# bentherien/point-cloud-reid

Measured on AMD Instinct MI355X. Metric: siamese pair-comparisons/sec @1024 pts, higher is better.
Workload: dtype bf16x3

## Files before the change

### include/pcr.h

```cpp
#ifndef PCR_H_
#define PCR_H_

#ifdef __cplusplus
extern "C" {
#endif

typedef void *pcr_stream_t;

enum pcr_status {
  PCR_OK = 0,
  PCR_ERR_INVALID = 1,
  PCR_ERR_LAUNCH = 2
};

int pcr_abi_version(void);
#define PCR_PREC_F32 0
#define PCR_PREC_BF16X3 1
#define PCR_PREC_BF16 2
const char *pcr_status_string(int status);


int pcr_fps_f32(const float *xyz, float *temp, int *idx, int B, int N, int M, pcr_stream_t stream);

int pcr_fps_dist_f32(const float *dist, float *temp, int *idx, int B, int N, int M,
// ... 1 lines not shown

int pcr_pairwise_sqdist_f32(const float *a, const float *b, float *out, int B, int N, int M, int C, int norm,
                            pcr_stream_t stream);

int pcr_ball_query_f32(const float *centres, const float *xyz, int *idx, int B, int N, int M,
                       float min_r, float max_r, int K, pcr_stream_t stream);

int pcr_ball_query_cnt_f32(const float *centres, const float *xyz, int *idx, int *cnt, int B, int N, int M,
                           float min_r, float max_r, int K, pcr_stream_t stream);

long pcr_ball_query_rows_floats(int B, int M, int K);
int pcr_ball_query_rows_ok(int N, int K, float min_r);
int pcr_ball_query_rows_f32(const float *centres, const float *xyz, int *idx, int *cnt, float *rows, int B, int N, int M,
                            float min_r, float max_r, int K, pcr_stream_t stream);

int pcr_fps_ball_query_rows_ok(int N, int M, int K);
int pcr_fps_ball_query_rows_f32(const float *xyz, float *temp, int *idx, float *new_xyz, int *cnt, float *rows, int B,
                                int N, int M, float max_r, int K, pcr_stream_t stream);

int pcr_fps_py_f32(const float *xyz, float *temp, const int *start, int *idx, int B, int N, int M,
                   pcr_stream_t stream);
int pcr_query_ball_point_f32(const float *centres, const float *xyz, int *idx, int B, int N, int M, float radius,
                             int K, pcr_stream_t stream);

int pcr_knn_f32(const float *xyz, const float *centres, int *idx, float *dist2, int B, int N, int M,
                int K, pcr_stream_t stream);

int pcr_gather_fwd_f32(const float *feat, const int *idx, float *out, int B, int C, int N, int M,
                       pcr_stream_t stream);
int pcr_gather_bwd_f32(const float *grad_out, const int *idx, float *grad_feat, int B, int C, int N,
                       int M, pcr_stream_t stream);

int pcr_group_fwd_f32(const float *feat, const int *idx, float *out, int B, int C, int N, int S,
                      int K, pcr_stream_t stream);
int pcr_group_bwd_f32(const float *grad_out, const int *idx, float *grad_feat, int B, int C, int N,
                      int S, int K, pcr_stream_t stream);

int pcr_three_nn_f32(const float *unknown, const float *known, float *dist2, int *idx, int B, int N,
                     int M, pcr_stream_t stream);

int pcr_three_interp_fwd_f32(const float *feat, const int *idx, const float *weight, float *out,
                             int B, int C, int M, int N, pcr_stream_t stream);
int pcr_three_interp_bwd_f32(const float *grad_out, const int *idx, const float *weight,
                             float *grad_feat, int B, int C, int N, int M, pcr_stream_t stream);


int pcr_box_frames_f32(const float *boxes, float *frames, int T, pcr_stream_t stream);

int pcr_points_in_boxes_batch_f32(const float *points, const float *boxes, int *out, int B, int P, int T,
                                  pcr_stream_t stream);

int pcr_points_in_boxes_f32(const float *points, const float *boxes, int *out, int B, int P, int T, pcr_stream_t stream);

#define PCR_CROP_FRAME_SENSOR 0
#define PCR_CROP_FRAME_CENTRED 1
#define PCR_CROP_FRAME_BOX 2
#define PCR_CROP_RULE_TRACKER 0
#define PCR_CROP_RULE_DATASET 1
#define PCR_CROP_MAX_POINTS 2617344
#define PCR_CROP_MAX_BOXES 65536
#define PCR_CROP_MAX_SAMPLES 65536
#define PCR_CROP_MAX_STRIDE 16
int pcr_crop_boxes_ok(int P, int M, int n, int stride);
int pcr_crop_boxes_f32(const float *points, int stride, const float *boxes, const int *rand, const long long *seed,
                       float *clouds, int *lengths, int P, int M, int n, int frame, int rule, int z_is_centre,
                       pcr_stream_t stream);


#define PCR_ASSOC_MAX_OBJECTS 4096
#define PCR_ASSOC_MAX_CLASSES 32
int pcr_assoc_pairs_ok(int T, int D, int num_classes, int cap);
int pcr_assoc_pairs_i32(const int *track_labels, const int *det_labels, const int *track_lengths, const int *det_lengths,
                        int *pairs, int *count, int T, int D, int num_classes, int min_points, int cap,
                        pcr_stream_t stream);

int pcr_assoc_cost_f32(const float *logits, const int *pairs, const int *count, const float *track_miss,
                       const float *det_new, const float *dist, float dist_max, float dist_penalty, float fill,
                       float *cost, int T, int D, int cap, pcr_stream_t stream);

#define PCR_LSA_MAX 1024
int pcr_lsa_ok(int B, int R, int C);
int pcr_lsa_f32(const float *cost, int *col4row, int *row4col, float *u, float *v, int *info, int B, int R, int C,
                pcr_stream_t stream);

int pcr_lsa_blocks_ok(int R, int C, int G);
int pcr_lsa_blocks_f32(const float *cost, const int *row_block, const int *col_block, int *col4row, int *row4col, float *u,
                       float *v, int *info, int R, int C, int G, pcr_stream_t stream);
int pcr_assoc_blocks_i32(const int *track_labels, const int *det_labels, int *row_block, int *col_block, int T, int D,
                         int de, int te, int num_classes, pcr_stream_t stream);

#define PCR_ASSOC_MAX_DECISIONS 4
#define PCR_COST_MARGIN 0
#define PCR_COST_SOFTMAX 1
typedef struct pcr_assoc_multi {
  int T, D, dd, td, cap;
  int kind, reduce;
  float dist_max, dist_penalty, fill;
  const float *logits;
  const int *pairs, *count;
  const float *det_dec, *trk_dec, *dist;
  void *ws;
  float *cost;
  int *det_choice, *trk_choice;
} pcr_assoc_multi;
typedef struct pcr_assoc_decode {
  int T, D, dd, td;
  int reduce, born_dec, kill_dec;
  float fill;
  const float *cost;
  const int *col4row, *row4col, *solver_info, *det_choice, *trk_choice;
  int *track_to_det, *det_to_track, *det_decision, *track_decision, *born, *kill, *info;
} pcr_assoc_decode;
int pcr_assoc_multi_ok(int T, int D, int dd, int td, int cap);
int pcr_assoc_multi_ws_bytes(int T, int D, int dd, int td);
int pcr_assoc_cost_multi_f32(const pcr_assoc_multi *p, pcr_stream_t stream);
int pcr_assoc_decode_i32(const pcr_assoc_decode *p, pcr_stream_t stream);


int pcr_nearest_bev_f32(const float *boxes7, float *out5, int N, pcr_stream_t stream);
int pcr_bev_frames_f32(const float *boxes5, float *frames, int N, pcr_stream_t stream);

#define PCR_IOU_AXIS 0
#define PCR_IOU_ROTATED 1
#define PCR_IOU_OVERLAP 2
#define PCR_IOU_MAX_BOXES 65535
int pcr_iou_bev_f32(const float *a, const float *b, float *out, int A, int B, int kind, pcr_stream_t stream);

#define PCR_NMS_MAX 4096
int pcr_nms_ok(int N);
int pcr_nms_ws_bytes(int N);
int pcr_nms_f32(const float *boxes, const float *scores, const float *thresh, int *order, int *keep, int *count,
                int *info, void *ws, int N, int kind, int pre_max, pcr_stream_t stream);

int pcr_track_nms_f32(const float *boxes5, const int *classes, const float *scores, const float *thresh,
                      int *suppressed, int N, pcr_stream_t stream);


#define PCR_BANK_MAX_ROW 1048576
typedef struct pcr_bank {
  int C, D, W;
  int frame_limit, replace_all, reset_on_match, propagate;
  int *lengths;
  float *boxes, *scores;
  int *labels, *ids, *steps, *misses, *next_id, *info;
  const int *track_to_det, *det_to_track, *det_labels, *det_lengths;
  const float *det_boxes, *det_scores;
  const int *born, *kill;
  const float *carry;
  int *src, *det_slot, *det_id;
} pcr_bank;
int pcr_bank_ok(int C, int D, int W, int feat_floats, int xyz_floats);
int pcr_bank_plan_i32(const pcr_bank *p, pcr_stream_t stream);
int pcr_bank_move_f32(const int *src, const float *det_feats, const float *det_xyz, float *feats, float *xyz, int C, int D,
                      int feat_floats, int xyz_floats, pcr_stream_t stream);
int pcr_bank_dist_f32(const float *boxes, const int *ids, const float *det_boxes, const float *carry_inv, float *out,
                      int C, int D, int W, pcr_stream_t stream);
int pcr_bank_retire_i32(const int *mask, int *labels, int *ids, int *lengths, int C, pcr_stream_t stream);


#define PCR_STORE_BUCKETS 20
#define PCR_STORE_PAIR_ATTEMPTS 32
#define PCR_STORE_PAIR_WORDS 40
#define PCR_STORE_MAX_SAMPLES 65536
#define PCR_STORE_INFO_RETRY 1
#define PCR_STORE_INFO_ITEM 2
#define PCR_STORE_INFO_ROW 4
typedef struct pcr_store_tables {
  int num_objects, num_classes;
  const int *obj_cls, *obj_fp, *obj_id;
  const int *nums_off, *nums_rows;
  const int *bucket_off, *bucket_rows;
  const int *pool_off, *pool_objs;
} pcr_store_tables;
int pcr_store_gather_f32(const float *points, const long long *offsets, int R, const int *rows, const int *keys,
                         const int *rand, const long long *seed, float *clouds, int *sizes, int *info, int B, int n,
                         pcr_stream_t stream);
int pcr_store_train_pairs_i32(const pcr_store_tables *tables, const int *items, const int *keys, const int *rand,
                              const long long *seed, int *rows, int *labels, int *ids, int *info, int B,
                              pcr_stream_t stream);


#define PCR_TRUTH_MAX_IDS 65536
#define PCR_TRUTH_DET_MATCH 0
#define PCR_TRUTH_DET_NEWBORN 1
#define PCR_TRUTH_DET_FP 2
#define PCR_TRUTH_TRACK_FN 3
#define PCR_TRUTH_TRACK_FP 4
#define PCR_TRUTH_TOTAL_GT 15
#define PCR_TRUTH_TOTAL_CORRECT 16
#define PCR_TRUTH_FRAMES 17
#define PCR_TRUTH_GT_TOTAL 18
#define PCR_TRUTH_TP 19
#define PCR_TRUTH_FP 20
#define PCR_TRUTH_FN 21
#define PCR_TRUTH_SWITCHES 22
#define PCR_TRUTH_UNTRACKED 23
#define PCR_TRUTH_STATS 24
typedef struct pcr_truth {
  int C, D, G, gt_cap, skip_empty, forced;
  const int *ids;
  int *slot_gt, *slot_tte, *gt_last, *stats;
  const int *col4row, *row4col, *info;
  const float *cost, *thresh;
  const int *gt_labels, *gt_ids, *gt_tte, *det_labels;
  const int *track_to_det, *det_to_track, *born, *kill;
  int *det_gt, *true_t2d, *true_d2t, *det_truth, *track_truth;
  const int *det_slot, *det_id;
} pcr_truth;
int pcr_truth_ok(int C, int D, int G, int W, int gt_cap);
int pcr_truth_cost_f32(const float *det_boxes, const int *det_labels, const float *gt_boxes, const int *gt_labels,
                       const int *gt_ids, const float *iou, float *cost, int D, int G, int W, int gt_cap,
                       pcr_stream_t stream);
int pcr_truth_decide_i32(const pcr_truth *p, pcr_stream_t stream);
int pcr_truth_record_i32(const pcr_truth *p, pcr_stream_t stream);


int pcr_knn_prefix_f32(const float *xyz, int *idx, int B, int N, int S, int K, pcr_stream_t stream);
int pcr_knn_prefix2_f32(const float *xyz, int *idx, int *idx2, int B, int N, int S, int K, int S2, int K2,
                        pcr_stream_t stream);

long pcr_packed_weight_floats(int cout, int cin);
int pcr_pack_weight_f32(const float *w, int cout, int cin, float *packed);
long pcr_packed_weight_bf16_floats(int cout, int cin);
int pcr_pack_weight_bf16x2_f32(const float *w, int cout, int cin, float *packed);

typedef struct pcr_sa_params {
  int mode, B, N, S, K, D;
  int c1, c2, c3;
  const float *xyz, *feat;
  const int *idx, *centre_idx;
  const float *wp[3], *scale[3], *shift[3];
  const float *wa, *wpq;
  const float *wps[2], *shift_pad[2];
  const int *cnt;
  int *tile_ws;
  float *pq_ws;
  int pq_ready;
  int feat_point_major, out_point_major;
  float *out;
  const float *wa_packed;
  int precision;
  const float *wps_bf[2];
  const float *wa_shift_packed;
  const float *row_tab;
  int *claim_ws;
  int pq_has_xyz;
} pcr_sa_params;
int pcr_sa_mlp_f32(const pcr_sa_params *p, pcr_stream_t stream);
long pcr_sa_claim_ws_ints(int c1, int c2, int c3, int K, int N, int precision);
long pcr_sa_tile_ws_ints(int B, int S, int K, int c2, int c3);
int pcr_sa_krow_uses_tiles(int c1, int c2, int c3, int K, int precision);
int pcr_sa_uses_row_table(int c1, int c2, int c3, int K, int precision);

int pcr_dense_pm_f32(const float *x, const float *wp, float *y, int B, int cin, int cout, int L,
                     int x_point_major, pcr_stream_t stream);
int pcr_dense_pm_prec_f32(const float *x, const float *wp_bf, float *y, int B, int cin, int cout, int L,
                          int x_point_major, int precision, pcr_stream_t stream);
int pcr_dense_pm_xyz_f32(const float *x, const float *wp_bf, const float *xyz, const float *wxyz, float *y, int B, int cin,
                         int cout, int L, int x_point_major, int precision, int q_rows, int q_off, pcr_stream_t stream);
int pcr_sa_tables_take_xyz(int mode, int D, int c1, int c2, int c3, int K, int precision);

typedef struct pcr_attn_params {
  int B, Lq, Sk;
  int c1, c2, d, cout;
  int nhead;
  int q_pos, residual;
  const float *feat_q, *xyz_q;
  const float *feat_k, *xyz_k;
  const int *kv_index;
  const int *q_index;
  const float *pos0_w, *pos0_b;
  const float *wq, *bq;
  const float *wkv, *bkv;
  const float *wmerge;
  const float *wmlp0, *wmlp2;
  const float *ln1_g, *ln1_b, *ln2_g, *ln2_b;
  const float *wfinal, *bfinal; int cfinal;
  const float *wkv_wide, *bkv_wide, *wmerge_packed;
  float *kv;
  float *out;
  int precision;
  const float *wq_bf, *wmlp0_bf, *wmlp2_bf, *wfinal_bf;
  int kv_splits;
  float *kv_part;
  const float *wkv_bf;
  const float *wmlp0_bf_xpad;
  float *pool_out;
} pcr_attn_params;
long pcr_attn_kv_floats(int d);
int pcr_attn_kv_splits(int B, int Sk, int d);
int pcr_attn_kv_f32(const pcr_attn_params *p, pcr_stream_t stream);
int pcr_attn_apply_f32(const pcr_attn_params *p, pcr_stream_t stream);
int pcr_attn_apply_pool_ok(const pcr_attn_params *p);

typedef struct pcr_live {
  const int *count;
  int period;
  int offset;
} pcr_live;
int pcr_attn_live_ok(const pcr_attn_params *p);
int pcr_attn_kv_live_f32(const pcr_attn_params *p, const pcr_live *live, pcr_stream_t stream);
int pcr_attn_apply_live_f32(const pcr_attn_params *p, const pcr_live *live, pcr_stream_t stream);

typedef struct pcr_head_params {
  int P, C, L, groups;
  const float *o;
  const float *w1, *w2;
  const float *gn1_g, *gn1_b, *gn2_g, *gn2_b;
  const float *w_out, *b_out;
  float *pooled, *logits;
  const float *w1t, *w2t;
} pcr_head_params;
int pcr_pool_head_f32(const pcr_head_params *p, pcr_stream_t stream);
int pcr_pool_head_live_f32(const pcr_head_params *p, const pcr_live *live, const float *dead_value, pcr_stream_t stream);

int pcr_pool_both_f32(const float *x, float *out, int B, int C, int L, pcr_stream_t stream);

int pcr_channel_max_f32(const float *x, float *out, int B, int C, int L, int window, pcr_stream_t stream);

int pcr_dense_f32(const float *x, const float *wp, const float *scale, const float *shift, float *y,
                  int B, int cin, int cout, int L, int act, pcr_stream_t stream);
int pcr_dense_xpm_f32(const float *x, const float *wp, const float *scale, const float *shift, float *y,
                      int B, int cin, int cout, int L, int act, pcr_stream_t stream);

int pcr_dense_gn_f32(const float *x, const float *wp, const float *gamma, const float *beta, const float *res,
                     float *y, int B, int cin, int cout, int L, int groups, int relu, pcr_stream_t stream);
int pcr_dense_prec_ok(int cin, int cout, int L);
int pcr_dense_prec_f32(const float *x, const float *wp_bf, const float *scale, const float *shift, float *y, int B, int cin,
                       int cout, int L, int act, int precision, pcr_stream_t stream);
int pcr_dense_gn_prec_f32(const float *x, const float *wp_bf, const float *gamma, const float *beta, const float *res,
                          float *y, int B, int cin, int cout, int L, int groups, int relu, int precision,
                          pcr_stream_t stream);
int pcr_dense_xpm_prec_ok(int cin, int cout, int L);
int pcr_dense_xpm_prec_f32(const float *x, const float *wp_bf, const float *scale, const float *shift, float *y, int B,
                           int cin, int cout, int L, int act, int precision, pcr_stream_t stream);


int pcr_max_over_l_f32(const float *x, float *out, int B, int C, int L, pcr_stream_t stream);

int pcr_dense_max_ok(int cin, int cout, int L);
int pcr_dense_max_f32(const float *x, const float *wp, const float *scale, const float *shift, float *out, int B, int cin,
                      int cout, int L, int act, pcr_stream_t stream);

int pcr_pack_bmm_f32(const float *t, float *wp_per_cloud, int B, int k, pcr_stream_t stream);
int pcr_dense_bmm_f32(const float *x, const float *wp_per_cloud, float *y, int B, int cin, int cout, int L,
                      pcr_stream_t stream);

int pcr_groupnorm_f32(const float *x, const float *gamma, const float *beta, const float *res, float *y, int B,
                      int C, int L, int groups, int relu, pcr_stream_t stream);


int pcr_knn_feat_f32(const float *x, float *xx_ws, int *idx, int B, int C, int N, int K, long x_bstride,
                     pcr_stream_t stream);

int pcr_edge_max_f32(const float *ta, const float *tb, const int *idx, const float *shift, float slope, float *out,
                     long out_bstride, float *out2, long out2_bstride, int B, int N, int Co, int K,
                     pcr_stream_t stream);

int pcr_local_attn_f32(const float *qkv, const int *idx, float *msg, int B, int N, int C, int K, int nhead, float eps,
                       pcr_stream_t stream);


int pcr_pack_weight_dev_f32(const float *w, int rows, int cols, int ld, int transpose, float *packed, pcr_stream_t stream);

int pcr_train_groups(int B, int L);
int pcr_train_groups_bwd(int B, int L, int cout, int cin);
struct pcr_tdense_fwd;
struct pcr_tdense_bwd;
int pcr_tdense_fwd_groups(const struct pcr_tdense_fwd *p);
int pcr_tdense_bwd_groups(const struct pcr_tdense_bwd *p);
int pcr_set_stream_min_blocks(int n);

typedef struct pcr_tdense_fwd {
  int B, cin1, cin2, cout, L;
  const float *x, *x2;
  const float *isc, *ish;
  int in_relu;
  const float *wp, *bias;
  const float *res;
  int out_relu;
  float *y;
  float *stats;
  int pool_K;
  const float *pool_gamma;
  float *pool_ymax;
  int *pool_arg;
} pcr_tdense_fwd;
int pcr_tdense_fwd_f32(const pcr_tdense_fwd *p, pcr_stream_t stream);
int pcr_tdense_fwd_pooled(const pcr_tdense_fwd *p);

typedef struct pcr_tdense_bwd {
  int B, cin1, cin2, cout, L;
  const float *g, *y;
  int dy_mode;
  const float *ka, *kb, *kc;
  const int *argmax;
  const float *pooled;
  int K, S;
  const float *x, *x2;
  const float *isc, *ish, *iinv;
  int in_relu;
  const float *wpT;
  float *dx, *dx2, *dstats, *dwp, *dbp;
  long part_stride;
  int precision;
  const float *wpT_bf;
} pcr_tdense_bwd;
int pcr_tdense_bwd_f32(const pcr_tdense_bwd *p, pcr_stream_t stream);
int pcr_pack_weight_bf16_dev_f32(const float *w, int rows, int cols, int ld, int transpose, float *packed,
                                 pcr_stream_t stream);

int pcr_local_attn_train_fwd_f32(const float *qkv, const int *idx, float *msg, int B, int N, int C, int K, int nhead,
                                 float eps, pcr_stream_t stream);
int pcr_local_attn_train_bwd_f32(const float *qkv, const int *idx, const float *g, float *dq, long dq_bstride, float *edge,
                                 int B, int N, int C, int K, int nhead, float eps, pcr_stream_t stream);

int pcr_reduce_parts_f32(const float *part, int nparts, long stride, int rows, int cols, int ld, float *out,
                         pcr_stream_t stream);

typedef struct pcr_reduce_job {
  const float *part;
  float *out;
  long stride;
  int nparts, rows, cols, ld;
} pcr_reduce_job;
int pcr_reduce_multi_f32(const pcr_reduce_job *jobs, int n, pcr_stream_t stream);

typedef struct pcr_bn_fwd_fin {
  const float *part;
  int nparts, C;
  double R;
  const float *gamma, *beta;
  float eps, momentum;
  float *running_mean, *running_var;
  float *scale, *shift, *inv_scale, *mean, *invstd;
  const float *shift0;
  int shift0_stride;
} pcr_bn_fwd_fin;
int pcr_bn_fwd_finalize_f32(const pcr_bn_fwd_fin *p, pcr_stream_t stream);

typedef struct pcr_bn_bwd_fin {
  const float *part;
  int nparts, C;
  double R;
  const float *gamma, *mean, *invstd;
  float *ka, *kb, *kc, *dgamma, *dbeta;
  const float *centre;
} pcr_bn_bwd_fin;
int pcr_bn_bwd_finalize_f32(const pcr_bn_bwd_fin *p, pcr_stream_t stream);

int pcr_sa_l1_fwd_f32(const float *xyz, const int *idx, const float *tab, const float *wa, const float *bias,
                      float *y, float *stats, int B, int N, int S, int K, int c1, pcr_stream_t stream);
int pcr_sa_l1_bwd_f32(const float *xyz, const int *idx, const float *g, const float *y, const float *ka,
                      const float *kb, const float *kc, float *dtab, float *dwa, int B, int N, int S, int K, int c1,
                      pcr_stream_t stream);
int pcr_sa_pool_fwd_f32(const float *y, const float *scale, const float *shift, float *pooled, int *argmax, float *ymax,
                        int B, int C, int S, int K, pcr_stream_t stream);
int pcr_sa_pool_bwd_stats_f32(const float *gp, const float *pooled, const float *ymax, float *part, float *gz, int B, int C,
                              int S, pcr_stream_t stream);

int pcr_tnorm_fwd_f32(const float *x, const float *gamma, const float *beta, const float *res, float *y, float *mean,
                      float *rstd, int B, int C, int L, int G, float eps, int relu, pcr_stream_t stream);
int pcr_tnorm_bwd_f32(const float *g, const float *x, const float *gamma, const float *mean, const float *rstd,
                      const float *y_relu, float *dx, float *dres, float *part, int B, int C, int L, int G,
                      pcr_stream_t stream);

typedef struct pcr_linattn {
  int B, Lq, Sk, d, H;
  float eps;
  const float *q, *k, *v;
  long q_bs, k_bs, v_bs;
  float *out, *A, *ks;
  const float *dout;
  float *dq, *dk, *dv;
  long dq_bs, dk_bs, dv_bs;
  int kv_roll;
} pcr_linattn;
int pcr_linattn_fwd_f32(const pcr_linattn *p, pcr_stream_t stream);
int pcr_linattn_bwd_f32(const pcr_linattn *p, pcr_stream_t stream);

typedef struct pcr_attn_tail {
  int B, L, d, c1, hid, out, residual;
  float eps;
  const float *msg, *res;
  const float *wm, *w0, *w2, *wmT, *w0T, *w2T;
  const float *g1, *b1, *g2, *b2;
  float *outp;
  const float *dout;
  float *dmsg, *dres, *parts;
  long part_stride;
  int precision;
  int fwd_precision;
} pcr_attn_tail;
int pcr_attn_tail_ok(int d, int c1, int hid, int out, int residual);
int pcr_attn_tail_part_floats(int d, int c1, int hid, int out);
int pcr_attn_tail_groups(const pcr_attn_tail *p);
int pcr_attn_tail_fwd_f32(const pcr_attn_tail *p, pcr_stream_t stream);
int pcr_attn_tail_bwd_f32(const pcr_attn_tail *p, pcr_stream_t stream);

typedef struct pcr_attn_head {
  int B, L, c, hd, d, np, src;
  const float *x, *xyz;
  const float *p1, *p2, *c1, *c2, *p2T;
  const float *w[3], *wT[3];
  float *outp;
  const float *dout;
  float *dx, *parts;
  long part_stride;
  int precision;
  int fwd_precision;
} pcr_attn_head;
int pcr_attn_head_ok(int c, int hd, int d, int np, int src);
int pcr_attn_head_part_floats(int c, int hd, int d, int np, int src);
int pcr_attn_head_groups(const pcr_attn_head *p);
int pcr_attn_head_fwd_f32(const pcr_attn_head *p, pcr_stream_t stream);
int pcr_attn_head_bwd_f32(const pcr_attn_head *p, pcr_stream_t stream);

int pcr_pool_pair_fwd_f32(const float *o, float *pooled, int *arg, int P, int C, int L, pcr_stream_t stream);
int pcr_pool_pair_bwd_f32(const float *g, const int *arg, float *dout, int P, int C, int L, pcr_stream_t stream);
int pcr_pool_both_fwd_f32(const float *o, float *pooled, int *arg, int P, int C, int L, pcr_stream_t stream);
int pcr_pool_both_bwd_f32(const float *g, const int *arg, float *dout, int P, int C, int L, pcr_stream_t stream);
int pcr_channel_max_fwd_f32(const float *x, float *y, int *arg, int B, int C, int L, int W, pcr_stream_t stream);
int pcr_channel_max_bwd_f32(const float *g, const int *arg, float *dx, int B, int C, int L, int W, pcr_stream_t stream);

int pcr_bn_sums_f32(const float *y, const float *g, const float *scale, const float *shift, int relu, float slope,
                    const float *centre, int centre_first, float *part, int nparts, int B, int C, int L,
                    pcr_stream_t stream);
int pcr_bn_affine_f32(const float *y, const float *g, const float *a0, const float *a1, const float *a2,
                      const float *scale, const float *shift, const float *centre, int relu, float slope, float *out,
                      int B, int C, int L, pcr_stream_t stream);
int pcr_edge_pool_fwd_f32(const float *y, const float *scale, const float *shift, float slope, float *pooled, int *arg,
                          float *yraw, int B, int C, int N, int K, pcr_stream_t stream);
int pcr_edge_pool_route_f32(const float *gp, const float *pooled, const int *arg, float slope, float *g, int B, int C,
                            int N, int K, pcr_stream_t stream);
int pcr_bmm_apply_f32(const float *x, const float *T, float *y, int B, int k, int N, int transposed, pcr_stream_t stream);
int pcr_bmm_dt_f32(const float *x, const float *dy, float *dT, int B, int k, int N, pcr_stream_t stream);

typedef struct pcr_pack_desc {
  const float *w;
  float *out;
  int rows, cols;
  int kind;
  int reserved;
} pcr_pack_desc;
int pcr_pack_weights_multi_f32(const pcr_pack_desc *descs_dev, int n, pcr_stream_t stream);

typedef struct pcr_opt_tensor {
  float *p, *g, *m, *v;
  long n;
  float step_size, bc2_sqrt, decay, one_m_beta1, beta2, one_m_beta2, eps, pad_;
} pcr_opt_tensor;
int pcr_opt_chunk(void);
int pcr_grad_sumsq_f32(const pcr_opt_tensor *tab, const int *chunk_tensor, const int *chunk_first, int n_chunks,
                       double *part, pcr_stream_t stream);
int pcr_adamw_step_f32(const pcr_opt_tensor *tab, const int *chunk_tensor, const int *chunk_first, int n_chunks,
                       const double *part, float max_norm, float *grad_norm, pcr_stream_t stream);


int pcr_wall_clock_khz(void);
int pcr_last_launch_arith(void);
int pcr_clock_probe(unsigned long long *ticks, int n_wg, int iters, pcr_stream_t stream);

#ifdef __cplusplus
}
#endif
#endif
```

### point-cloud-reid_amd/csrc/attn_kernels_impl.h

```cpp
#pragma once
#ifndef PCR_ATTN_PREC
#define PCR_ATTN_PREC 0
#endif
#include "tile_dense.h"

#include <stdio.h>

#include <vector>

namespace {
constexpr int kAPrec = PCR_ATTN_PREC;
struct AttnArgs {
  pcr_attn_params p;
  int dbg;
  int wpc;
  const int *live_count;
  int live_period, live_offset;
};

struct LiveWalk {
  unsigned n, period;
  long total;
  __device__ __forceinline__ long map(long v) const {
    const unsigned q = (unsigned)v / n;
    return (long)q * period + ((unsigned)v - q * n);
  }
};
__device__ __forceinline__ unsigned live_pairs(const AttnArgs &a) {
  int c = __builtin_amdgcn_readfirstlane(*a.live_count);
  c = c < 0 ? 0 : c;
  c -= a.live_offset;
  return (unsigned)(c < 0 ? 0 : (c > a.live_period ? a.live_period : c));
}
__device__ __forceinline__ LiveWalk live_walk(const AttnArgs &a) {
  LiveWalk w;
  w.n = live_pairs(a);
  w.period = (unsigned)a.live_period;
  const unsigned B = (unsigned)a.p.B, full = B / w.period, rem = B - full * w.period;
  w.total = (long)full * w.n + (rem < w.n ? rem : w.n);
  return w;
}
__device__ __forceinline__ bool live_cloud(const AttnArgs &a, unsigned b) {
  return b % (unsigned)a.live_period < live_pairs(a);
}

constexpr int kATraceWgs = 512, kATraceRecs = 24, kATraceMarks = 8;
__device__ unsigned long long g_attn_trace[2 * kATraceWgs * kATraceRecs * kATraceMarks];


__device__ __forceinline__ void pos_hidden(float *dst, int RP, const float *P, const float *w0,
                                           const float *b0, int d, int T) {
  for (int e = threadIdx.x; e < d * T; e += blockDim.x) {
    const int o = e / T, t = e - o * T;
    const float v = w0[o * 3] * P[t] + w0[o * 3 + 1] * P[RP + t] + w0[o * 3 + 2] * P[2 * RP + t] + b0[o];
    dst[o * RP + t] = fmaxf(v, 0.f);
  }
}

__device__ __forceinline__ void load_xyz3(float *P, int RP, const float *xyz, int L, int t0, int T) {
  for (int e = threadIdx.x; e < 3 * T; e += blockDim.x) {
    const int c = e / T, t = e - c * T;
    P[c * RP + t] = t0 + t < L ? xyz[(size_t)(t0 + t) * 3 + c] : 0.f;
  }
}

__device__ __forceinline__ void attn_kv_fold_write(const pcr_attn_params &p, const float *KVl, const float *s_kt, size_t b) {
  const int d = p.d, dh = d / p.nhead, ld = d + 1, tid = threadIdx.x;
  float *kv = p.kv + b * ((size_t)d * d + d);
  const int d_o = kThreads / d, d_dd = kThreads - d_o * d;
  int o = tid / d, dd = tid - o * d;
  int v0 = (dd / dh) * dh;
  for (int e = tid; e < d * d; e += kThreads, o += d_o, dd += d_dd) {
    if (dd >= d) {
      dd -= d;
      o++;
    }
    if (d_dd) v0 = (dd / dh) * dh;
    const float *wm = p.wmerge + (size_t)o * d + v0;
    const float *kr = KVl + dd * ld + v0;
    float m = 0.f;
#pragma unroll 8
    for (int v = 0; v < dh; v++) m += wm[v] * kr[v];
    if constexpr (kAPrec == 0) {
      const int kb = dd >> 3, rem = dd & 7;
      kv[(((size_t)kb * d + o) * 2 + (rem & 1)) * 4 + (rem >> 1)] = m;
    } else {
      const int s16 = dd >> 4, kk = dd & 15;
      const int hh = (kk >> 2) & 1, jj = (kk & 3) + ((kk >> 3) << 2);
      const size_t unit = (((size_t)s16 * (d >> 5) + (o >> 5)) * 2) * 64 + hh * 32 + (o & 31);
      const __bf16 hi = (__bf16)m;
      const __bf16 lo = (__bf16)(m - (float)hi);
      __bf16 *img = reinterpret_cast<__bf16 *>(kv);
      img[unit * 8 + jj] = hi;
      img[(unit + 64) * 8 + jj] = lo;
    }
  }
  __syncthreads();
  if (tid < d) kv[(size_t)d * d + tid] = s_kt[tid];
}

__device__ __forceinline__ void attn_kv_fold_mfma(const pcr_attn_params &p, const float *KVt, const float *s_kt, size_t b) {
  const int d = p.d, dh = d / p.nhead, ld = d + 1, tid = threadIdx.x;
  float *kv = p.kv + b * ((size_t)d * d + d);
  for (int hd = 0; hd < p.nhead; hd++) {
    const float *wm = p.wmerge_packed + (size_t)(hd * dh / 8) * d * 8;
    tile_dense(KVt + (size_t)(hd * dh) * ld + hd * dh, dh, ld, dh >> 5, wm, d, [&](float m, int o, int t) {
      const int dd = hd * dh + t;
      if constexpr (kAPrec == 0) {
        const int kb = dd >> 3, rem = dd & 7;
        kv[(((size_t)kb * d + o) * 2 + (rem & 1)) * 4 + (rem >> 1)] = m;
      } else {
        const int s16 = dd >> 4, kk = dd & 15;
        const int hh = (kk >> 2) & 1, jj = (kk & 3) + ((kk >> 3) << 2);
        const size_t unit = (((size_t)s16 * (d >> 5) + (o >> 5)) * 2) * 64 + hh * 32 + (o & 31);
        const __bf16 hi = (__bf16)m;
        const __bf16 lo = (__bf16)(m - (float)hi);
        __bf16 *img = reinterpret_cast<__bf16 *>(kv);
        img[unit * 8 + jj] = hi;
        img[(unit + 64) * 8 + jj] = lo;
      }
    });
  }
  __syncthreads();
  if (tid < d) kv[(size_t)d * d + tid] = s_kt[tid];
}

template <int TB, int NR, int WSEL, int NTW, bool BFP = false>
__device__ __forceinline__ void attn_kv_body(const AttnArgs &a) {
  constexpr int T = 32 * TB, RP = T + 1;
  constexpr int NPF = 4;
  extern __shared__ __attribute__((aligned(16))) float smem[];
  const pcr_attn_params &p = a.p;
  const int d = p.d, c2 = p.c2;
  float *XH = smem;
  float *KB = XH;
  float *VB = XH + d * RP;
  float *P = XH + (c2 + d) * RP;
  float *s_w0 = P + 3 * RP, *s_b0 = s_w0 + 3 * d;
  const int tail_a = (c2 + d + 3) * RP + 4 * d, tail_b = d * (d + 1) + d;
  float *s_ks = smem + (tail_a > tail_b ? tail_a : tail_b);
  const int tid = threadIdx.x, lane = tid & 63, wave = tid >> 6;
  const int l31 = lane & 31, h = lane >> 5;
  const size_t b = blockIdx.x;
  for (int e = tid; e < 3 * d; e += kThreads) s_w0[e] = p.pos0_w[e];
  for (int e = tid; e < d; e += kThreads) s_b0[e] = p.pos0_b[e];
  const float *feat = p.feat_k + b * c2 * p.Sk;
  const float *xyz = p.xyz_k + b * p.Sk * 3;
  const int nb = d >> 5, nT = nb * nb;
  const int dh = d / p.nhead;
  const float sk = (float)p.Sk;
  const float *bkv = p.bkv;

  f32x16 acc[NTW];
#pragma unroll
  for (int i = 0; i < NTW; i++)
#pragma unroll
    for (int r = 0; r < 16; r++) acc[i][r] = 0.f;
  int tile_ib[NTW];
#pragma unroll
  for (int it = 0; it < NTW; it++) tile_ib[it] = (wave + 4 * it) / nb;
  const int krow = tid % d, kpart = tid / d, kparts = kThreads / d;
  float ksum = 0.f;

  const int Q = T >> 2, npieces = c2 * Q;
#ifndef PCR_KV_PREFETCH
#define PCR_KV_PREFETCH 1
#endif
  const bool vec_ok = PCR_KV_PREFETCH && ((p.Sk & 3) == 0) && ((reinterpret_cast<size_t>(feat) & 15) == 0) && npieces <= NPF * kThreads;
  f32x4 pf[NPF];
  auto fetch = [&](int t0) {
#pragma unroll
    for (int u = 0; u < NPF; u++) {
      const int e = tid + u * kThreads;
      const int c = e / Q, q = e - c * Q;
      const bool ok = e < npieces;
      pf[u] = *reinterpret_cast<const f32x4 *>(feat + (size_t)(ok ? c : 0) * p.Sk + t0 + 4 * (ok ? q : 0));
    }
  };
  auto stash = [&]() {
#pragma unroll
    for (int u = 0; u < NPF; u++) {
      const int e = tid + u * kThreads;
      if (e < npieces) {
        const int c = e / Q, q = e - c * Q;
        float *dst = XH + c * RP + 4 * q;
        dst[0] = pf[u][0];
        dst[1] = pf[u][1];
        dst[2] = pf[u][2];
        dst[3] = pf[u][3];
      }
    }
  };
  const int nsplit = p.kv_splits > 1 ? p.kv_splits : 1;
  const int ntile = (p.Sk + T - 1) / T, tps = (ntile + nsplit - 1) / nsplit;
  const int t_lo = (int)blockIdx.y * tps * T;
  const int t_hi = (t_lo + tps * T) < p.Sk ? (t_lo + tps * T) : p.Sk;
  bool have = false;
  if (vec_ok && t_lo + T <= p.Sk && t_lo < t_hi) {
    fetch(t_lo);
    have = true;
  }
  for (int t0 = t_lo; t0 < t_hi; t0 += T) {
    const int valid = p.Sk - t0;
    if (have) stash();
    else load_tile(XH, RP, feat, c2, c2, p.Sk, t0, T);
    load_xyz3(P, RP, xyz, p.Sk, t0, T);
    __syncthreads();
    have = vec_ok && t0 + 2 * T <= p.Sk && t0 + T < t_hi;
    pos_hidden(XH + c2 * RP, RP, P, s_w0, s_b0, d, T);
    __syncthreads();
    auto kv_epi = [&](const f32x16 &acc, int cb, int tb, int l31, int h) {
      const int t = tb * 32 + l31;
      float *dst = XH + (cb * 32 + 4 * h) * RP + t;
      const bool live = t < valid;
      if (cb * 32 < d) {
#pragma unroll
        for (int r = 0; r < 16; r++) dst[((r & 3) + 8 * (r >> 2)) * RP] = live ? elu1(acc[r]) : 0.f;
      } else {
#pragma unroll
        for (int r = 0; r < 16; r++) dst[((r & 3) + 8 * (r >> 2)) * RP] = live ? acc[r] / sk : 0.f;
      }
    };
    auto kv_hook = [&]() { if (have) fetch(t0 + T); };
    if constexpr (BFP && kAPrec != 0 && WSEL != 0)
      tile_dense2p<kAPrec, TB, NR, WSEL, true>(XH, c2 + d, p.wkv_bf, 2 * d, true, kv_epi, bkv, nullptr, kv_hook);
    else
      tile_dense2<TB, NR, WSEL, true>(XH, c2 + d, p.wkv, 2 * d, true, kv_epi, bkv, nullptr, kv_hook);
    __syncthreads();
    {
      const float *row = KB + krow * RP;
      for (int t = kpart; t < T; t += kparts) ksum += row[t];
    }
#pragma unroll
    for (int it = 0; it < NTW; it++) {
      const int item = wave + 4 * it;
      if (item < nT) {
        const int ib = tile_ib[it], jb = item - ib * nb;
        const float *ap = KB + (ib * 32 + l31) * RP + h;
        const float *bp = VB + (jb * 32 + l31) * RP + h;
#pragma unroll 4
        for (int ks = 0; ks < T / 2; ks++)
          acc[it] = __builtin_amdgcn_mfma_f32_32x32x2f32(ap[2 * ks], bp[2 * ks], acc[it], 0, 0, 0);
      }
    }
    __syncthreads();
  }
  if (nsplit > 1) {
    float *part = p.kv_part + ((size_t)b * nsplit + blockIdx.y) * ((size_t)d * d + d);
    s_ks[tid] = ksum;
#pragma unroll
    for (int it = 0; it < NTW; it++) {
      const int item = wave + 4 * it;
      if (item < nT) {
        const int ib = tile_ib[it], jb = item - ib * nb;
#pragma unroll
        for (int r = 0; r < 16; r++)
          part[(size_t)(ib * 32 + (r & 3) + 8 * (r >> 2) + 4 * h) * d + jb * 32 + l31] = acc[it][r];
      }
    }
    __syncthreads();
    if (tid < d) {
      float s = 0.f;
      for (int pp = 0; pp < kparts; pp++) s += s_ks[pp * d + tid];
      part[(size_t)d * d + tid] = s;
    }
    return;
  }
  float *KVl = smem;
  const int ld = d + 1;
  const bool mfma_fold = p.wmerge_packed != nullptr && (dh & 31) == 0 && (d & 31) == 0;
  float *s_kt = smem + d * ld;
  s_ks[tid] = ksum;
#pragma unroll
  for (int it = 0; it < NTW; it++) {
    const int item = wave + 4 * it;
    if (item < nT) {
      const int ib = tile_ib[it], jb = item - ib * nb;
      const int v = jb * 32 + l31;
      const int hv = v / dh;
      const bool aligned = (dh & 31) == 0;
      const bool same_blk = (ib * 32) / dh == hv;
#pragma unroll
      for (int r = 0; r < 16; r++) {
        const int dd = ib * 32 + (r & 3) + 8 * (r >> 2) + 4 * h;
        const bool same = aligned ? same_blk : (dd / dh == hv);
        if (mfma_fold) KVl[v * ld + dd] = same ? acc[it][r] : 0.f;
        else KVl[dd * ld + v] = same ? acc[it][r] : 0.f;
      }
    }
  }
  __syncthreads();
  if (tid < d) {
    float s = 0.f;
    for (int pp = 0; pp < kparts; pp++) s += s_ks[pp * d + tid];
    s_kt[tid] = s;
  }
  if (mfma_fold) attn_kv_fold_mfma(p, KVl, s_kt, b);
  else attn_kv_fold_write(p, KVl, s_kt, b);
}

template <int TB, int NR, int WSEL, int NTW>
__global__ __launch_bounds__(kThreads) void attn_kv_kernel(AttnArgs a) {
  attn_kv_body<TB, NR, WSEL, NTW>(a);
}
template <int TB, int NR, int WSEL, int NTW>
__global__ __launch_bounds__(kThreads) __attribute__((amdgpu_waves_per_eu(3, 3))) void attn_kv_kernel_o3(AttnArgs a) {
  attn_kv_body<TB, NR, WSEL, NTW>(a);
}
template <int TB, int NR, int WSEL, int NTW>
__global__ __launch_bounds__(kThreads) __attribute__((amdgpu_waves_per_eu(3, 3))) void attn_kv_kernel_o3_live(AttnArgs a) {
  if (!live_cloud(a, blockIdx.x)) return;
  attn_kv_body<TB, NR, WSEL, NTW>(a);
}
template <int TB, int NR, int WSEL, int NTW, bool BFP = false>
__global__ __launch_bounds__(kThreads) __attribute__((amdgpu_waves_per_eu(2, 2))) void attn_kv_kernel_o2(AttnArgs a) {
  attn_kv_body<TB, NR, WSEL, NTW, BFP>(a);
}

constexpr int kKvsWaves = 8;
template <bool DIAG, bool BF, int XS = 4, bool ONEW = false, bool GATE = false>
// ... 382 lines not shown
          for (int e = 0; e < 8; e++) xv[e] = xf[8 * s2 + e];
          bf_split8(xv, ah[s2], al[s2], true);
        }
        f32x16 acc[2];
#pragma unroll
        for (int cb = 0; cb < 2; cb++)
#pragma unroll
          for (int r = 0; r < 16; r++) acc[cb][r] = 0.f;
        const bf16x8 *wb = reinterpret_cast<const bf16x8 *>(s_w) + lane;
#pragma unroll
        for (int s2 = 0; s2 < 4; s2++) {
          bf16x8 wh[2], wl[2];
#pragma unroll
          for (int cb = 0; cb < 2; cb++) {
            wh[cb] = wb[((s2 * 2 + cb) * 2) * 64];
            wl[cb] = wb[((s2 * 2 + cb) * 2 + 1) * 64];
          }
#pragma unroll
          for (int cb = 0; cb < 2; cb++) acc[cb] = __builtin_amdgcn_mfma_f32_32x32x16_bf16(ah[s2], wh[cb], acc[cb], 0, 0, 0);
#pragma unroll
          for (int cb = 0; cb < 2; cb++) acc[cb] = __builtin_amdgcn_mfma_f32_32x32x16_bf16(al[s2], wh[cb], acc[cb], 0, 0, 0);
#pragma unroll
          for (int cb = 0; cb < 2; cb++) acc[cb] = __builtin_amdgcn_mfma_f32_32x32x16_bf16(ah[s2], wl[cb], acc[cb], 0, 0, 0);
        }
#pragma unroll
        for (int r = 0; r < 16; r++) {
          acc[0][r] = elu1(acc[0][r] + bias0);
          acc[1][r] = (acc[1][r] + bias1) * inv_sk;
          ks += acc[0][r];
        }
#pragma unroll
        for (int r = 0; r < 16; r++) kv = __builtin_amdgcn_mfma_f32_32x32x2f32(acc[0][r], acc[1][r], kv, 0, 0, 0);
      }
    }
    ks += __shfl_xor(ks, 32, 64);
    float *KVl = s_red + cslot * KVS, *s_kt = KVl + D * LD;
    for (int round = 0; round < wpc2; round++) {
      if (wsub == round) {
#pragma unroll
        for (int r = 0; r < 16; r++) {
          float *dst = KVl + ((r & 3) + 8 * (r >> 2) + 4 * h) * LD + j;
          *dst = round == 0 ? kv[r] : *dst + kv[r];
        }
        if (h == 0) s_kt[j] = round == 0 ? ks : s_kt[j] + ks;
      }
      __syncthreads();
    }
    if (live && wsub == 0) {
      float *kvo = p.kv + (size_t)b * ((size_t)D * D + D);
      const float *ap = s_wm + j * LD + h;
      const float *bp = KVl + j * LD + h;
      const int hd = j / dh;
      f32x16 m;
#pragma unroll
      for (int r = 0; r < 16; r++) m[r] = 0.f;
#pragma unroll 4
      for (int s2 = 0; s2 < 16; s2++) {
        const float bv = bp[2 * s2];
        m = __builtin_amdgcn_mfma_f32_32x32x2f32((2 * s2 + h) / dh == hd ? bv : 0.f, ap[2 * s2], m, 0, 0, 0);
      }
      bf16x8 *img = reinterpret_cast<bf16x8 *>(kvo);
#pragma unroll
      for (int G = 0; G < 2; G++) {
        float v[8];
#pragma unroll
        for (int e = 0; e < 8; e++) v[e] = m[8 * G + e];
        bf16x8 hi, lo;
        bf_split8(v, hi, lo, true);
        const size_t unit = (((size_t)G * (D >> 5)) * 2) * 64 + h * 32 + j;
        img[unit] = hi;
        img[unit + 64] = lo;
      }
      if (lane < D) kvo[(size_t)D * D + lane] = s_kt[lane];
    }
    __syncthreads();
  }
}
#endif

__global__ __launch_bounds__(kThreads) void attn_kv_fold_kernel(AttnArgs a) {
  extern __shared__ __attribute__((aligned(16))) float smem[];
  const pcr_attn_params &p = a.p;
  const int d = p.d, dh = d / p.nhead, ld = d + 1, nsplit = p.kv_splits, tid = threadIdx.x;
  const size_t b = blockIdx.x, per = (size_t)d * d + d;
  float *KVl = smem, *s_kt = smem + d * ld;
  const float *part = p.kv_part + b * nsplit * per;
  for (int e = tid; e < d * d + d; e += kThreads) {
    float v = part[e];
    for (int y = 1; y < nsplit; y++) v += part[(size_t)y * per + e];
    if (e < d * d) {
      const int dd = e / d, c = e - dd * d;
      KVl[dd * ld + c] = (dd / dh == c / dh) ? v : 0.f;
    } else {
      s_kt[e - d * d] = v;
    }
  }
  __syncthreads();
  attn_kv_fold_write(p, KVl, s_kt, b);
}

#if PCR_ATTN_PREC == 0
template <int NRW>
__global__ __launch_bounds__(kThreads) void attn_kv_wide_kernel(AttnArgs a) {
  constexpr int TB = 1, T = 32, RP = 33, BAND = 64, RPK = BAND + 1;
  extern __shared__ __attribute__((aligned(16))) float smem[];
  const pcr_attn_params &p = a.p;
  const int d = p.d, c2 = p.c2, dh = d / p.nhead;
  const int g = blockIdx.x, hd = (g * BAND) / dh;
  const int OPW = BAND + dh;
  float *XH = smem;
  float *KB = XH, *VB = XH + BAND * RP;
  float *P = XH + (c2 + d) * RP;
  float *s_w0 = P + 3 * RP, *s_b0 = s_w0 + 3 * d;
  float *s_ks = s_b0 + d;
  const int tid = threadIdx.x, lane = tid & 63, wave = tid >> 6;
  const int l31 = lane & 31, h = lane >> 5;
  const size_t b = blockIdx.y;
  for (int e = tid; e < 3 * d; e += kThreads) s_w0[e] = p.pos0_w[e];
  for (int e = tid; e < d; e += kThreads) s_b0[e] = p.pos0_b[e];
  const float *feat = p.feat_k + b * c2 * p.Sk;
  const float *xyz = p.xyz_k + b * p.Sk * 3;
  const float sk = (float)p.Sk;
  const float *wband = p.wkv_wide + (size_t)g * ((size_t)ceil8(c2 + d) * OPW);
  const float *bband = p.bkv_wide + (size_t)g * OPW;
  const int nj = dh >> 5, nT = 2 * nj;
  f32x16 acc[4];
#pragma unroll
  for (int i = 0; i < 4; i++)
#pragma unroll
    for (int r = 0; r < 16; r++) acc[i][r] = 0.f;
  const int krow = tid & (BAND - 1), kpart = tid >> 6;
  float ksum = 0.f;
  for (int t0 = 0; t0 < p.Sk; t0 += T) {
    const int valid = p.Sk - t0;
    load_tile(XH, RP, feat, c2, c2, p.Sk, t0, T);
    load_xyz3(P, RP, xyz, p.Sk, t0, T);
    __syncthreads();
    pos_hidden(XH + c2 * RP, RP, P, s_w0, s_b0, d, T);
    __syncthreads();
    tile_dense2<TB, NRW, 0, true>(XH, c2 + d, wband, OPW, true,
                                  [&](const f32x16 &acc, int cb, int tb, int l31, int h) {
      const int t = tb * 32 + l31;
      float *dst = XH + (cb * 32 + 4 * h) * RP + t;
      const bool live = t < valid;
      if (cb * 32 < BAND) {
#pragma unroll
        for (int r = 0; r < 16; r++) dst[((r & 3) + 8 * (r >> 2)) * RP] = live ? elu1(acc[r]) : 0.f;
      } else {
#pragma unroll
        for (int r = 0; r < 16; r++) dst[((r & 3) + 8 * (r >> 2)) * RP] = live ? acc[r] / sk : 0.f;
      }
    }, bband);
    __syncthreads();
    {
      const float *row = KB + krow * RP;
      for (int t = kpart; t < T; t += 4) ksum += row[t];
    }
#pragma unroll
    for (int it = 0; it < 4; it++) {
      const int item = wave + 4 * it;
      if (item < nT) {
        const int ib = item / nj, jb = item - ib * nj;
        const float *ap = KB + (ib * 32 + l31) * RP + h;
        const float *bp = VB + (jb * 32 + l31) * RP + h;
#pragma unroll 4
        for (int ks = 0; ks < T / 2; ks++)
          acc[it] = __builtin_amdgcn_mfma_f32_32x32x2f32(ap[2 * ks], bp[2 * ks], acc[it], 0, 0, 0);
      }
    }
    __syncthreads();
  }
  float *KVt = smem;
  s_ks[tid] = ksum;
  __syncthreads();
  const float ks_total = tid < BAND ? s_ks[tid] + s_ks[64 + tid] + s_ks[128 + tid] + s_ks[192 + tid] : 0.f;
  __syncthreads();
#pragma unroll
  for (int it = 0; it < 4; it++) {
    const int item = wave + 4 * it;
    if (item < nT) {
      const int ib = item / nj, jb = item - ib * nj;
      const int v = jb * 32 + l31;
#pragma unroll
      for (int r = 0; r < 16; r++) KVt[v * RPK + ib * 32 + (r & 3) + 8 * (r >> 2) + 4 * h] = acc[it][r];
    }
  }
  __syncthreads();
  float *kv = p.kv + b * ((size_t)d * d + d);
  if (tid < BAND) kv[(size_t)d * d + g * BAND + tid] = ks_total;
  const float *wm = p.wmerge_packed + (size_t)(hd * dh / 8) * d * 8;
  tile_dense(KVt, dh, RPK, 2, wm, d, [&](float m, int o, int t) {
    const int dd = g * BAND + t;
    const int kb = dd >> 3, rem = dd & 7;
    kv[(((size_t)kb * d + o) * 2 + (rem & 1)) * 4 + (rem >> 1)] = m;
  });
}

#endif

template <int TB, int NR, bool GATE = false>
__global__ __launch_bounds__(kThreads) void attn_apply_kernel(AttnArgs a) {
  if constexpr (GATE) {
    if (!live_cloud(a, blockIdx.y)) return;
  }
  constexpr int T = 32 * TB, RP = T + 1;
  extern __shared__ __attribute__((aligned(16))) float smem[];
  const pcr_attn_params &p = a.p;
  const int d = p.d, c1 = p.c1, cout = p.cout;
  const int catC = c1 + d, catP = ceil8(catC);
  int rowsU = catP > 2 * d ? catP : 2 * d;
  if (ceil32(cout) > rowsU) rowsU = ceil32(cout);
  if (ceil32(p.cfinal) > rowsU) rowsU = ceil32(p.cfinal);
  float *U = smem;
  float *P = U + rowsU * RP;
  float *zs = P + 3 * RP;
  float *red = zs + p.nhead * RP;
  float *cst = red + 2 * (kThreads / T) * T;
  float *s_ksum = cst, *s_ln1g = cst + d, *s_ln1b = cst + 2 * d, *s_ln2g = cst + 3 * d, *s_ln2b = s_ln2g + cout;
  float *s_w0 = s_ln2b + cout, *s_b0 = s_w0 + 3 * d;
  const int tid = threadIdx.x;
  const size_t b = blockIdx.y;
  const int t0 = blockIdx.x * T;
  const size_t bq_ = p.q_index ? (size_t)p.q_index[b] : b;
  const float *feat = p.feat_q + bq_ * c1 * p.Lq;
  const size_t kb_ = p.kv_index ? (size_t)p.kv_index[b] : b;
  const float *kv = p.kv + kb_ * ((size_t)d * d + d);
  const int dh = d / p.nhead;
  for (int e = tid; e < d; e += kThreads) {
    s_ksum[e] = kv[(size_t)d * d + e];
    s_ln1g[e] = p.ln1_g[e];
    s_ln1b[e] = p.ln1_b[e];
    if (p.q_pos) {
      s_w0[3 * e] = p.pos0_w[3 * e];
      s_w0[3 * e + 1] = p.pos0_w[3 * e + 1];
      s_w0[3 * e + 2] = p.pos0_w[3 * e + 2];
      s_b0[e] = p.pos0_b[e];
    }
  }
  for (int e = tid; e < cout; e += kThreads) {
    s_ln2g[e] = p.ln2_g[e];
    s_ln2b[e] = p.ln2_b[e];
  }
  const float *ksum = s_ksum;
  float *MSG = U + c1 * RP;

  load_tile(U, RP, feat, c1, c1, p.Lq, t0, T);
  if (p.q_pos) {
    load_xyz3(P, RP, p.xyz_q + bq_ * p.Lq * 3, p.Lq, t0, T);
    __syncthreads();
    pos_hidden(MSG, RP, P, s_w0, s_b0, d, T);
    for (int e = tid; e < (catP - catC) * T; e += kThreads) U[(catC + e / T) * RP + e % T] = 0.f;
  } else {
    for (int e = tid; e < (catP - c1) * T; e += kThreads) U[(c1 + e / T) * RP + e % T] = 0.f;
  }
  __syncthreads();
  tile_dense2p<kAPrec, TB, NR>(U, p.q_pos ? catP : ceil8(c1), p.wq, d, true,
                               [&](float v, int o, int t) { MSG[o * RP + t] = elu1(v); }, p.bq);
  __syncthreads();
  for (int e = tid; e < p.nhead * T; e += kThreads) {
    const int hd = e / T, t = e - hd * T;
    float z = 0.f;
    for (int c = 0; c < dh; c++) z += MSG[(hd * dh + c) * RP + t] * ksum[hd * dh + c];
    zs[hd * RP + t] = (1.0f / (z + 1e-6f)) * (float)p.Sk;
  }
  __syncthreads();
  for (int hd = 0; hd < p.nhead; hd++)
    for (int e = tid; e < dh * T; e += kThreads) {
      const int o = hd * dh + e / T, t = e % T;
      MSG[o * RP + t] *= zs[hd * RP + t];
    }
  __syncthreads();
  tile_dense2p<kAPrec, TB, NR>(MSG, d, kv, d, true, [&](float v, int o, int t) { MSG[o * RP + t] = v; });
  __syncthreads();
  tile_layernorm(MSG, d, RP, T, s_ln1g, s_ln1b, red);
  tile_dense2p<kAPrec, TB, NR>(U, catP, p.wmlp0, 2 * d, true, [&](float v, int o, int t) { U[o * RP + t] = fmaxf(v, 0.f); });
  __syncthreads();
  tile_dense2p<kAPrec, TB, NR>(U, 2 * d, p.wmlp2, ceil32(cout), true, [&](float v, int o, int t) { U[o * RP + t] = v; });
  __syncthreads();
  tile_layernorm(U, cout, RP, T, s_ln2g, s_ln2b, red);
  if (p.residual) {
    for (int e = tid; e < cout * T; e += kThreads) {
      const int c = e / T, t = e - c * T;
      if (t0 + t < p.Lq) U[c * RP + t] += feat[(size_t)c * p.Lq + t0 + t];
    }
    __syncthreads();
  }
  int cres = cout;
  if (p.cfinal) {
    const int cf = p.cfinal;
    tile_dense2p<kAPrec, TB, NR>(U, cout, p.wfinal, ceil32(cf), true, [&](float v, int o, int t) { U[o * RP + t] = v; },
                                 p.bfinal);
    __syncthreads();
    cres = cf;
  }
  float *out = p.out + b * cres * p.Lq;
  for (int e = tid; e < cres * T; e += kThreads) {
    const int c = e / T, t = e - c * T;
    if (t0 + t < p.Lq) out[(size_t)c * p.Lq + t0 + t] = U[c * RP + t];
  }
}

#if PCR_ATTN_PREC != 0
constexpr int kApsWaves = 8;
template <bool QPOS, int C1S, int CF, int NOB = 2, int ND = 2, bool POOL = false, bool GATE = false>
__global__ __launch_bounds__(64 * kApsWaves) __attribute__((amdgpu_waves_per_eu(2, 2)))
void attn_apply_stream64_kernel(AttnArgs a) {
  static_assert(!QPOS || C1S == 2 * ND, "q_pos needs c1 == d");
  static_assert(NOB <= 2 || (NOB == 4 && !CF), "cout = 128 has no trailing conv");
  static_assert(!POOL || (!CF && NOB == 2), "pooled output: cout = 64, no trailing conv");
  constexpr int D = 32 * ND, SD = 2 * ND;
  constexpr int SQ = C1S + (QPOS ? SD : 0), S0 = C1S + SD, NX = 8 * C1S;
  extern __shared__ __attribute__((aligned(16))) float smem[];
  const pcr_attn_params &p = a.p;
  bf16x8 *s_wq = reinterpret_cast<bf16x8 *>(smem);
  bf16x8 *s_w0 = s_wq + SQ * ND * 128;
  bf16x8 *s_w2 = s_w0 + S0 * ND * 256;
  float *s_c = reinterpret_cast<float *>(s_w2 + ND * NOB * 512);
  f32x4 *s_p0 = reinterpret_cast<f32x4 *>(s_c + 448);
  float *s_ks = reinterpret_cast<float *>(s_p0 + 64);
  const int tid = threadIdx.x, lane = tid & 63, j = lane & 31, h = lane >> 5;
  const int wave = __builtin_amdgcn_readfirstlane(tid >> 6);
  LiveWalk lw{};
  if constexpr (GATE) {
    lw = live_walk(a);
    if ((long)blockIdx.x * kApsWaves >= lw.total * (POOL ? 1 : (p.Lq >> 5))) return;
  }
  {
    const f32x4 *wq = reinterpret_cast<const f32x4 *>(p.wq),
                *w0 = reinterpret_cast<const f32x4 *>((p.c1 & 15) ? p.wmlp0_bf_xpad : p.wmlp0),
                *w2 = reinterpret_cast<const f32x4 *>(p.wmlp2);
    f32x4 *dq = reinterpret_cast<f32x4 *>(s_wq), *d0 = reinterpret_cast<f32x4 *>(s_w0), *d2 = reinterpret_cast<f32x4 *>(s_w2);
    for (int e = tid; e < SQ * ND * 128; e += 64 * kApsWaves) dq[e] = wq[e];
    for (int e = tid; e < S0 * ND * 256; e += 64 * kApsWaves) d0[e] = w0[e];
    for (int e = tid; e < ND * NOB * 512; e += 64 * kApsWaves) d2[e] = w2[e];
    if (tid < D) {
      s_c[tid] = p.bq[tid];
      s_c[64 + tid] = p.ln1_g[tid];
      s_c[128 + tid] = p.ln1_b[tid];

      if (QPOS) s_p0[tid] = f32x4{p.pos0_w[3 * tid], p.pos0_w[3 * tid + 1], p.pos0_w[3 * tid + 2], p.pos0_b[tid]};
    }
    if (tid < 32 * NOB) {
      s_c[192 + tid] = p.ln2_g[tid];
      s_c[192 + 32 * NOB + tid] = p.ln2_b[tid];
    }
    if (CF && tid < 32 * CF) s_c[320 + tid] = p.bfinal[tid];
  }
  __syncthreads();
  const int nblk = p.Lq >> 5;
  const long nB = GATE ? lw.total : (long)p.B;
  const long nitem = nB * nblk;
  const int dh = D / p.nhead;
  const float skf = (float)p.Sk;
  float *ksw = s_ks + wave * 64;
  auto cvec = [&](const float *base, int cb, int g) __attribute__((always_inline)) {
    return *reinterpret_cast<const f32x4 *>(base + 32 * cb + 8 * g + 4 * h);
  };
  auto to_ops = [&](const f32x16 &acc, int G, bf16x8 &oh, bf16x8 &ol) __attribute__((always_inline)) {
    float v[8];
#pragma unroll
    for (int e = 0; e < 8; e++) v[e] = acc[8 * G + e];
    bf_split8(v, oh, ol, true);
  };
#ifdef PCR_SA_TRACE_BUILD
  const bool tracing = (a.dbg & 256) && lane == 0 && (wave == 0 || wave == 5) && blockIdx.x < kATraceWgs;
  unsigned long long *trace = g_attn_trace + (size_t)(2 * blockIdx.x + (wave ? 1 : 0)) * (kATraceRecs * kATraceMarks);
  int trace_it = 0;
#define PCR_AMARK(m)                                                                                       \
  do {                                                                                                     \
    if (tracing && trace_it < kATraceRecs) trace[trace_it * kATraceMarks + (m)] = __builtin_readcyclecounter(); \
  } while (0)
#define PCR_ANEXT() trace_it++
#else
#define PCR_AMARK(m) do { } while (0)
#define PCR_ANEXT() do { } while (0)
#endif
  const long nwav = (long)gridDim.x * kApsWaves, gw = (long)blockIdx.x * kApsWaves + wave;
  long pc = gw;
  int pblk = 0;
  float pmax = -INFINITY, psum = 0.f;
  for (long it = gw; POOL ? pc < nB : it < nitem; it += POOL ? 0 : nwav) {
    asm volatile("" ::: "memory");
    PCR_AMARK(0);
    const long vb = POOL ? pc : it / nblk;
    const int blk = POOL ? pblk : (int)(it - vb * nblk);
    const long b = GATE ? lw.map(vb) : vb;
    const size_t bq_ = p.q_index ? (size_t)p.q_index[b] : (size_t)b;
    const size_t kb_ = p.kv_index ? (size_t)p.kv_index[b] : (size_t)b;
    const float *kvp = p.kv + kb_ * ((size_t)D * D + D);
    const int t = blk * 32 + j;
    const __amdgpu_buffer_rsrc_t rfeat = __builtin_amdgcn_make_buffer_rsrc(
        const_cast<float *>(p.feat_q + bq_ * p.c1 * p.Lq), 0, p.c1 * p.Lq * 4, 0x00020000);
    const int vo = (4 * h * p.Lq + t) * 4;
    float xf[NX];
#pragma unroll
    for (int e = 0; e < NX; e++) {
      const int ch = 16 * (e >> 3) + bf_kpos(0, e & 7);
      xf[e] = __builtin_bit_cast(float, __builtin_amdgcn_raw_buffer_load_b32(rfeat, vo, ch * p.Lq * 4, 0));
    }
    if (lane < D) ksw[lane] = kvp[(size_t)D * D + lane];
    bf16x8 bh[4 * ND], bl[4 * ND];
    if constexpr (QPOS) {
      const float *xyz = p.xyz_q + (bq_ * p.Lq + t) * 3;
      const float px = xyz[0], py = xyz[1], pz = xyz[2];
#pragma unroll
      for (int s2 = 0; s2 < SD; s2++) {
        float hv[8];
#pragma unroll
        for (int e = 0; e < 8; e++) {
          const f32x4 w = s_p0[16 * s2 + bf_kpos(0, e) + 4 * h];
          const float v = w[0] * px + w[1] * py + w[2] * pz + w[3];
          hv[e] = relu_i(v);
        }
        bf_split8(hv, bh[C1S + s2], bl[C1S + s2], true);
      }
    }
#pragma unroll
    for (int e = 0; e < NX; e++) asm volatile("" : "+v"(xf[e]));
#pragma unroll
    for (int s2 = 0; s2 < C1S; s2++) {
      float xv[8];
#pragma unroll
      for (int e = 0; e < 8; e++) xv[e] = xf[8 * s2 + e];
      bf_split8(xv, bh[s2], bl[s2], true);
    }
    PCR_AMARK(1);
    f32x16 q[ND];
#pragma unroll
    for (int cb = 0; cb < ND; cb++)
#pragma unroll
      for (int r = 0; r < 16; r++) q[cb][r] = 0.f;
    {
      const bf16x8 *wb = s_wq + lane;
#pragma unroll
      for (int s2 = 0; s2 < SQ; s2++) {
        bf16x8 wh[ND], wl[ND];
#pragma unroll
        for (int cb = 0; cb < ND; cb++) {
          wh[cb] = wb[((s2 * ND + cb) * 2) * 64];
          wl[cb] = wb[((s2 * ND + cb) * 2 + 1) * 64];
        }
#pragma unroll
        for (int cb = 0; cb < ND; cb++) q[cb] = __builtin_amdgcn_mfma_f32_32x32x16_bf16(wh[cb], bh[s2], q[cb], 0, 0, 0);
#pragma unroll
        for (int cb = 0; cb < ND; cb++) q[cb] = __builtin_amdgcn_mfma_f32_32x32x16_bf16(wh[cb], bl[s2], q[cb], 0, 0, 0);
#pragma unroll
        for (int cb = 0; cb < ND; cb++) q[cb] = __builtin_amdgcn_mfma_f32_32x32x16_bf16(wl[cb], bh[s2], q[cb], 0, 0, 0);
      }
    }
    PCR_AMARK(2);
    bf16x8 mh[SD][ND], ml[SD][ND];
    {
      const bf16x8 *mb = reinterpret_cast<const bf16x8 *>(kvp) + lane;
#pragma unroll
      for (int s2 = 0; s2 < SD; s2++)
#pragma unroll
        for (int cb = 0; cb < ND; cb++) {
          mh[s2][cb] = mb[((s2 * ND + cb) * 2) * 64];
          ml[s2][cb] = mb[((s2 * ND + cb) * 2 + 1) * 64];
        }
    }
    __builtin_amdgcn_fence(__ATOMIC_RELEASE, "wavefront");
    __builtin_amdgcn_wave_barrier();
    __builtin_amdgcn_fence(__ATOMIC_ACQUIRE, "wavefront");
    float z16[2][2] = {{0.f, 0.f}, {0.f, 0.f}};
#pragma unroll
    for (int cb = 0; cb < ND; cb++)
#pragma unroll
      for (int g = 0; g < 4; g++) {
        const f32x4 bqv = cvec(s_c, cb, g), ksv = cvec(ksw, cb, g);
        float zz = 0.f;
#pragma unroll
        for (int qq = 0; qq < 4; qq++) {
          const float v = elu1(q[cb][4 * g + qq] + bqv[qq]);
          q[cb][4 * g + qq] = v;
          zz += v * ksv[qq];
        }
        if ((g & 1) == 0) z16[cb][g >> 1] = zz;
        else z16[cb][g >> 1] += zz;
      }
    float zs[2][2];
    {
      float za = z16[0][0], zb = z16[0][1], zc = z16[1][0], zd = z16[1][1];
      if (dh >= 32) {
        za += zb; zb = za;
        zc += zd; zd = zc;
      }
      if (ND == 2 && dh >= 64) {
        za += zc; zb = za; zc = za; zd = za;
      }
      za += __shfl_xor(za, 32, 64);
      zb += __shfl_xor(zb, 32, 64);
      zc += __shfl_xor(zc, 32, 64);
      zd += __shfl_xor(zd, 32, 64);
      zs[0][0] = (1.0f / (za + 1e-6f)) * skf;
      zs[0][1] = (1.0f / (zb + 1e-6f)) * skf;
      zs[1][0] = (1.0f / (zc + 1e-6f)) * skf;
      zs[1][1] = (1.0f / (zd + 1e-6f)) * skf;
    }
#pragma unroll
    for (int cb = 0; cb < ND; cb++)
#pragma unroll
      for (int r = 0; r < 16; r++) q[cb][r] *= zs[cb][r >> 3];
    bf16x8 ch_[SD], cl_[SD];
#pragma unroll
    for (int cb = 0; cb < ND; cb++)
#pragma unroll
      for (int G = 0; G < 2; G++) to_ops(q[cb], G, ch_[2 * cb + G], cl_[2 * cb + G]);
    f32x16 m[ND];
#pragma unroll
    for (int cb = 0; cb < ND; cb++)
#pragma unroll
      for (int r = 0; r < 16; r++) m[cb][r] = 0.f;
#pragma unroll
    for (int s2 = 0; s2 < SD; s2++) {
#pragma unroll
      for (int cb = 0; cb < ND; cb++) m[cb] = __builtin_amdgcn_mfma_f32_32x32x16_bf16(mh[s2][cb], ch_[s2], m[cb], 0, 0, 0);
#pragma unroll
      for (int cb = 0; cb < ND; cb++) m[cb] = __builtin_amdgcn_mfma_f32_32x32x16_bf16(mh[s2][cb], cl_[s2], m[cb], 0, 0, 0);
#pragma unroll
      for (int cb = 0; cb < ND; cb++) m[cb] = __builtin_amdgcn_mfma_f32_32x32x16_bf16(ml[s2][cb], ch_[s2], m[cb], 0, 0, 0);
    }
    auto layernorm = [&](auto &v, auto nb_tag, const float *gam, const float *bet) __attribute__((always_inline)) {
      constexpr int NB = decltype(nb_tag)::value;
      float sm = 0.f;
#pragma unroll
      for (int cb = 0; cb < NB; cb++)
#pragma unroll
        for (int r = 0; r < 16; r++) sm += v[cb][r];
      sm += __shfl_xor(sm, 32, 64);
      const float mean = sm / (32.0f * NB);
      float vr = 0.f;
#pragma unroll
      for (int cb = 0; cb < NB; cb++)
#pragma unroll
        for (int r = 0; r < 16; r++) {
          const float dlt = v[cb][r] - mean;
          vr += dlt * dlt;
        }
      vr += __shfl_xor(vr, 32, 64);
      const float inv = 1.0f / sqrtf(vr / (32.0f * NB) + 1e-5f);
#pragma unroll
      for (int cb = 0; cb < NB; cb++)
#pragma unroll
        for (int g = 0; g < 4; g++) {
          const f32x4 gv = cvec(gam, cb, g), bv = cvec(bet, cb, g);
#pragma unroll
          for (int qq = 0; qq < 4; qq++) v[cb][4 * g + qq] = (v[cb][4 * g + qq] - mean) * inv * gv[qq] + bv[qq];
        }
    };
    PCR_AMARK(3);
    layernorm(m, std::integral_constant<int, ND>{}, s_c + 64, s_c + 128);
    PCR_AMARK(4);
#pragma unroll
    for (int s2 = 0; s2 < C1S; s2++) {
      float xv[8];
#pragma unroll
      for (int e = 0; e < 8; e++) xv[e] = xf[8 * s2 + e];
      bf_split8(xv, bh[s2], bl[s2], true);
    }
#pragma unroll
    for (int cb = 0; cb < ND; cb++)
#pragma unroll
      for (int G = 0; G < 2; G++) to_ops(m[cb], G, bh[C1S + 2 * cb + G], bl[C1S + 2 * cb + G]);
    f32x16 f[SD];
#pragma unroll
    for (int cb = 0; cb < SD; cb++)
#pragma unroll
      for (int r = 0; r < 16; r++) f[cb][r] = 0.f;
    {
      const bf16x8 *wb = s_w0 + lane;
#pragma unroll
      for (int s2 = 0; s2 < S0; s2++) {
        bf16x8 wh[SD], wl[SD];
#pragma unroll
        for (int cb = 0; cb < SD; cb++) {
          wh[cb] = wb[((s2 * SD + cb) * 2) * 64];
          wl[cb] = wb[((s2 * SD + cb) * 2 + 1) * 64];
        }
#pragma unroll
        for (int cb = 0; cb < SD; cb++) f[cb] = __builtin_amdgcn_mfma_f32_32x32x16_bf16(wh[cb], bh[s2], f[cb], 0, 0, 0);
#pragma unroll
        for (int cb = 0; cb < SD; cb++) f[cb] = __builtin_amdgcn_mfma_f32_32x32x16_bf16(wh[cb], bl[s2], f[cb], 0, 0, 0);
#pragma unroll
        for (int cb = 0; cb < SD; cb++) f[cb] = __builtin_amdgcn_mfma_f32_32x32x16_bf16(wl[cb], bh[s2], f[cb], 0, 0, 0);
      }
    }
#pragma unroll
    for (int cb = 0; cb < SD; cb++) {
#pragma unroll
      for (int r = 0; r < 16; r++) f[cb][r] = relu_i(f[cb][r]);
#pragma unroll
      for (int G = 0; G < 2; G++) to_ops(f[cb], G, bh[2 * cb + G], bl[2 * cb + G]);
    }
    PCR_AMARK(5);
    f32x16 o[NOB];
#pragma unroll
    for (int cb = 0; cb < NOB; cb++)
#pragma unroll
      for (int r = 0; r < 16; r++) o[cb][r] = 0.f;
    {
      const bf16x8 *wb = s_w2 + lane;
#pragma unroll
      for (int s2 = 0; s2 < 4 * ND; s2++) {
        bf16x8 wh[NOB], wl[NOB];
#pragma unroll
        for (int cb = 0; cb < NOB; cb++) {
          wh[cb] = wb[((s2 * NOB + cb) * 2) * 64];
          wl[cb] = wb[((s2 * NOB + cb) * 2 + 1) * 64];
        }
#pragma unroll
        for (int cb = 0; cb < NOB; cb++) o[cb] = __builtin_amdgcn_mfma_f32_32x32x16_bf16(wh[cb], bh[s2], o[cb], 0, 0, 0);
#pragma unroll
        for (int cb = 0; cb < NOB; cb++) o[cb] = __builtin_amdgcn_mfma_f32_32x32x16_bf16(wh[cb], bl[s2], o[cb], 0, 0, 0);
#pragma unroll
        for (int cb = 0; cb < NOB; cb++) o[cb] = __builtin_amdgcn_mfma_f32_32x32x16_bf16(wl[cb], bh[s2], o[cb], 0, 0, 0);
      }
    }
    PCR_AMARK(6);
    layernorm(o, std::integral_constant<int, NOB>{}, s_c + 192, s_c + 192 + 32 * NOB);
    if constexpr (C1S == 2 * NOB) {
      if (p.residual) {
#pragma unroll
        for (int cb = 0; cb < NOB; cb++)
#pragma unroll
          for (int r = 0; r < 16; r++) o[cb][r] += xf[16 * cb + r];
      }
    }
    if constexpr (POOL) {
      float vm[16], vs[16];
      {
        const bool up = (j & 1) != 0;
#pragma unroll
        for (int r = 0; r < 16; r++) {
          const float lo_ = o[r >> 4][r & 15], hi_ = o[(r + 16) >> 4][(r + 16) & 15];
          const float tk = up ? hi_ : lo_, uk = up ? lo_ : hi_;
          const float pu = __uint_as_float(pcr_sort_partner<2, 1>(__float_as_uint(uk), lane));
          vm[r] = fmaxf(tk, pu);
          vs[r] = tk + pu;
        }
      }
#define PCR_POOL_STEP(N, J, BIT)                                                                      \
      {                                                                                               \
        const bool up = (j & BIT) != 0;                                                               \
        _Pragma("unroll") for (int r = 0; r < N; r++) {                                               \
          const float tm = up ? vm[r + N] : vm[r], um = up ? vm[r] : vm[r + N];                       \
          const float ts = up ? vs[r + N] : vs[r], us = up ? vs[r] : vs[r + N];                       \
          vm[r] = fmaxf(tm, __uint_as_float(pcr_sort_partner<2 * J, J>(__float_as_uint(um), lane)));  \
          vs[r] = ts + __uint_as_float(pcr_sort_partner<2 * J, J>(__float_as_uint(us), lane));        \
        }                                                                                             \
      }
      PCR_POOL_STEP(8, 2, 2)
      PCR_POOL_STEP(4, 4, 4)
      PCR_POOL_STEP(2, 8, 8)
      PCR_POOL_STEP(1, 16, 16)
#undef PCR_POOL_STEP
      pmax = fmaxf(pmax, vm[0]);
      psum += vs[0];
      if (++pblk == nblk) {
        const int e = ((j & 1) << 4) | ((j & 2) << 2) | (j & 4) | ((j & 8) >> 2) | ((j & 16) >> 4);
        const int ch = 16 * (e >> 3) + bf_kpos(h, e & 7);
        float *po = p.pool_out + (size_t)b * 128;
        po[ch] = pmax;
        po[64 + ch] = psum;
        pmax = -INFINITY;
        psum = 0.f;
        pblk = 0;
        pc += nwav;
      }
    } else if constexpr (!CF) {
      const __amdgpu_buffer_rsrc_t rout =
          __builtin_amdgcn_make_buffer_rsrc(p.out + (size_t)b * (32 * NOB) * p.Lq, 0, 32 * NOB * p.Lq * 4, 0x00020000);
#pragma unroll
      for (int e = 0; e < 16 * NOB; e++) {
        const int ch = 16 * (e >> 3) + bf_kpos(0, e & 7);
        const float v = o[e >> 4][e & 15];
        __builtin_amdgcn_raw_buffer_store_b32(__builtin_bit_cast(unsigned, v), rout, vo, ch * p.Lq * 4, 0);
      }
    } else {
#pragma unroll
      for (int cb = 0; cb < NOB; cb++)
#pragma unroll
        for (int G = 0; G < 2; G++) to_ops(o[cb], G, bh[2 * cb + G], bl[2 * cb + G]);
      f32x16 fo[CF ? CF : 1];
#pragma unroll
      for (int cb = 0; cb < CF; cb++)
#pragma unroll
        for (int r = 0; r < 16; r++) fo[cb][r] = 0.f;
      const bf16x8 *wb = reinterpret_cast<const bf16x8 *>(p.wfinal) + lane;
#pragma unroll
      for (int s2 = 0; s2 < 2 * NOB; s2++) {
        bf16x8 wh[CF ? CF : 1], wl[CF ? CF : 1];
#pragma unroll
        for (int cb = 0; cb < CF; cb++) {
          wh[cb] = wb[((s2 * CF + cb) * 2) * 64];
          wl[cb] = wb[((s2 * CF + cb) * 2 + 1) * 64];
        }
#pragma unroll
        for (int cb = 0; cb < CF; cb++) fo[cb] = __builtin_amdgcn_mfma_f32_32x32x16_bf16(wh[cb], bh[s2], fo[cb], 0, 0, 0);
#pragma unroll
        for (int cb = 0; cb < CF; cb++) fo[cb] = __builtin_amdgcn_mfma_f32_32x32x16_bf16(wh[cb], bl[s2], fo[cb], 0, 0, 0);
#pragma unroll
        for (int cb = 0; cb < CF; cb++) fo[cb] = __builtin_amdgcn_mfma_f32_32x32x16_bf16(wl[cb], bh[s2], fo[cb], 0, 0, 0);
      }
      const __amdgpu_buffer_rsrc_t rout =
          __builtin_amdgcn_make_buffer_rsrc(p.out + (size_t)b * (32 * CF) * p.Lq, 0, 32 * CF * p.Lq * 4, 0x00020000);
#pragma unroll
      for (int cb = 0; cb < CF; cb++)
#pragma unroll
        for (int g = 0; g < 4; g++) {
          const f32x4 bv = cvec(s_c + 320, cb, g);
#pragma unroll
          for (int qq = 0; qq < 4; qq++) {
            const int e = 16 * cb + 4 * g + qq;
            const int ch = 16 * (e >> 3) + bf_kpos(0, e & 7);
            const float v = fo[cb][4 * g + qq] + bv[qq];
            __builtin_amdgcn_raw_buffer_store_b32(__builtin_bit_cast(unsigned, v), rout, vo, ch * p.Lq * 4, 0);
          }
        }
    }
    __builtin_amdgcn_wave_barrier();
    PCR_AMARK(7);
    PCR_ANEXT();
  }
#undef PCR_AMARK
#undef PCR_ANEXT
}

template <int NB, bool TRANS = false>
__device__ __forceinline__ void ap128_step(f32x16 (&acc)[NB], const bf16x8 *wb, int ls, const bf16x8 &bh, const bf16x8 &bl) {
  auto mm = [](const bf16x8 &w, const bf16x8 &x, const f32x16 &c) __attribute__((always_inline)) {
    return TRANS ? __builtin_amdgcn_mfma_f32_32x32x16_bf16(x, w, c, 0, 0, 0) : __builtin_amdgcn_mfma_f32_32x32x16_bf16(w, x, c, 0, 0, 0);
  };
#pragma unroll
  for (int c0 = 0; c0 < NB; c0 += 4) {
    bf16x8 wh[4], wl[4];
#pragma unroll
    for (int cb = 0; cb < 4; cb++) {
      wh[cb] = wb[((ls * NB + c0 + cb) * 2) * 64];
      wl[cb] = wb[((ls * NB + c0 + cb) * 2 + 1) * 64];
    }
#pragma unroll
    for (int cb = 0; cb < 4; cb++) acc[c0 + cb] = mm(wh[cb], bh, acc[c0 + cb]);
#pragma unroll
    for (int cb = 0; cb < 4; cb++) acc[c0 + cb] = mm(wh[cb], bl, acc[c0 + cb]);
#pragma unroll
    for (int cb = 0; cb < 4; cb++) acc[c0 + cb] = mm(wl[cb], bh, acc[c0 + cb]);
    asm volatile("" ::: "memory");
  }
}
constexpr int kAp128Waves = 4, kAp128ChunkU = 2048, kAp128Chunks = 16;
constexpr int kAp128Npc = kAp128ChunkU / (64 * kAp128Waves);
__device__ __forceinline__ void ring128_fetch(f32x4 (&stg)[kAp128Npc], __amdgpu_buffer_rsrc_t r, int kk, int tid) {
#pragma unroll
  for (int u = 0; u < kAp128Npc; u++)
    stg[u] = __builtin_bit_cast(f32x4, __builtin_amdgcn_raw_buffer_load_b128(r, tid * 16, (kk * kAp128ChunkU + u * 64 * kAp128Waves) * 16, 0));
  asm volatile("" ::: "memory");
}
__device__ __forceinline__ void ring128_commit(f32x4 *s_ring, const f32x4 (&stg)[kAp128Npc], int k, int tid) {
  f32x4 *dst = s_ring + (k & 1) * kAp128ChunkU + tid;
#pragma unroll
  for (int u = 0; u < kAp128Npc; u++) dst[u * 64 * kAp128Waves] = stg[u];
  __syncthreads();
}
constexpr size_t kAp128Lds = (size_t)2 * kAp128ChunkU * 16 + (640 + 4 * 128 + kAp128Waves * 128) * sizeof(float);
template <int NH>
__global__ __launch_bounds__(64 * kAp128Waves) __attribute__((amdgpu_waves_per_eu(1, 1)))
void attn_apply_stream128_kernel(AttnArgs a) {
  constexpr int D = 128, ND = 4, SD = 8, GPH = 8 / NH;
  extern __shared__ __attribute__((aligned(16))) float smem[];
  const pcr_attn_params &p = a.p;
  f32x4 *s_ring = reinterpret_cast<f32x4 *>(smem);
  int coff = 2 * kAp128ChunkU * 4;
  asm volatile("" : "+s"(coff));
  float *s_c = smem + coff;
  f32x4 *s_p0 = reinterpret_cast<f32x4 *>(s_c + 640);
  float *s_ks = s_c + 640 + 4 * 128;
  const int tid = threadIdx.x, lane = tid & 63, j = lane & 31, h = lane >> 5;
  const int wave = __builtin_amdgcn_readfirstlane(tid >> 6);
  const __amdgpu_buffer_rsrc_t rwq = __builtin_amdgcn_make_buffer_rsrc(const_cast<float *>(p.wq), 0, 4 * kAp128ChunkU * 16, 0x00020000),
                               rw0 = __builtin_amdgcn_make_buffer_rsrc(const_cast<float *>(p.wmlp0), 0, 8 * kAp128ChunkU * 16, 0x00020000),
                               rw2 = __builtin_amdgcn_make_buffer_rsrc(const_cast<float *>(p.wmlp2), 0, 4 * kAp128ChunkU * 16, 0x00020000);
  f32x4 stg[kAp128Npc];
  auto fetch = [&](int k) __attribute__((always_inline)) {
    k %= kAp128Chunks;
    ring128_fetch(stg, k < 4 ? rwq : (k < 12 ? rw0 : rw2), k < 4 ? k : (k < 12 ? k - 4 : k - 12), tid);
  };
  auto commit = [&](int k) __attribute__((always_inline)) { ring128_commit(s_ring, stg, k, tid); };
  for (int e = tid; e < D; e += 64 * kAp128Waves) {
    s_c[e] = p.bq[e];
    s_c[128 + e] = p.ln1_g[e];
    s_c[256 + e] = p.ln1_b[e];
    s_c[384 + e] = p.ln2_g[e];
    s_c[512 + e] = p.ln2_b[e];
    s_p0[e] = f32x4{p.pos0_w[3 * e], p.pos0_w[3 * e + 1], p.pos0_w[3 * e + 2], p.pos0_b[e]};
  }
  fetch(0);
  commit(0);
  const int nblk = p.Lq >> 5;
  const long nitem = (long)p.B * nblk;
  const float skf = (float)p.Sk;
  float *ksw = s_ks + wave * 128;
  auto cvec = [&](const float *base, int cb, int g) __attribute__((always_inline)) {
    return *reinterpret_cast<const f32x4 *>(base + 32 * cb + 8 * g + 4 * h);
  };
  auto to_ops = [&](const f32x16 &acc, int G, bf16x8 &oh, bf16x8 &ol) __attribute__((always_inline)) {
    float v[8];
#pragma unroll
    for (int e = 0; e < 8; e++) v[e] = acc[8 * G + e];
    bf_split8(v, oh, ol, true);
  };
  auto layernorm = [&](f32x16 (&v)[ND], const float *gam, const float *bet) __attribute__((always_inline)) {
    float sm = 0.f;
#pragma unroll
    for (int cb = 0; cb < ND; cb++)
#pragma unroll
      for (int r = 0; r < 16; r++) sm += v[cb][r];
    sm += __shfl_xor(sm, 32, 64);
    const float mean = sm / (float)D;
    float vr = 0.f;
#pragma unroll
    for (int cb = 0; cb < ND; cb++)
#pragma unroll
      for (int r = 0; r < 16; r++) {
        const float dlt = v[cb][r] - mean;
        vr += dlt * dlt;
      }
    vr += __shfl_xor(vr, 32, 64);
    const float inv = 1.0f / sqrtf(vr / (float)D + 1e-5f);
#pragma unroll
    for (int cb = 0; cb < ND; cb++)
#pragma unroll
      for (int g = 0; g < 4; g++) {
        const f32x4 gv = cvec(gam, cb, g), bv = cvec(bet, cb, g);
#pragma unroll
        for (int qq = 0; qq < 4; qq++) v[cb][4 * g + qq] = (v[cb][4 * g + qq] - mean) * inv * gv[qq] + bv[qq];
      }
  };
  for (long it0 = (long)blockIdx.x * kAp128Waves; it0 < nitem; it0 += (long)gridDim.x * kAp128Waves) {
    const long item = it0 + wave;
    const bool live = item < nitem;
    const long it = live ? item : nitem - 1;
    const long b = it / nblk;
    const int blk = (int)(it - b * nblk);
    const size_t bq_ = p.q_index ? (size_t)p.q_index[b] : (size_t)b;
    const size_t kb_ = p.kv_index ? (size_t)p.kv_index[b] : (size_t)b;
    const float *kvp = p.kv + kb_ * ((size_t)D * D + D);
    const int t = blk * 32 + j;
    const __amdgpu_buffer_rsrc_t rfeat = __builtin_amdgcn_make_buffer_rsrc(
        const_cast<float *>(p.feat_q + bq_ * D * p.Lq), 0, D * p.Lq * 4, 0x00020000);
    const int vo = (4 * h * p.Lq + t) * 4;
    auto load_x = [&](float (&xf)[64]) __attribute__((always_inline)) {
#pragma unroll
      for (int e = 0; e < 64; e++) {
        const int ch = 16 * (e >> 3) + bf_kpos(0, e & 7);
        xf[e] = __builtin_bit_cast(float, __builtin_amdgcn_raw_buffer_load_b32(rfeat, vo, ch * p.Lq * 4, 0));
      }
    };
    ksw[lane] = kvp[(size_t)D * D + lane];
    ksw[64 + lane] = kvp[(size_t)D * D + 64 + lane];
    bf16x8 bh[16], bl[16];
    {
      float xf[64];
      load_x(xf);
      const float *xyz = p.xyz_q + (bq_ * p.Lq + t) * 3;
      const float px = xyz[0], py = xyz[1], pz = xyz[2];
#pragma unroll
      for (int s2 = 0; s2 < SD; s2++) {
        float hv[8];
#pragma unroll
        for (int e = 0; e < 8; e++) {
          const f32x4 w = s_p0[16 * s2 + bf_kpos(0, e) + 4 * h];
          const float v = w[0] * px + w[1] * py + w[2] * pz + w[3];
          hv[e] = relu_i(v);
        }
        bf_split8(hv, bh[SD + s2], bl[SD + s2], true);
      }
#pragma unroll
      for (int e = 0; e < 64; e++) asm volatile("" : "+v"(xf[e]));
#pragma unroll
      for (int s2 = 0; s2 < SD; s2++) {
        float xv[8];
#pragma unroll
        for (int e = 0; e < 8; e++) xv[e] = xf[8 * s2 + e];
        bf_split8(xv, bh[s2], bl[s2], true);
      }
    }
    f32x16 q[ND];
#pragma unroll
    for (int cb = 0; cb < ND; cb++)
#pragma unroll
      for (int g = 0; g < 4; g++) {
        const f32x4 bqv = cvec(s_c, cb, g);
#pragma unroll
        for (int qq = 0; qq < 4; qq++) q[cb][4 * g + qq] = bqv[qq];
      }
#pragma unroll
    for (int k = 0; k < 4; k++) {
      fetch(k + 1);
      const bf16x8 *wb = reinterpret_cast<const bf16x8 *>(s_ring + (k & 1) * kAp128ChunkU) + lane;
#pragma unroll
      for (int ls = 0; ls < 4; ls++) ap128_step<ND>(q, wb, ls, bh[4 * k + ls], bl[4 * k + ls]);
      commit(k + 1);
    }
    float zg[SD];
#pragma unroll
    for (int cb = 0; cb < ND; cb++)
#pragma unroll
      for (int g = 0; g < 4; g++) {
        const f32x4 ksv = cvec(ksw, cb, g);
        float zz = 0.f;
#pragma unroll
        for (int qq = 0; qq < 4; qq++) {
          const float v = elu1(q[cb][4 * g + qq]);
          q[cb][4 * g + qq] = v;
          zz += v * ksv[qq];
        }
        if ((g & 1) == 0) zg[2 * cb + (g >> 1)] = zz;
        else zg[2 * cb + (g >> 1)] += zz;
      }
    float zs[NH];
#pragma unroll
    for (int hd = 0; hd < NH; hd++) {
      float z = zg[hd * GPH];
#pragma unroll
      for (int gi = 1; gi < GPH; gi++) z += zg[hd * GPH + gi];
      z += __shfl_xor(z, 32, 64);
      zs[hd] = (1.0f / (z + 1e-6f)) * skf;
    }
#pragma unroll
    for (int cb = 0; cb < ND; cb++)
#pragma unroll
      for (int r = 0; r < 16; r++) q[cb][r] *= zs[(2 * cb + (r >> 3)) / GPH];
    {
      bf16x8 ch_[SD], cl_[SD];
#pragma unroll
      for (int cb = 0; cb < ND; cb++)
#pragma unroll
        for (int G = 0; G < 2; G++) to_ops(q[cb], G, ch_[2 * cb + G], cl_[2 * cb + G]);
#pragma unroll
      for (int cb = 0; cb < ND; cb++)
#pragma unroll
        for (int r = 0; r < 16; r++) q[cb][r] = 0.f;
      const bf16x8 *mb = reinterpret_cast<const bf16x8 *>(kvp) + lane;
      bf16x8 mh[2][ND], ml[2][ND];
#pragma unroll
      for (int cb = 0; cb < ND; cb++) {
        mh[0][cb] = mb[(cb * 2) * 64];
        ml[0][cb] = mb[(cb * 2 + 1) * 64];
      }
#pragma unroll
      for (int s2 = 0; s2 < SD; s2++) {
        const int c = s2 & 1;
        if (s2 + 1 < SD) {
#pragma unroll
          for (int cb = 0; cb < ND; cb++) {
            mh[c ^ 1][cb] = mb[(((s2 + 1) * ND + cb) * 2) * 64];
            ml[c ^ 1][cb] = mb[(((s2 + 1) * ND + cb) * 2 + 1) * 64];
          }
        }
        asm volatile("" ::: "memory");
#pragma unroll
        for (int cb = 0; cb < ND; cb++) q[cb] = __builtin_amdgcn_mfma_f32_32x32x16_bf16(mh[c][cb], ch_[s2], q[cb], 0, 0, 0);
#pragma unroll
        for (int cb = 0; cb < ND; cb++) q[cb] = __builtin_amdgcn_mfma_f32_32x32x16_bf16(mh[c][cb], cl_[s2], q[cb], 0, 0, 0);
#pragma unroll
        for (int cb = 0; cb < ND; cb++) q[cb] = __builtin_amdgcn_mfma_f32_32x32x16_bf16(ml[c][cb], ch_[s2], q[cb], 0, 0, 0);
      }
    }
    layernorm(q, s_c + 128, s_c + 256);
#pragma unroll
    for (int cb = 0; cb < ND; cb++)
#pragma unroll
      for (int G = 0; G < 2; G++) to_ops(q[cb], G, bh[SD + 2 * cb + G], bl[SD + 2 * cb + G]);
    f32x16 f[2 * ND];
#pragma unroll
    for (int cb = 0; cb < 2 * ND; cb++)
#pragma unroll
      for (int r = 0; r < 16; r++) f[cb][r] = 0.f;
#pragma unroll
// ... 131 lines not shown
        fetch(k + 1);
        if (has) {
          const bf16x8 *wb = reinterpret_cast<const bf16x8 *>(s_ring + (k & 1) * kAp128ChunkU) + lane;
#pragma unroll
          for (int ls = 0; ls < 2; ls++) {
            if (k < 4) {
              ap128_step<8, true>(acc, wb, ls, bh[2 * k + ls], bl[2 * k + ls]);
            } else {
              const int s2 = 2 * k + ls - SD;
              float hv[8];
#pragma unroll
              for (int e = 0; e < 8; e++) {
                const f32x4 w = s_p0[16 * s2 + bf_kpos(0, e) + 4 * h];
                const float v = w[0] * pxyz[0] + w[1] * pxyz[1] + w[2] * pxyz[2] + w[3];
                hv[e] = relu_i(v);
              }
              bf16x8 hh, hl;
              bf_split8(hv, hh, hl, true);
              ap128_step<8, true>(acc, wb, ls, hh, hl);
            }
          }
        }
        commit(k + 1);
      }
      if (hasn) issue(bn, blkn);
      else {
#pragma unroll
        for (int e = 0; e < 64; e++) xf[e] = 0.f;
        pxyz[0] = pxyz[1] = pxyz[2] = 0.f;
      }
      if (has) {
        float bias[8];
#pragma unroll
        for (int cb = 0; cb < 8; cb++) bias[cb] = s_bkv[cb * 32 + j];
#pragma unroll
        for (int r = 0; r < 16; r++) {
#pragma unroll
          for (int cb = 0; cb < 4; cb++) {
            acc[cb][r] = elu1(acc[cb][r] + bias[cb]);
            ks[cb] += acc[cb][r];
            acc[4 + cb][r] = (acc[4 + cb][r] + bias[4 + cb]) * inv_sk;
          }
        }
#pragma unroll
        for (int i = 0; i < NKV; i++) {
          const int hd = i / (TPH * TPH), ib = hd * TPH + (i % (TPH * TPH)) / TPH, jb = hd * TPH + i % TPH;
#pragma unroll
          for (int r = 0; r < 16; r++) kv[i] = __builtin_amdgcn_mfma_f32_32x32x2f32(acc[4 + jb][r], acc[ib][r], kv[i], 0, 0, 0);
        }
      }
    }
#pragma unroll
    for (int cb = 0; cb < 4; cb++) ks[cb] += __shfl_xor(ks[cb], 32, 64);
    if (wpc > 1) {
      int ln = lane;
      asm volatile("" : "+v"(ln));
      float *red = s_red + (size_t)cslot * KVU * 64 + ln;
      for (int round = 0; round < wpc; round++) {
        if (wsub == round) {
#pragma unroll
          for (int i = 0; i < NKV; i++)
#pragma unroll
            for (int r = 0; r < 16; r++) {
              float *dst = red + (i * 16 + r) * 64;
              *dst = round == 0 ? kv[i][r] : *dst + kv[i][r];
            }
#pragma unroll
          for (int cb = 0; cb < 4; cb++) {
            float *dst = red + (NKV * 16 + cb) * 64;
            *dst = round == 0 ? ks[cb] : *dst + ks[cb];
          }
        }
        __syncthreads();
      }
#pragma unroll
      for (int i = 0; i < NKV; i++)
#pragma unroll
        for (int r = 0; r < 16; r++) kv[i][r] = red[(i * 16 + r) * 64];
#pragma unroll
      for (int cb = 0; cb < 4; cb++) ks[cb] = red[(NKV * 16 + cb) * 64];
    }
    if (live) {
      int ln = lane;
      asm volatile("" : "+v"(ln));
      const int j = ln & 31, h = ln >> 5;
      const __amdgpu_buffer_rsrc_t rkv =
          __builtin_amdgcn_make_buffer_rsrc(p.kv + (size_t)b * ((size_t)D * D + D), 0, (D * D + D) * 4, 0x00020000);
      const __amdgpu_buffer_rsrc_t rwm = __builtin_amdgcn_make_buffer_rsrc(const_cast<float *>(p.wmerge), 0, D * D * 4, 0x00020000);
      for (int ob = wsub; ob < 4; ob += wpc) {
        const int wrow = ((ob * 32 + j) * D + 4 * h) * 4;
#pragma unroll
        for (int hd = 0; hd < NH; hd++) {
          f32x4 w[TPH][4];
#pragma unroll
          for (int jj = 0; jj < TPH; jj++)
#pragma unroll
            for (int g = 0; g < 4; g++)
              w[jj][g] = __builtin_bit_cast(f32x4, __builtin_amdgcn_raw_buffer_load_b128(rwm, wrow, ((hd * TPH + jj) * 32 + 8 * g) * 4, 0));
#pragma unroll
          for (int dl = 0; dl < TPH; dl++) {
            const int db = hd * TPH + dl;
            f32x16 m;
#pragma unroll
            for (int r = 0; r < 16; r++) m[r] = 0.f;
#pragma unroll
            for (int jj = 0; jj < TPH; jj++) {
              const int i = hd * TPH * TPH + dl * TPH + jj;
#pragma unroll
              for (int r = 0; r < 16; r++) m = __builtin_amdgcn_mfma_f32_32x32x2f32(kv[i][r], w[jj][r >> 2][r & 3], m, 0, 0, 0);
            }
#pragma unroll
            for (int G = 0; G < 2; G++) {
              float v[8];
#pragma unroll
              for (int e = 0; e < 8; e++) v[e] = m[8 * G + e];
              bf16x8 hi, lo;
              bf_split8(v, hi, lo, true);
              const int unit = (((db * 2 + G) * (D >> 5) + ob) * 2) * 64 + h * 32 + j;
              __builtin_amdgcn_raw_buffer_store_b128(__builtin_bit_cast(u32x4, hi), rkv, unit * 16, 0, 0);
              __builtin_amdgcn_raw_buffer_store_b128(__builtin_bit_cast(u32x4, lo), rkv, (unit + 64) * 16, 0, 0);
            }
          }
        }
      }
      if (wsub == 0 && h == 0) {
#pragma unroll
        for (int cb = 0; cb < 4; cb++)
          __builtin_amdgcn_raw_buffer_store_b32(__builtin_bit_cast(unsigned, ks[cb]), rkv, (D * D + cb * 32 + j) * 4, 0, 0);
      }
    }
  }
}
#endif

}

static int attn_check(const pcr_attn_params &p) {
  if (p.B < 0 || p.Lq < 1 || p.Sk < 1 || p.c1 < 1 || p.c2 < 1 || p.cout < 1 || p.nhead < 1) return 1;
  if (p.d < 32 || p.d > 512 || (p.d & 31) || p.d % p.nhead) return 1;
  if (p.d > 128 && ((p.d & 63) || ((p.d / p.nhead) & 63) || p.d / p.nhead > 256)) return 1;
  if ((p.c2 & 7) || p.cout > 512 || p.cfinal > 512) return 1;
  if (!p.feat_q || !p.feat_k || !p.xyz_k || !p.kv || !p.pos0_w || !p.pos0_b || !p.wq || !p.bq || !p.wkv ||
      !p.bkv || !p.wmerge || !p.wmlp0 || !p.wmlp2 || !p.ln1_g || !p.ln1_b || !p.ln2_g || !p.ln2_b)
    return 1;
  if (p.q_pos && (!p.xyz_q || p.c1 != p.c2 || p.c1 != p.d)) return 1;
  if (p.residual && p.cout != p.c1) return 1;
  if (p.cfinal && (!p.wfinal || !p.bfinal || (p.cout & 7))) return 1;
  return 0;
}

static void attn_dump_trace(const char *path, const char *tag, int wgs, int B, int Sk) {
  static int launches = 0;
  static const int skip = pcr_tune_int("PCR_SA_TRACE_SKIP");
  launches++;
  if (launches <= skip || launches > skip + 8) return;
  static std::vector<unsigned long long> host(2 * kATraceWgs * kATraceRecs * kATraceMarks);
  if (hipDeviceSynchronize() != hipSuccess) return;
  if (hipMemcpyFromSymbol(host.data(), HIP_SYMBOL(g_attn_trace), host.size() * sizeof(unsigned long long)) != hipSuccess) return;
  FILE *f = fopen(path, "a");
  if (!f) return;
  const int n = 2 * (wgs < kATraceWgs ? wgs : kATraceWgs);
  fprintf(f, "launch %d kernel %s wgs %d B %d Sk %d\n", launches, tag, wgs, B, Sk);
  for (int w = 0; w < n; w++) {
    const unsigned long long *t = host.data() + (size_t)w * (kATraceRecs * kATraceMarks);
    fprintf(f, "wg %d", w);
    for (int i = 0; i < kATraceRecs * kATraceMarks; i++) fprintf(f, " %llu", t[i]);
    fprintf(f, "\n");
  }
  fclose(f);
}

static bool attn_set_live(AttnArgs &a, const pcr_live *live) {
  a.live_count = nullptr;
  a.live_period = a.live_offset = 0;
  if (!live) return true;
  if (!live->count || live->period < 1 || live->offset < 0) return false;
  a.live_count = live->count;
  a.live_period = live->period;
  a.live_offset = live->offset;
  return true;
}
static bool attn_live_shape(const pcr_attn_params &p) {
  return p.d == 64 && p.c1 == 64 && p.c2 == 64 && p.cout == 64 && p.kv_splits <= 1;
}
template <auto KERN, auto KERN_LIVE>
static inline int attn_launch_g(dim3 grid, dim3 block, size_t lds, hipStream_t st, const AttnArgs &a) {
  return a.live_count ? pcr_launch_lds<KERN_LIVE>(grid, block, lds, st, a) : pcr_launch_lds<KERN>(grid, block, lds, st, a);
}

static int attn_kv_narrow(const pcr_attn_params *pp, const pcr_live *live, pcr_stream_t stream) {
  AttnArgs a;
  a.p = *pp;
  a.dbg = 0;
  a.wpc = 0;
  if (!attn_set_live(a, live) || (live && !attn_live_shape(*pp))) return PCR_ERR_INVALID;
  const int d = pp->d;
  if (pp->c2 < pp->d) return PCR_ERR_INVALID;
  const int tb = d <= 64 ? 2 : 1, RP = 32 * tb + 1;
  size_t lds = (size_t)(pp->c2 + d + 3) * RP + 4 * d;
  const size_t lds2 = (size_t)d * (d + 1) + d;
  if (lds2 > lds) lds = lds2;
  lds = (lds + kThreads) * sizeof(float);
  if (lds > (size_t)kMaxDynLds) return PCR_ERR_INVALID;
  const int ntile = (pp->Sk + 32 * tb - 1) / (32 * tb);
  int ns = pp->kv_splits > 1 ? pp->kv_splits : 1;
  if (ns > 1 && (!pp->kv_part || ns > 64)) return PCR_ERR_INVALID;
  if (ns > ntile) ns = ntile;
  a.p.kv_splits = ns;
  dim3 g(pp->B, ns), blk(kThreads);
  hipStream_t st = pcr_s(stream);
  constexpr bool kBfUnit = kAPrec != 0;
  const bool bfk = kBfUnit && pp->wkv_bf != nullptr;
  if (ns == 1 && d == 64 && (pp->c2 == 64 || (pp->c2 == 128 && bfk && pp->Sk >= 128)) && (pp->Sk & 31) == 0 && pp->nhead >= 1 &&
      64 % pp->nhead == 0) {
    const bool bf = bfk;
    const bool wide = pp->c2 == 128;
    pcr_note_arith(bf ? PCR_PREC_BF16X3 : PCR_PREC_F32);
    const int nblk = pp->Sk >> 5;
    const int minw = wide ? 4 : 2;
    int wpc2 = 1;
    while (wpc2 * 2 <= (nblk < 4 ? nblk : 4)) wpc2 *= 2;
    if (wpc2 < minw) wpc2 = minw;
    static const int no_onew = pcr_tune_int("PCR_ATTN_NO_ONEW");
    const bool onew = kBfUnit && bf && !wide && nblk <= 4 && !no_onew;
    if (onew) wpc2 = 1;
    const int cpg = kKvsWaves / wpc2;
    const size_t wu = bf ? (size_t)((wide ? 8 : 4) + 4) * 512 : 4096;
    const size_t lds_s = (wu * 4 + 256 + 128 + 64 * 65 + (onew ? (size_t)0 : (size_t)cpg * (64 * 65 + 64))) * sizeof(float);
    const long rounds = ((long)pp->B + cpg - 1) / cpg;
    const int gs = (int)(rounds < pcr_cu_count() ? rounds : pcr_cu_count());
    const dim3 gg(gs), bb(64 * kKvsWaves);
    const bool mh = pp->nhead >= 2;
    if (bf && wide) {
      if (live) return PCR_ERR_INVALID;
      constexpr int W = kBfUnit ? 8 : 4;
      return mh ? pcr_launch_lds<attn_kv_stream64_kernel<true, kBfUnit, W>>(gg, bb, lds_s, st, a)
                : pcr_launch_lds<attn_kv_stream64_kernel<false, kBfUnit, W>>(gg, bb, lds_s, st, a);
    }
    if (!bf)
      return mh ? attn_launch_g<attn_kv_stream64_kernel<true, false>, attn_kv_stream64_kernel<true, false, 4, false, true>>(gg, bb, lds_s, st, a)
                : attn_launch_g<attn_kv_stream64_kernel<false, false>, attn_kv_stream64_kernel<false, false, 4, false, true>>(gg, bb, lds_s, st, a);
    static const char *atrace = pcr_tune_str("PCR_ATTN_TRACE");
    if (atrace) a.dbg |= 256;
    int rc;
    if (onew)
      rc = mh ? attn_launch_g<attn_kv_stream64_kernel<true, kBfUnit, 4, kBfUnit>, attn_kv_stream64_kernel<true, kBfUnit, 4, kBfUnit, true>>(gg, bb, lds_s, st, a)
              : attn_launch_g<attn_kv_stream64_kernel<false, kBfUnit, 4, kBfUnit>, attn_kv_stream64_kernel<false, kBfUnit, 4, kBfUnit, true>>(gg, bb, lds_s, st, a);
    else
      rc = mh ? attn_launch_g<attn_kv_stream64_kernel<true, kBfUnit>, attn_kv_stream64_kernel<true, kBfUnit, 4, false, true>>(gg, bb, lds_s, st, a)
              : attn_launch_g<attn_kv_stream64_kernel<false, kBfUnit>, attn_kv_stream64_kernel<false, kBfUnit, 4, false, true>>(gg, bb, lds_s, st, a);
    if (atrace) attn_dump_trace(atrace, "kv64", gs, (int)pp->B, pp->Sk);
    return rc;
  }
#if PCR_ATTN_PREC != 0
  if (ns == 1 && d == 32 && pp->c2 == 32 && pp->wkv_bf && (pp->Sk & 31) == 0 && pp->nhead >= 1 && 32 % pp->nhead == 0) {
    pcr_note_arith(PCR_PREC_BF16X3);
    const int nblk = pp->Sk >> 5;
    int wpc2 = 1;
    while (wpc2 * 2 <= (nblk < kKvsWaves ? nblk : kKvsWaves)) wpc2 *= 2;
    if (wpc2 < 2) wpc2 = 2;
    const int cpg = kKvsWaves / wpc2;
    const size_t lds_s = (size_t)(4096 + 128 + 64 + 32 * 33 + cpg * (32 * 33 + 32)) * sizeof(float);
    const long rounds = ((long)pp->B + cpg - 1) / cpg;
    const long cap = 2L * pcr_cu_count();
    return pcr_launch_lds<attn_kv_stream32_kernel>(dim3((unsigned)(rounds < cap ? rounds : cap)), dim3(64 * kKvsWaves), lds_s, st, a);
  }
  static const int no_kv128 = pcr_tune_int("PCR_ATTN_NO_KV128");
  if (ns == 1 && d == 128 && pp->c2 == 128 && pp->wkv_bf && (pp->Sk & 31) == 0 && pp->Sk >= 256 &&
      (pp->nhead == 2 || pp->nhead == 4) && !no_kv128) {
    pcr_note_arith(PCR_PREC_BF16X3);
    a.wpc = attn_kv128_wpc(pp->Sk >> 5);
    static const int wpc_t = pcr_tune_int("PCR_ATTN_KV128_WPC");
    if (wpc_t == 1 || wpc_t == 2 || wpc_t == 4) a.wpc = wpc_t;
    const int cpg = kAp128Waves / a.wpc;
    const size_t lds_s = kKv128Lds0 + (a.wpc > 1 ? (size_t)cpg * (16 * (16 / pp->nhead) + 4) * 64 * sizeof(float) : 0);
    const long nwg = ((long)pp->B + cpg - 1) / cpg;
    const dim3 gg((unsigned)(nwg < pcr_cu_count() ? nwg : pcr_cu_count())), bb(64 * kAp128Waves);
    return pp->nhead == 2 ? pcr_launch_lds<attn_kv_stream128_kernel<2>>(gg, bb, lds_s, st, a)
                          : pcr_launch_lds<attn_kv_stream128_kernel<4>>(gg, bb, lds_s, st, a);
  }
#endif
  if (live && (d != 64 || ns != 1)) return PCR_ERR_INVALID;
  pcr_note_arith(PCR_PREC_F32);
  int rc;
  if (d == 32) rc = pcr_launch_lds<attn_kv_kernel<2, 1, 2, 1>>(g, blk, lds, st, a);
  else if (d == 64) rc = attn_launch_g<attn_kv_kernel_o3<2, 1, 1, 1>, attn_kv_kernel_o3_live<2, 1, 1, 1>>(g, blk, lds, st, a);
  else if (d == 128) {
    if (kBfUnit && pp->wkv_bf && pp->Sk >= 256) rc = pcr_launch_lds<attn_kv_kernel_o2<1, 2, 1, 4, true>>(g, blk, lds, st, a);
    else rc = pcr_launch_lds<attn_kv_kernel_o2<1, 2, 1, 4>>(g, blk, lds, st, a);
  }
  else rc = pcr_launch_lds<attn_kv_kernel<1, 2, 0, 4>>(g, blk, lds, st, a);
  if (rc != PCR_OK || ns == 1) return rc;
  return pcr_launch_lds<attn_kv_fold_kernel>(dim3(pp->B), blk, ((size_t)d * (d + 1) + d) * sizeof(float), st, a);
}

static bool aps64_shape(const pcr_attn_params &p) {
  const bool aps_in = p.c1 == 64 || ((p.c1 == 32 || (p.c1 < 16 && p.wmlp0_bf_xpad)) && !p.q_pos && !p.residual);
  const bool aps_out = (p.cout == 64 && (p.cfinal == 0 || p.cfinal == 128) && p.c1 >= 32) ||
                       (p.cout == 128 && !p.cfinal && !p.residual && p.c1 == 64) ||
                       (p.cout == 32 && p.cfinal == 64 && !p.residual && p.c1 < 16);
  return p.d == 64 && aps_in && aps_out && (p.Lq & 31) == 0 && (p.nhead == 1 || p.nhead == 2 || p.nhead == 4);
}

static int attn_apply_launch(const pcr_attn_params *pp, const pcr_live *live, pcr_stream_t stream) {
  const pcr_attn_params &p = *pp;
  AttnArgs a;
  a.p = p;
  a.dbg = 0;
  a.wpc = 0;
  if (!attn_set_live(a, live) || (live && !attn_live_shape(p))) return PCR_ERR_INVALID;
  const int tb = p.d <= 32 ? 4 : (p.d <= 64 ? 2 : 1), T = 32 * tb, RP = T + 1;
  const int catP = ceil8(p.c1 + p.d);
  int rowsU = catP > 2 * p.d ? catP : 2 * p.d;
  if (ceil32(p.cout) > rowsU) rowsU = ceil32(p.cout);
  if (ceil32(p.cfinal) > rowsU) rowsU = ceil32(p.cfinal);
  size_t lds = ((size_t)(rowsU + 3 + p.nhead) * RP + 2 * (kThreads / T) * T + 7 * p.d + 2 * p.cout) *
               sizeof(float);
  if (lds > (size_t)kMaxDynLds) return PCR_ERR_INVALID;
  dim3 g((p.Lq + T - 1) / T, p.B), blk(kThreads);
  hipStream_t st = pcr_s(stream);
  pcr_note_arith(kAPrec != 0 ? PCR_PREC_BF16X3 : PCR_PREC_F32);
#if PCR_ATTN_PREC != 0
  const int aps_c1s = (p.c1 + 15) >> 4, aps_nd = p.d >> 5;
  const size_t aps_lds = (size_t)((aps_c1s + (p.q_pos ? 2 * aps_nd : 0)) * aps_nd * 128 + (aps_c1s + 2 * aps_nd) * aps_nd * 256 +
                                  aps_nd * (p.cout >> 5) * 512) * 16 +
                         (size_t)(448 + 256 + 64 * kApsWaves) * sizeof(float);
  static const int no_s128 = pcr_tune_int("PCR_ATTN_NO_STREAM128");
  if (p.d == 128 && p.c1 == 128 && p.cout == 128 && !p.cfinal && p.q_pos && p.residual && (p.Lq & 31) == 0 && p.Lq >= 256 &&
      (p.nhead == 1 || p.nhead == 2 || p.nhead == 4) && !no_s128) {
    const long nitem = (long)p.B * (p.Lq >> 5);
    const long nwg = (nitem + kAp128Waves - 1) / kAp128Waves;
    const dim3 gg((unsigned)(nwg < pcr_cu_count() ? nwg : pcr_cu_count())), bb(64 * kAp128Waves);
    if (p.nhead == 1) return pcr_launch_lds<attn_apply_stream128_kernel<1>>(gg, bb, kAp128Lds, st, a);
    if (p.nhead == 2) return pcr_launch_lds<attn_apply_stream128_kernel<2>>(gg, bb, kAp128Lds, st, a);
    return pcr_launch_lds<attn_apply_stream128_kernel<4>>(gg, bb, kAp128Lds, st, a);
  }
  if (p.d == 32 && p.c1 == 32 && p.cout == 32 && !p.cfinal && (p.Lq & 31) == 0 && (p.nhead == 1 || p.nhead == 2)) {
    const long nitem = (long)p.B * (p.Lq >> 5);
    const long nwg = (nitem + kApsWaves - 1) / kApsWaves;
    const dim3 gg((unsigned)(nwg < pcr_cu_count() ? nwg : pcr_cu_count())), bb(64 * kApsWaves);
    return p.q_pos ? pcr_launch_lds<attn_apply_stream64_kernel<true, 2, 0, 1, 1>>(gg, bb, aps_lds, st, a)
                   : pcr_launch_lds<attn_apply_stream64_kernel<false, 2, 0, 1, 1>>(gg, bb, aps_lds, st, a);
  }
  if (aps64_shape(p) && aps_lds <= (size_t)kMaxDynLds) {
    const int nob = p.cout >> 5;
    const long nitem = (long)p.B * (p.Lq >> 5);
    const long nwg = (nitem + kApsWaves - 1) / kApsWaves;
    const dim3 gg((unsigned)(nwg < pcr_cu_count() ? nwg : pcr_cu_count())), bb(64 * kApsWaves);
    const bool cf = p.cfinal != 0;
    static const char *aptrace = pcr_tune_str("PCR_ATTN_TRACE");
    if (aptrace) a.dbg = 256;
    if (pp->pool_out) {
      const long nwgp = ((long)p.B + kApsWaves - 1) / kApsWaves;
      const dim3 ggp((unsigned)(nwgp < pcr_cu_count() ? nwgp : pcr_cu_count()));
      return attn_launch_g<attn_apply_stream64_kernel<false, 4, 0, 2, 2, true>, attn_apply_stream64_kernel<false, 4, 0, 2, 2, true, true>>(ggp, bb, aps_lds, st, a);
    }
    int rc;
    if (nob == 4)
      rc = p.q_pos ? pcr_launch_lds<attn_apply_stream64_kernel<true, 4, 0, 4>>(gg, bb, aps_lds, st, a)
                   : pcr_launch_lds<attn_apply_stream64_kernel<false, 4, 0, 4>>(gg, bb, aps_lds, st, a);
    else if (p.c1 < 16) rc = pcr_launch_lds<attn_apply_stream64_kernel<false, 1, 2, 1>>(gg, bb, aps_lds, st, a);
    else if (p.c1 == 32)
      rc = cf ? pcr_launch_lds<attn_apply_stream64_kernel<false, 2, 4>>(gg, bb, aps_lds, st, a)
              : pcr_launch_lds<attn_apply_stream64_kernel<false, 2, 0>>(gg, bb, aps_lds, st, a);
    else if (p.q_pos)
      rc = cf ? attn_launch_g<attn_apply_stream64_kernel<true, 4, 4>, attn_apply_stream64_kernel<true, 4, 4, 2, 2, false, true>>(gg, bb, aps_lds, st, a)
              : attn_launch_g<attn_apply_stream64_kernel<true, 4, 0>, attn_apply_stream64_kernel<true, 4, 0, 2, 2, false, true>>(gg, bb, aps_lds, st, a);
    else
      rc = cf ? attn_launch_g<attn_apply_stream64_kernel<false, 4, 4>, attn_apply_stream64_kernel<false, 4, 4, 2, 2, false, true>>(gg, bb, aps_lds, st, a)
              : attn_launch_g<attn_apply_stream64_kernel<false, 4, 0>, attn_apply_stream64_kernel<false, 4, 0, 2, 2, false, true>>(gg, bb, aps_lds, st, a);
    if (aptrace) attn_dump_trace(aptrace, "apply64", (int)gg.x, (int)p.B, p.Lq);
    return rc;
  }
#endif
  const bool wide = 2 * p.d > 128 || p.cout > 128 || p.cfinal > 128;
  if (tb == 4 && !live)
    return wide ? pcr_launch_lds<attn_apply_kernel<4, 2>>(g, blk, lds, st, a) : pcr_launch_lds<attn_apply_kernel<4, 1>>(g, blk, lds, st, a);
  if (tb == 2)
    return wide ? attn_launch_g<attn_apply_kernel<2, 2>, attn_apply_kernel<2, 2, true>>(g, blk, lds, st, a)
                : attn_launch_g<attn_apply_kernel<2, 1>, attn_apply_kernel<2, 1, true>>(g, blk, lds, st, a);
  if (live) return PCR_ERR_INVALID;
  int widest = 2 * p.d > p.cout ? 2 * p.d : p.cout;
  if (p.cfinal > widest) widest = p.cfinal;
#if PCR_ATTN_PREC == 0
  if (widest > 512) return pcr_launch_lds<attn_apply_kernel<1, 8>>(g, blk, lds, st, a);
  if (widest > 256) return pcr_launch_lds<attn_apply_kernel<1, 4>>(g, blk, lds, st, a);
#else
  if (widest > 256) return PCR_ERR_INVALID;
#endif
  return pcr_launch_lds<attn_apply_kernel<1, 2>>(g, blk, lds, st, a);
}

#if PCR_ATTN_PREC == 1
int pcr_attn_kv_bf3(const pcr_attn_params *pp, const pcr_live *live, pcr_stream_t stream) { return attn_kv_narrow(pp, live, stream); }
int pcr_attn_apply_bf3(const pcr_attn_params *pp, const pcr_live *live, pcr_stream_t stream) { return attn_apply_launch(pp, live, stream); }
#else
int pcr_attn_kv_bf3(const pcr_attn_params *pp, const pcr_live *live, pcr_stream_t stream);
int pcr_attn_apply_bf3(const pcr_attn_params *pp, const pcr_live *live, pcr_stream_t stream);

static bool attn_bf(const pcr_attn_params &p, pcr_attn_params &q) {
  const int widest = 2 * p.d > p.cout ? (2 * p.d > p.cfinal ? 2 * p.d : p.cfinal) : (p.cout > p.cfinal ? p.cout : p.cfinal);
  if (p.precision == 0 || p.d > 128 || widest > 256 || !p.wq_bf || !p.wmlp0_bf || !p.wmlp2_bf ||
      (p.cfinal && !p.wfinal_bf))
    return false;
  q = p;
  q.wq = p.wq_bf; q.wmlp0 = p.wmlp0_bf; q.wmlp2 = p.wmlp2_bf; q.wfinal = p.wfinal_bf;
  return true;
}

PCR_EXPORT int pcr_attn_kv_splits(int B, int Sk, int d) {
  (void)B;
  if (Sk < 1 || d > 64) return 1;
  if ((d == 64 || d == 32) && (Sk & 31) == 0) return 1;
  const int ntile = (Sk + 63) / 64;
  return ntile >= 16 ? 4 : (ntile >= 8 ? 2 : 1);
}

static int attn_kv_entry(const pcr_attn_params *pp, const pcr_live *live, pcr_stream_t stream) {
  if (!pp || attn_check(*pp)) return PCR_ERR_INVALID;
  if (live && !attn_live_shape(*pp)) return PCR_ERR_INVALID;
  if (pp->B == 0) return PCR_OK;
  const int d = pp->d;
  if (d > 128) {
    AttnArgs a;
    a.p = *pp;
    a.dbg = 0;
    a.wpc = 0;
    if (!pp->wkv_wide || !pp->bkv_wide || !pp->wmerge_packed || pp->B > 65535) return PCR_ERR_INVALID;
    pcr_note_arith(PCR_PREC_F32);
    const int dh = d / pp->nhead;
    size_t lds = ((size_t)(pp->c2 + d + 3) * 33 + 4 * d + kThreads) * sizeof(float);
    const size_t lds2 = (size_t)dh * 65 * sizeof(float);
    if (lds2 > lds) lds = lds2;
    if (lds > (size_t)kMaxDynLds) return PCR_ERR_INVALID;
    dim3 g(d / 64, pp->B), blk(kThreads);
    if (64 + dh <= 256) return pcr_launch_lds<attn_kv_wide_kernel<2>>(g, blk, lds, pcr_s(stream), a);
    return pcr_launch_lds<attn_kv_wide_kernel<3>>(g, blk, lds, pcr_s(stream), a);
  }
  pcr_attn_params q;
  if (attn_bf(*pp, q)) return pcr_attn_kv_bf3(&q, live, stream);
  return attn_kv_narrow(pp, live, stream);
}

PCR_EXPORT int pcr_attn_kv_f32(const pcr_attn_params *pp, pcr_stream_t stream) { return attn_kv_entry(pp, nullptr, stream); }
PCR_EXPORT int pcr_attn_kv_live_f32(const pcr_attn_params *pp, const pcr_live *live, pcr_stream_t stream) {
  return attn_kv_entry(pp, live, stream);
}
PCR_EXPORT int pcr_attn_live_ok(const pcr_attn_params *pp) {
  return (pp && !attn_check(*pp) && attn_live_shape(*pp)) ? 1 : 0;
}

static bool attn_pool_ok(const pcr_attn_params &p) {
  pcr_attn_params q;
  return aps64_shape(p) && p.c1 == 64 && p.cout == 64 && !p.cfinal && !p.q_pos && attn_bf(p, q);
}

PCR_EXPORT int pcr_attn_apply_pool_ok(const pcr_attn_params *pp) {
  return (pp && !attn_check(*pp) && attn_pool_ok(*pp)) ? 1 : 0;
}

static int attn_apply_entry(const pcr_attn_params *pp, const pcr_live *live, pcr_stream_t stream) {
  if (!pp || attn_check(*pp) || (!pp->out && !pp->pool_out)) return PCR_ERR_INVALID;
  if (pp->pool_out && !attn_pool_ok(*pp)) return PCR_ERR_INVALID;
  if (live && !attn_live_shape(*pp)) return PCR_ERR_INVALID;
  if (pp->B == 0) return PCR_OK;
  if (pp->B > 65535) return PCR_ERR_INVALID;
  pcr_attn_params q;
  if (attn_bf(*pp, q)) return pcr_attn_apply_bf3(&q, live, stream);
  return attn_apply_launch(pp, live, stream);
}

PCR_EXPORT int pcr_attn_apply_f32(const pcr_attn_params *pp, pcr_stream_t stream) { return attn_apply_entry(pp, nullptr, stream); }
PCR_EXPORT int pcr_attn_apply_live_f32(const pcr_attn_params *pp, const pcr_live *live, pcr_stream_t stream) {
  return attn_apply_entry(pp, live, stream);
}
#endif
```

### point-cloud-reid_amd/mmdet3d/models/backbone_net.py

```python
import torch.nn as nn

from .pointnet2_utils import PointNetFeaturePropagationSA, PointNetSetAbstractionEdgeSA


_NO_KNN2 = bool(__import__("os").environ.get("PCR_NO_KNN2"))


class Pointnet_Backbone(nn.Module):
    def __init__(self, input_channels=3, use_xyz=True, conv_out=32, mul=1, radius=[0.3, 0.5, 0.7],
                 nsample=[32, 48, 48]):
        super().__init__()
        sa1, sa2, sa3 = 32 * mul, 64 * mul, 128 * mul
        self.SA_modules = nn.ModuleList()
        for r, k, widths in ((radius[0], nsample[0], [input_channels, sa1, sa1, sa1]),
                             (radius[1], nsample[1], [sa2, sa2, sa2, sa2]),
                             (radius[2], nsample[2], [sa3, sa3, sa3, sa3])):
            self.SA_modules.append(PointNetSetAbstractionEdgeSA(npoint=None, radius=r, nsample=k, mlp=widths,
                                                                sampling="RANDOM", use_xyz=use_xyz, use_knn=True))
        self.FP_modules = nn.ModuleList()
        self.FP_modules.append(PointNetFeaturePropagationSA(mlp=[67, sa1, sa1], mlp_inte=[sa2, 3, sa2, sa2, sa1]))
        self.FP_modules.append(PointNetFeaturePropagationSA(mlp=[160, sa3, sa2], mlp_inte=[sa3, sa1, sa3, sa2, sa2]))
        self.FP_modules.append(PointNetFeaturePropagationSA(mlp=[192, sa3, sa3], mlp_inte=[sa3, sa2, sa3, sa2, sa3]))
        self.cov_final = nn.Conv1d(sa1, conv_out, kernel_size=1)
        self.FP_modules[0].interpolation.fuse_final_conv(self.cov_final)

    def _break_up_pc(self, pc):
        xyz = pc[..., 0:3].contiguous()
        features = pc[..., 3:].transpose(1, 2).contiguous() if pc.size(-1) > 3 else None
        return xyz, features

    def forward(self, pointcloud, numpoints):
        if self.training:
            from pcr_amd import train_graph
            return train_graph.backbone(self, pointcloud, numpoints)
        xyz, features = self._break_up_pc(pointcloud)
        l_xyz, l_features = [xyz], [features]
        shared = None
        for i, sa in enumerate(self.SA_modules):
            knn_idx = None
            if i == 0 and len(self.SA_modules) > 1 and hasattr(sa, "shares_knn_with") and not _NO_KNN2 and \
                    sa.shares_knn_with(self.SA_modules[1], xyz.shape[1], numpoints[0], numpoints[1]):
                from pcr_amd import engine
                knn_idx, shared = engine.knn_prefix2(xyz.contiguous(), numpoints[0], sa.nsample, numpoints[1],
                                                     self.SA_modules[1].nsample)
            elif i == 1 and shared is not None:
                knn_idx = shared
            li_xyz, li_features = sa(l_xyz[i], l_features[i], numpoints[i]) if knn_idx is None else \
                sa(l_xyz[i], l_features[i], numpoints[i], knn_idx=knn_idx)
            l_xyz.append(li_xyz)
            l_features.append(li_features)
        l_features[0] = xyz.transpose(1, 2).contiguous()
        for i in (2, 1, 0):
            l_features[i] = self.FP_modules[i](l_xyz[i], l_xyz[i + 1], l_features[i], l_features[i + 1])
        if self.FP_modules[0].interpolation._final is not None:
            return l_xyz[0], l_features[0]
        return l_xyz[0], self._cov_final_unfused(l_features[0])

    def _cov_final_unfused(self, x):
        from pcr_amd import engine
        key = (str(x.device), engine.param_version(self.cov_final))
        if getattr(self, "_cf_key", None) != key:
            object.__setattr__(self, "_cf_w", engine.pack_weight(self.cov_final.weight, x.device))
            object.__setattr__(self, "_cf_b", self.cov_final.bias.detach().to(x.device).float().contiguous())
            object.__setattr__(self, "_cf_key", key)
        return engine.dense(x.contiguous(), self._cf_w, self.cov_final.weight.shape[0], None, self._cf_b, 0)
```

### point-cloud-reid_amd/mmdet3d/models/pointnet2_utils.py

```python
import torch
import torch.nn as nn

from pcr_amd import engine
from pcr_amd import _lib as L


def random_point_sample(xyz, npoint):
    return torch.arange(npoint, dtype=torch.long, device=xyz.device).repeat(xyz.size(0), 1)


def farthest_point_sample(xyz, npoint, start=None):
    L.require_cuda(xyz)
    L.require_f32(xyz)
    xyz = xyz.contiguous()
    B, N, _ = xyz.shape
    if start is None:
        start = torch.randint(0, N, (B,), dtype=torch.long).to(xyz.device)
    if not start.is_cuda and start.numel() and (int(start.min()) < 0 or int(start.max()) >= N):
        raise L.PcrError("farthest_point_sample: start index outside [0, %d)" % N)
    start = start.to(device=xyz.device, dtype=torch.int32).contiguous()
    idx = torch.empty((B, npoint), dtype=torch.int32, device=xyz.device)
    temp = torch.full((B, N), 1e10, dtype=torch.float32, device=xyz.device)
    L.run.pcr_fps_py_f32(xyz, temp, start, idx, B, N, npoint, L.stream_ptr())
    return idx.long()


def query_ball_point(radius, nsample, xyz, new_xyz):
    L.require_cuda(xyz, new_xyz)
    L.require_f32(xyz, new_xyz)
    xyz, new_xyz = xyz.contiguous(), new_xyz.contiguous()
    B, N, _ = xyz.shape
    S = new_xyz.shape[1]
    idx = torch.empty((B, S, nsample), dtype=torch.int32, device=xyz.device)
    L.run.pcr_query_ball_point_f32(new_xyz, xyz, idx, B, N, S, radius, nsample, L.stream_ptr())
    return idx.long()


def knn_point(nsample, xyz, new_xyz):
    from mmdet3d.ops.point_ops import knn
    return knn(nsample, xyz.contiguous(), new_xyz.contiguous(), False).transpose(1, 2).contiguous().long()


def index_points(points, idx):
    from mmdet3d.ops.point_ops import gather_points, grouping_operation
    feats = points.transpose(1, 2).contiguous()
    i32 = idx.to(torch.int32).contiguous()
    if idx.dim() == 2:
        return gather_points(feats, i32).transpose(1, 2).contiguous()
    return grouping_operation(feats, i32).permute(0, 2, 3, 1).contiguous()


class _Planned(nn.Module):

    def _plan(self, device, build):
        if self.training:
            raise L.PcrError(
                "%s: the fused HIP path implements eval-mode inference (BatchNorm folded from running "
                "statistics); call .eval() -- training kernels are listed as next work in DESIGN.md"
                % type(self).__name__)
        key = (str(device), engine.param_version(self))
        if getattr(self, "_plan_key", None) != key:
            object.__setattr__(self, "_plan_obj", build(device))
            object.__setattr__(self, "_plan_key", key)
        return self._plan_obj


def _attn_holder(m, pos_name, d_model, c_q, c_k, c_pos_out, c_ff_in, out_dim):
    setattr(m, pos_name, nn.Sequential(nn.Linear(3, d_model), nn.ReLU(), nn.Linear(d_model, c_pos_out)))
    m.q_proj = nn.Linear(c_q, d_model, bias=False)
    m.k_proj = nn.Linear(c_k, d_model, bias=False)
    m.v_proj = nn.Linear(c_k, d_model, bias=False)
    m.merge = nn.Linear(d_model, d_model, bias=False)
    m.mlp = nn.Sequential(nn.Linear(c_ff_in, d_model * 2, bias=False), nn.ReLU(True),
                          nn.Linear(d_model * 2, out_dim, bias=False))
    m.norm1 = nn.LayerNorm(d_model)
    m.norm2 = nn.LayerNorm(out_dim)


class Self_Attention(_Planned):

    def __init__(self, d_model, nhead, attention="linear"):
        super().__init__()
        self.dim = d_model // nhead
        self.nhead = nhead
        _attn_holder(self, "pos_mlp", d_model, d_model, d_model, d_model, d_model * 2, d_model)

    def forward(self, feat, xyz, mask=None):
        assert mask is None, "masks are never passed by the ReID model path"
        plan = self._plan(feat.device, lambda dev: engine.AttnPlan(self, "pos_mlp", dev, self.nhead,
                                                                   q_pos=True, k_pos=True, residual=True))
        feat = feat.contiguous()
        xyz = xyz.contiguous()
        return plan.run(feat, xyz, feat, xyz)


class PointNetSetAbstractionEdgeSA(_Planned):
    def __init__(self, npoint, radius, nsample, mlp, sampling, use_xyz=True, group_all=False, use_knn=False):
        super().__init__()
        if group_all:
            raise NotImplementedError("group_all SA layers are never built by the ReID backbone (backbone_net.py:50-81)")
        if sampling not in ("RANDOM", "FPS"):
            raise ValueError("sampling must be 'RANDOM' or 'FPS'")
        self.npoint, self.radius, self.nsample = npoint, radius, nsample
        self.use_xyz, self.sampling, self.use_knn, self.group_all = use_xyz, sampling, use_knn, group_all
        mlp = list(mlp)
        if use_xyz:
            mlp[0] += 3
        self.mlp_convs = nn.ModuleList()
        self.mlp_bns = nn.ModuleList()
        last = mlp[0]
        for out_channel in mlp[1:]:
            self.mlp_convs.append(nn.Conv2d(last, out_channel, 1))
            self.mlp_bns.append(nn.BatchNorm2d(out_channel))
            last = out_channel
        self.self_attention = Self_Attention(last, 2, "linear")

    def shares_knn_with(self, nxt, n, numpoints, numpoints_next):
        return (isinstance(nxt, PointNetSetAbstractionEdgeSA) and self.sampling == "RANDOM" and self.use_knn and
                nxt.sampling == "RANDOM" and nxt.use_knn and numpoints == n and numpoints_next <= numpoints and
                self.nsample <= nxt.nsample <= min(64, n))

    def forward(self, xyz, points, numpoints, knn_idx=None):
        plan = self._plan(xyz.device, lambda dev: engine.SaPlan(list(self.mlp_convs), list(self.mlp_bns), dev, mode=0))
        xyz = xyz.contiguous()
        points = None if points is None else points.contiguous()
        if self.sampling == "RANDOM" and self.use_knn:
            idx = knn_idx if knn_idx is not None else engine.knn_prefix(xyz, numpoints, self.nsample)
            assert idx.shape == (xyz.shape[0], numpoints, self.nsample)
            pooled = engine.guarded(lambda: plan.run(xyz, points, idx))
            new_xyz = xyz[:, :numpoints].contiguous()
            return new_xyz, self.self_attention(pooled, new_xyz)
        centre = (farthest_point_sample(xyz, numpoints) if self.sampling == "FPS"
                  else random_point_sample(xyz, numpoints)).to(torch.int32).contiguous()
        new_xyz = index_points(xyz, centre)
        idx = (knn_point(self.nsample, xyz, new_xyz) if self.use_knn
               else query_ball_point(self.radius, self.nsample, xyz, new_xyz)).to(torch.int32).contiguous()
        pooled = engine.guarded(lambda: plan.run(xyz, points, idx, centre_idx=centre))
        return new_xyz, self.self_attention(pooled, new_xyz)


class FP_SA(_Planned):

    def __init__(self, last_channel, feat1_dim, feat2_dim, d_model, out_dim, nhead, attention="linear"):
        super().__init__()
        self.dim = d_model // nhead
        self.nhead = nhead
        _attn_holder(self, "pos_mlp2", d_model, feat1_dim, feat2_dim, feat2_dim, feat1_dim + d_model, out_dim)
        self._final = None

    def fuse_final_conv(self, conv):
        object.__setattr__(self, "_final", conv)
        object.__setattr__(self, "_plan_key", None)

    def forward(self, feat1, xyz1, feat2, xyz2, mask=None):
        assert mask is None
        plan = self._plan(feat1.device, lambda dev: engine.AttnPlan(self, "pos_mlp2", dev, self.nhead, q_pos=False,
                                                                    k_pos=False, residual=False, final=self._final))
        return plan.run(feat1.contiguous(), xyz1.contiguous(), feat2.contiguous(), xyz2.contiguous())

    def _plan(self, device, build):
        key = (str(device), engine.param_version(self),
               None if self._final is None else engine.param_version(self._final))
        if self.training:
            raise L.PcrError("FP_SA: the fused HIP path implements eval-mode inference; call .eval()")
        if getattr(self, "_plan_key", None) != key:
            object.__setattr__(self, "_plan_obj", build(device))
            object.__setattr__(self, "_plan_key", key)
        return self._plan_obj


class PointNetFeaturePropagationSA(nn.Module):
    def __init__(self, mlp, mlp_inte):
        super().__init__()
        self.mlp_convs = nn.ModuleList()
        self.mlp_bns = nn.ModuleList()
        last = mlp[0]
        for out_channel in mlp[1:]:
            self.mlp_convs.append(nn.Conv1d(last, out_channel, 1))
            self.mlp_bns.append(nn.BatchNorm1d(out_channel))
            last = out_channel
        self.interpolation = FP_SA(last_channel=mlp_inte[0], feat1_dim=mlp_inte[1], feat2_dim=mlp_inte[2],
                                   d_model=mlp_inte[3], out_dim=mlp_inte[4], nhead=2, attention="linear")

    def forward(self, xyz1, xyz2, points1, points2):
        return self.interpolation(points1, xyz1, points2, xyz2)
```

### point-cloud-reid_amd/pcr_amd/abi.py

```python
import ctypes

import numpy as np
import torch

_CTYPES = {"int": ctypes.c_int, "float": ctypes.c_float, "double": ctypes.c_double, "long": ctypes.c_long,
           "ptr": ctypes.c_void_p}


def _block(name, decl):
    fields = []
    for group in decl.split(";"):
        ty, *names = group.split()
        base, _, n = ty.partition("[")
        ct = _CTYPES[base] * int(n[:-1]) if n else _CTYPES[base]
        fields += [(f, ct) for f in names]
    return type(name, (ctypes.Structure,), {"_fields_": fields})


BankParams = _block("BankParams", """
    int C D W frame_limit replace_all reset_on_match propagate;
    ptr lengths boxes scores labels ids steps misses next_id info;
    ptr track_to_det det_to_track det_labels det_lengths det_boxes det_scores born kill carry; ptr src det_slot det_id""")

AssocMultiParams = _block("AssocMultiParams", """
    int T D dd td cap kind reduce; float dist_max dist_penalty fill; ptr logits pairs count det_dec trk_dec dist ws cost;
    ptr det_choice trk_choice""")
AssocDecodeParams = _block("AssocDecodeParams", """
    int T D dd td reduce born_dec kill_dec; float fill; ptr cost col4row row4col solver_info det_choice trk_choice;
    ptr track_to_det det_to_track det_decision track_decision born kill info""")

TruthParams = _block("TruthParams", """
    int C D G gt_cap skip_empty forced; ptr ids slot_gt slot_tte gt_last stats col4row row4col info cost thresh;
    ptr gt_labels gt_ids gt_tte det_labels track_to_det det_to_track born kill;
    ptr det_gt true_t2d true_d2t det_truth track_truth det_slot det_id""")

StoreTables = _block("StoreTables", """
    int num_objects num_classes; ptr obj_cls obj_fp obj_id nums_off nums_rows bucket_off bucket_rows pool_off pool_objs""")

SaParams = _block("SaParams", """
    int mode B N S K D c1 c2 c3; ptr xyz feat idx centre_idx; ptr[3] wp scale shift; ptr wa wpq; ptr[2] wps shift_pad;
    ptr cnt tile_ws pq_ws; int pq_ready feat_point_major out_point_major; ptr out wa_packed; int precision;
    ptr[2] wps_bf; ptr wa_shift_packed row_tab claim_ws; int pq_has_xyz""")
AttnParams = _block("AttnParams", """
    int B Lq Sk c1 c2 d cout nhead q_pos residual; ptr feat_q xyz_q feat_k xyz_k kv_index q_index pos0_w pos0_b;
    ptr wq bq wkv bkv wmerge wmlp0 wmlp2 ln1_g ln1_b ln2_g ln2_b wfinal bfinal; int cfinal;
    ptr wkv_wide bkv_wide wmerge_packed kv out; int precision; ptr wq_bf wmlp0_bf wmlp2_bf wfinal_bf; int kv_splits;
    ptr kv_part wkv_bf wmlp0_bf_xpad pool_out""")
HeadParams = _block("HeadParams", """
    int P C L groups; ptr o w1 w2 gn1_g gn1_b gn2_g gn2_b w_out b_out pooled logits w1t w2t""")
LiveParams = _block("LiveParams", "ptr count; int period offset")

_TFwd = _block("_TFwd", """
    int B cin1 cin2 cout L; ptr x x2 isc ish; int in_relu; ptr wp bias res; int out_relu; ptr y stats; int pool_K;
    ptr pool_gamma pool_ymax pool_arg""")
_TBwd = _block("_TBwd", """
    int B cin1 cin2 cout L; ptr g y; int dy_mode; ptr ka kb kc argmax pooled; int K S; ptr x x2 isc ish iinv; int in_relu;
    ptr wpT dx dx2 dstats dwp dbp; long part_stride; int precision; ptr wpT_bf""")
_BnFwd = _block("_BnFwd", """
    ptr part; int nparts C; double R; ptr gamma beta; float eps momentum;
    ptr running_mean running_var scale shift inv_scale mean invstd shift0; int shift0_stride""")
_BnBwd = _block("_BnBwd", """
    ptr part; int nparts C; double R; ptr gamma mean invstd ka kb kc dgamma dbeta centre""")
_ReduceJob = _block("_ReduceJob", "ptr part out; long stride; int nparts rows cols ld")
_LinAttnP = _block("_LinAttnP", """
    int B Lq Sk d H; float eps; ptr q k v; long q_bs k_bs v_bs; ptr out A ks dout dq dk dv; long dq_bs dk_bs dv_bs;
    int kv_roll""")
_AttnTailP = _block("_AttnTailP", """
    int B L d c1 hid out residual; float eps; ptr msg res wm w0 w2 wmT w0T w2T g1 b1 g2 b2 outp dout dmsg dres parts;
    long part_stride; int precision fwd_precision""")
_AttnHeadP = _block("_AttnHeadP", """
    int B L c hd d np src; ptr x xyz p1 p2 c1 c2 p2T; ptr[3] w wT; ptr outp dout dx parts; long part_stride;
    int precision fwd_precision""")

BLOCKS = {"pcr_assoc_multi": AssocMultiParams, "pcr_assoc_decode": AssocDecodeParams, "pcr_bank": BankParams,"pcr_truth": TruthParams, "pcr_store_tables": StoreTables, "pcr_sa_params": SaParams, "pcr_attn_params": AttnParams, "pcr_head_params": HeadParams,
          "pcr_live": LiveParams,
          "pcr_tdense_fwd": _TFwd, "pcr_tdense_bwd": _TBwd, "pcr_bn_fwd_fin": _BnFwd, "pcr_bn_bwd_fin": _BnBwd,
          "pcr_reduce_job": _ReduceJob, "pcr_linattn": _LinAttnP, "pcr_attn_tail": _AttnTailP,
          "pcr_attn_head": _AttnHeadP}

pcr_pack_desc = np.dtype([("w", "<u8"), ("out", "<u8"), ("rows", "<i4"), ("cols", "<i4"), ("kind", "<i4"),
                          ("reserved", "<i4")])
pcr_opt_tensor = np.dtype([("p", "<u8"), ("g", "<u8"), ("m", "<u8"), ("v", "<u8"), ("n", "<i8"), ("step_size", "<f4"),
                           ("bc2_sqrt", "<f4"), ("decay", "<f4"), ("one_m_beta1", "<f4"), ("beta2", "<f4"),
                           ("one_m_beta2", "<f4"), ("eps", "<f4"), ("pad_", "<f4")])
TABLES = {"pcr_pack_desc": pcr_pack_desc, "pcr_opt_tensor": pcr_opt_tensor}


class _TensorPtr:
    dtype = None

    @classmethod
    def from_param(cls, v):
        if isinstance(v, torch.Tensor):
            if v.dtype is not cls.dtype:
                raise TypeError("expected a %s tensor, got %s" % (cls.dtype, v.dtype))
            if not v.is_cuda or v.device.index != torch.cuda.current_device():
                raise TypeError("expected a tensor on the current GPU, got one on %s" % v.device)
            return ctypes.c_void_p(v.data_ptr())
        if v is None:
            return None
        if isinstance(v, int):
            return ctypes.c_void_p(v)
        return ctypes.c_void_p.from_param(v)


class FloatPtr(_TensorPtr):
    dtype = torch.float32


class IntPtr(_TensorPtr):
    dtype = torch.int32


SIGNATURES = {
    "pcr_abi_version": "i ",
    "pcr_status_string": "c i",
    "pcr_fps_f32": "s FFIiiiS",
    "pcr_fps_dist_f32": "s FFIiiiS",
    "pcr_pairwise_sqdist_f32": "s FFFiiiiiS",
    "pcr_ball_query_f32": "s FFIiiiffiS",
    "pcr_ball_query_cnt_f32": "s FFIIiiiffiS",
    "pcr_ball_query_rows_floats": "l iii",
    "pcr_ball_query_rows_ok": "i iif",
    "pcr_ball_query_rows_f32": "s FFIIFiiiffiS",
    "pcr_fps_ball_query_rows_ok": "i iii",
    "pcr_fps_ball_query_rows_f32": "s FFIFIFiiifiS",
    "pcr_fps_py_f32": "s FFIIiiiS",
    "pcr_query_ball_point_f32": "s FFIiiifiS",
    "pcr_knn_f32": "s FFIFiiiiS",
    "pcr_gather_fwd_f32": "s FIFiiiiS",
    "pcr_gather_bwd_f32": "s FIFiiiiS",
    "pcr_group_fwd_f32": "s FIFiiiiiS",
    "pcr_group_bwd_f32": "s FIFiiiiiS",
    "pcr_three_nn_f32": "s FFFIiiiS",
    "pcr_three_interp_fwd_f32": "s FIFFiiiiS",
    "pcr_three_interp_bwd_f32": "s FIFFiiiiS",
    "pcr_box_frames_f32": "s FFiS",
    "pcr_points_in_boxes_batch_f32": "s FFIiiiS",
    "pcr_points_in_boxes_f32": "s FFIiiiS",
    "pcr_crop_boxes_ok": "i iiii",
    "pcr_crop_boxes_f32": "s FiFIPFIiiiiiiS",
    "pcr_assoc_pairs_ok": "i iiii",
    "pcr_assoc_pairs_i32": "s IIIIIIiiiiiS",
    "pcr_assoc_cost_f32": "s FIIFFFfffFiiiS",
    "pcr_lsa_ok": "i iii",
    "pcr_lsa_f32": "s FIIFFIiiiS",
    "pcr_lsa_blocks_ok": "i iii",
    "pcr_lsa_blocks_f32": "s FIIIIFFIiiiS",
    "pcr_assoc_blocks_i32": "s IIIIiiiiiS",
    "pcr_assoc_multi_ok": "i iiiii",
    "pcr_assoc_multi_ws_bytes": "i iiii",
    "pcr_assoc_cost_multi_f32": "s <AssocMultiParams>S",
    "pcr_assoc_decode_i32": "s <AssocDecodeParams>S",
    "pcr_nearest_bev_f32": "s FFiS",
    "pcr_bev_frames_f32": "s FFiS",
    "pcr_iou_bev_f32": "s FFFiiiS",
    "pcr_nms_ok": "i i",
    "pcr_nms_ws_bytes": "i i",
    "pcr_nms_f32": "s FFFIIIIPiiiS",
    "pcr_track_nms_f32": "s FIFFIiS",
    "pcr_bank_ok": "i iiiii",
    "pcr_bank_plan_i32": "s <BankParams>S",
    "pcr_bank_move_f32": "s IFFFFiiiiS",
    "pcr_bank_dist_f32": "s FIFFFiiiS",
    "pcr_bank_retire_i32": "s IIIIiS",
    "pcr_store_gather_f32": "s FPiIIIPFIIiiS",
    "pcr_store_train_pairs_i32": "s <StoreTables>IIIPIIIIiS",
    "pcr_truth_ok": "i iiiii",
    "pcr_truth_cost_f32": "s FIFIIFFiiiiS",
    "pcr_truth_decide_i32": "s <TruthParams>S",
    "pcr_truth_record_i32": "s <TruthParams>S",
    "pcr_knn_prefix_f32": "s FIiiiiS",
    "pcr_knn_prefix2_f32": "s FIIiiiiiiS",
    "pcr_packed_weight_floats": "l ii",
    "pcr_pack_weight_f32": "s FiiF",
    "pcr_packed_weight_bf16_floats": "l ii",
    "pcr_pack_weight_bf16x2_f32": "s FiiF",
    "pcr_sa_mlp_f32": "s <SaParams>S",
    "pcr_sa_claim_ws_ints": "l iiiiii",
    "pcr_sa_tile_ws_ints": "l iiiii",
    "pcr_sa_krow_uses_tiles": "i iiiii",
    "pcr_sa_uses_row_table": "i iiiii",
    "pcr_dense_pm_f32": "s FFFiiiiiS",
    "pcr_dense_pm_prec_f32": "s FFFiiiiiiS",
    "pcr_dense_pm_xyz_f32": "s FFFFFiiiiiiiiS",
    "pcr_sa_tables_take_xyz": "i iiiiiii",
    "pcr_attn_kv_floats": "l i",
    "pcr_attn_kv_splits": "i iii",
    "pcr_attn_kv_f32": "s <AttnParams>S",
    "pcr_attn_apply_f32": "s <AttnParams>S",
    "pcr_attn_apply_pool_ok": "i <AttnParams>",
    "pcr_attn_live_ok": "i <AttnParams>",
    "pcr_attn_kv_live_f32": "s <AttnParams><LiveParams>S",
    "pcr_attn_apply_live_f32": "s <AttnParams><LiveParams>S",
    "pcr_pool_head_f32": "s <HeadParams>S",
    "pcr_pool_head_live_f32": "s <HeadParams><LiveParams>FS",
    "pcr_pool_both_f32": "s FFiiiS",
    "pcr_channel_max_f32": "s FFiiiiS",
    "pcr_dense_f32": "s FFFFFiiiiiS",
    "pcr_dense_xpm_f32": "s FFFFFiiiiiS",
    "pcr_dense_gn_f32": "s FFFFFFiiiiiiS",
    "pcr_dense_prec_ok": "i iii",
    "pcr_dense_prec_f32": "s FFFFFiiiiiiS",
    "pcr_dense_gn_prec_f32": "s FFFFFFiiiiiiiS",
    "pcr_dense_xpm_prec_ok": "i iii",
    "pcr_dense_xpm_prec_f32": "s FFFFFiiiiiiS",
    "pcr_max_over_l_f32": "s FFiiiS",
    "pcr_dense_max_ok": "i iii",
    "pcr_dense_max_f32": "s FFFFFiiiiiS",
    "pcr_pack_bmm_f32": "s FFiiS",
    "pcr_dense_bmm_f32": "s FFFiiiiS",
    "pcr_groupnorm_f32": "s FFFFFiiiiiS",
    "pcr_knn_feat_f32": "s FFIiiiilS",
    "pcr_edge_max_f32": "s FFIFfFlFliiiiS",
    "pcr_local_attn_f32": "s FIFiiiiifS",
    "pcr_pack_weight_dev_f32": "s FiiiiFS",
    "pcr_train_groups": "i ii",
    "pcr_train_groups_bwd": "i iiii",
    "pcr_tdense_fwd_groups": "i <_TFwd>",
    "pcr_tdense_bwd_groups": "i <_TBwd>",
    "pcr_set_stream_min_blocks": "i i",
    "pcr_tdense_fwd_f32": "s <_TFwd>S",
    "pcr_tdense_fwd_pooled": "i <_TFwd>",
    "pcr_tdense_bwd_f32": "s <_TBwd>S",
    "pcr_pack_weight_bf16_dev_f32": "s FiiiiFS",
    "pcr_local_attn_train_fwd_f32": "s FIFiiiiifS",
    "pcr_local_attn_train_bwd_f32": "s FIFFlFiiiiifS",
    "pcr_reduce_parts_f32": "s FiliiiFS",
    "pcr_reduce_multi_f32": "s <_ReduceJob>iS",
    "pcr_bn_fwd_finalize_f32": "s <_BnFwd>S",
    "pcr_bn_bwd_finalize_f32": "s <_BnBwd>S",
    "pcr_sa_l1_fwd_f32": "s FIFFFFFiiiiiS",
    "pcr_sa_l1_bwd_f32": "s FIFFFFFFFiiiiiS",
    "pcr_sa_pool_fwd_f32": "s FFFFIFiiiiS",
    "pcr_sa_pool_bwd_stats_f32": "s FFFFFiiiS",
    "pcr_tnorm_fwd_f32": "s FFFFFFFiiiifiS",
    "pcr_tnorm_bwd_f32": "s FFFFFFFFFiiiiS",
    "pcr_linattn_fwd_f32": "s <_LinAttnP>S",
    "pcr_linattn_bwd_f32": "s <_LinAttnP>S",
    "pcr_attn_tail_ok": "i iiiii",
    "pcr_attn_tail_part_floats": "i iiii",
    "pcr_attn_tail_groups": "i <_AttnTailP>",
    "pcr_attn_tail_fwd_f32": "s <_AttnTailP>S",
    "pcr_attn_tail_bwd_f32": "s <_AttnTailP>S",
    "pcr_attn_head_ok": "i iiiii",
    "pcr_attn_head_part_floats": "i iiiii",
    "pcr_attn_head_groups": "i <_AttnHeadP>",
    "pcr_attn_head_fwd_f32": "s <_AttnHeadP>S",
    "pcr_attn_head_bwd_f32": "s <_AttnHeadP>S",
    "pcr_pool_pair_fwd_f32": "s FFIiiiS",
    "pcr_pool_pair_bwd_f32": "s FIFiiiS",
    "pcr_pool_both_fwd_f32": "s FFIiiiS",
    "pcr_pool_both_bwd_f32": "s FIFiiiS",
    "pcr_channel_max_fwd_f32": "s FFIiiiiS",
    "pcr_channel_max_bwd_f32": "s FIFiiiiS",
    "pcr_bn_sums_f32": "s FFFFifFiFiiiiS",
    "pcr_bn_affine_f32": "s FFFFFFFFifFiiiS",
    "pcr_edge_pool_fwd_f32": "s FFFfFIFiiiiS",
    "pcr_edge_pool_route_f32": "s FFIfFiiiiS",
    "pcr_bmm_apply_f32": "s FFFiiiiS",
    "pcr_bmm_dt_f32": "s FFFiiiS",
    "pcr_pack_weights_multi_f32": "s PiS",
    "pcr_opt_chunk": "i ",
    "pcr_grad_sumsq_f32": "s PIIiPS",
    "pcr_adamw_step_f32": "s PIIiPfFS",
    "pcr_wall_clock_khz": "i ",
    "pcr_last_launch_arith": "i ",
    "pcr_clock_probe": "s PiiS",
}

_RETURN = {"s": ctypes.c_int, "i": ctypes.c_int, "l": ctypes.c_long, "c": ctypes.c_char_p}
_KIND = {"i": ctypes.c_int, "f": ctypes.c_float, "l": ctypes.c_long, "S": ctypes.c_void_p, "P": ctypes.c_void_p,
         "F": FloatPtr, "I": IntPtr}


def kinds(sig):
    ret, _, params = sig.partition(" ")
    out, i = [], 0
    while i < len(params):
        j = params.index(">", i) + 1 if params[i] == "<" else i + 1
        out.append(params[i:j])
        i = j
    return ret, out


def prototype(sig):
    ret, params = kinds(sig)
    return _RETURN[ret], [_KIND[k] if k in _KIND else ctypes.POINTER(globals()[k[1:-1]]) for k in params]
```

### point-cloud-reid_amd/pcr_amd/engine.py

```python
import ctypes
import os

import numpy as np
import torch

from . import _lib as L
from ._lib import _p
from .abi import AttnParams, HeadParams, LiveParams, SaParams

import os as _os
PRECISIONS = {"f32": 0, "bf16x3": 1, "bf16": 2}
PRECISION = _os.environ.get("PCR_PRECISION", "bf16x3")
if PRECISION not in PRECISIONS:
    raise L.PcrError("PCR_PRECISION must be one of %s" % sorted(PRECISIONS))


KV_SPLITS = int(os.environ["PCR_KV_SPLITS"]) if os.environ.get("PCR_KV_SPLITS") else None


def set_precision(name):
    global PRECISION
    if name not in PRECISIONS:
        raise L.PcrError("precision must be one of %s" % sorted(PRECISIONS))
    prev, PRECISION = PRECISION, name
    return prev


class precision:

    def __init__(self, name):
        self.name = name

    def __enter__(self):
        self.prev = set_precision(self.name)

    def __exit__(self, *exc):
        set_precision(self.prev)
        return False


GUARD = _os.environ.get("PCR_GUARD", "1") != "0"
GUARD_BOUND = float(_os.environ.get("PCR_GUARD_BOUND", "5e-5"))
GUARD_ACCEPT = float(_os.environ.get("PCR_GUARD_ACCEPT", "0.9"))
GUARD_EVERY = int(_os.environ.get("PCR_GUARD_EVERY", "64"))
GUARD_SENTINEL_PAIRS = int(_os.environ.get("PCR_GUARD_SENTINEL_PAIRS", "8"))
_LEVEL = 0


class guard_level:

    def __init__(self, level):
        self.level = int(level)

    def __enter__(self):
        global _LEVEL
        self.prev_level, _LEVEL = _LEVEL, self.level
        self.prev_prec = set_precision("f32") if (self.level >= 2 and PRECISION == "bf16x3") else None

    def __exit__(self, *exc):
        global _LEVEL
        _LEVEL = self.prev_level
        if self.prev_prec is not None:
            set_precision(self.prev_prec)
        return False


def guarded(fn):
    if _LEVEL >= 1 and PRECISION == "bf16x3":
        with precision("f32"):
            return fn()
    return fn()


SA_CLAIMS = _os.environ.get("PCR_SA_CLAIMS", "1") != "0"

SA_XYZ_TABLES = _os.environ.get("PCR_SA_XYZ_TABLES", "1") != "0"

PROFILE = None
ARITH_NAMES = {0: "f32", 1: "bf16x3", 2: "bf16"}


class _prof:
    def __init__(self, name, flops=0.0, nbytes=0.0, exec_flops=None, arith=None):
        self.name, self.flops, self.nbytes, self.arith = name, flops, nbytes, arith
        self.exec_flops = flops if exec_flops is None else exec_flops

    def __enter__(self):
        if PROFILE is not None:
            self.e0 = torch.cuda.Event(enable_timing=True)
            self.e1 = torch.cuda.Event(enable_timing=True)
            self.e0.record()
        return self

    def __exit__(self, *exc):
        if PROFILE is not None:
            self.e1.record()
            arith = self.arith
            if arith == "lib":
                arith = ARITH_NAMES.get(L.load().pcr_last_launch_arith(), "f32")
            PROFILE.append((self.name, self.e0, self.e1, self.flops, self.nbytes, self.exec_flops, arith))
        return False


def _dev32(t, device):
    return t.detach().to(device=device, dtype=torch.float32).contiguous()


def pack_weight(w, device):
    w2 = w.detach().reshape(w.shape[0], -1).to("cpu", torch.float32).contiguous().numpy()
    cout, cin = w2.shape
    lib = L.load()
    n = lib.pcr_packed_weight_floats(cout, cin)
    out = np.empty(n, np.float32)
    L.run.pcr_pack_weight_f32(w2.ctypes.data_as(ctypes.c_void_p), cout, cin, out.ctypes.data_as(ctypes.c_void_p))
    return torch.from_numpy(out).to(device)


def pack_weight_bf(w, device):
    w2 = w.detach().reshape(w.shape[0], -1).to("cpu", torch.float32).contiguous().numpy()
    cout, cin = w2.shape
    lib = L.load()
    n = lib.pcr_packed_weight_bf16_floats(cout, cin)
    out = np.empty(n, np.float32)
    L.run.pcr_pack_weight_bf16x2_f32(w2.ctypes.data_as(ctypes.c_void_p), cout, cin,
                                     out.ctypes.data_as(ctypes.c_void_p))
    return torch.from_numpy(out).to(device)


def pack_weight_dual(w, device):
    wp = pack_weight(w, device)
    cout, cin = w.shape[0], int(np.prod(w.shape[1:]))
    if L.load().pcr_dense_prec_ok(cin, cout, 1) or L.load().pcr_dense_xpm_prec_ok(cin, cout, 1):
        wp._pcr_bf = pack_weight_bf(w, device)
    return wp


def fold_bn(bn, conv_bias, device):
    scale = bn.weight.detach().double() / torch.sqrt(bn.running_var.detach().double() + bn.eps)
    bias = conv_bias.detach().double() if conv_bias is not None else 0.0
    shift = (bias - bn.running_mean.detach().double()) * scale + bn.bias.detach().double()
    return _dev32(scale.float(), device), _dev32(shift.float(), device)


def param_version(module):
    return tuple((t.data_ptr(), t._version) for t in list(module.parameters()) + list(module.buffers()))


def knn_prefix(xyz, S, K):
    L.require_cuda(xyz)
    assert xyz.is_contiguous() and xyz.dtype == torch.float32
    B, N, _ = xyz.shape
    idx = torch.empty((B, S, K), dtype=torch.int32, device=xyz.device)
    with _prof("knn_prefix[N=%d,S=%d,K=%d]" % (N, S, K), 8.0 * B * S * N, 12.0 * B * N + 4.0 * B * S * K):
        L.run.pcr_knn_prefix_f32(xyz, idx, B, N, S, K, L.stream_ptr())
    return idx


def knn_prefix2(xyz, S, K, S2, K2):
    L.require_cuda(xyz)
    assert xyz.is_contiguous() and xyz.dtype == torch.float32 and S2 <= S and K2 >= K
    B, N, _ = xyz.shape
    if S2 == 0 or B == 0:
        return knn_prefix(xyz, S, K), torch.empty((B, S2, K2), dtype=torch.int32, device=xyz.device)
    idx = torch.empty((B, S, K), dtype=torch.int32, device=xyz.device)
    idx2 = torch.empty((B, S2, K2), dtype=torch.int32, device=xyz.device)
    with _prof("knn_prefix2[N=%d,S=%d,K=%d,S2=%d,K2=%d]" % (N, S, K, S2, K2), 8.0 * B * S * N,
               12.0 * B * N + 4.0 * B * (S * K + S2 * K2)):
        L.run.pcr_knn_prefix2_f32(xyz, idx, idx2, B, N, S, K, S2, K2, L.stream_ptr())
    return idx, idx2


class SaPlan:

    def __init__(self, convs, bns, device, mode, fast=True):
        assert len(convs) == 3 and len(bns) == 3, "the fused SA kernel covers 3-layer MLPs"
        self.mode = mode
        self.cin = convs[0].weight.shape[1]
        self.couts = [c.weight.shape[0] for c in convs]
        self.wp = [pack_weight(c.weight, device) for c in convs]
        folded = [fold_bn(b, c.bias, device) for c, b in zip(convs, bns)]
        self.scale = [f[0] for f in folded]
        self.shift = [f[1] for f in folded]
        w1 = convs[0].weight.detach().reshape(self.couts[0], -1).double().cpu()
        D = (self.cin - 3) // 2 if mode == 0 else self.cin - 3
        self.D = D
        sc1 = self.scale[0].detach().double().cpu().unsqueeze(1)
        self.wa = _dev32((w1[:, :3] * sc1).float(), device)
        self.wa_packed = pack_weight((w1[:, :3] * sc1).float(), device)
        self.wa_shift_packed = pack_weight(torch.cat([w1[:, :3] * sc1, self.shift[0].detach().double().cpu().unsqueeze(1)],
                                                     dim=1).float(), device)
        self.wpq = None
        self.fast = fast
        self.wps, self.shift_pad, self.wps_bf = [], [], []
        for l in (1, 2):
            w = convs[l].weight.detach().reshape(self.couts[l], -1).double().cpu()
            sc = self.scale[l].detach().double().cpu().unsqueeze(1)
            self.wps.append(pack_weight((w * sc).float(), device))
            self.wps_bf.append(pack_weight_bf((w * sc).float(), device))
            pad = torch.zeros((self.couts[l] + 31) // 32 * 32, dtype=torch.float32, device=device)
            pad[:self.couts[l]] = self.shift[l]
            self.shift_pad.append(pad)
        if D > 0:
            if mode == 0:
                wc, wf = w1[:, 3:3 + D], w1[:, 3 + D:3 + 2 * D]
                stacked = torch.cat([wf * sc1, (wc - wf) * sc1], dim=0)
            else:
                stacked = w1[:, 3:3 + D] * sc1
            self.wpq = pack_weight(stacked.float(), device)
            self.wpq_bf = pack_weight_bf(stacked.float(), device)
            if mode == 0:
                wa64 = w1[:, :3] * sc1
                sh64 = self.shift[0].detach().double().cpu().unsqueeze(1)
                self.wxyz = _dev32(torch.cat([torch.cat([wa64, torch.zeros_like(sh64)], dim=1),
                                              torch.cat([-wa64, sh64], dim=1)], dim=0).float().contiguous(), device)

    def wants_row_table(self, N, K, min_radius, B=1, S=1):
        lib = L.load()
        if os.environ.get("PCR_SA_NO_STREAM") or int(B) * int(S) >= 2 ** 31:
            return False
        return bool(self.fast and self.mode == 1 and lib.pcr_ball_query_rows_ok(N, K, min_radius or 0.0) and
                    lib.pcr_sa_uses_row_table(self.couts[0], self.couts[1], self.couts[2], K, PRECISIONS[PRECISION]))

    def run(self, xyz, feat, idx, centre_idx=None, cnt=None, out_point_major=False, rows=None, K=None):
        B, N, _ = xyz.shape
        if rows is not None:
            S = cnt.shape[1]
            assert cnt is not None and self.wants_row_table(N, K, 0.0, B, S), "row table given to a layer that does not read it"
            L.require_cuda(xyz, cnt, rows)
            assert rows.is_contiguous() and rows.numel() == L.load().pcr_ball_query_rows_floats(B, S, K)
        else:
            L.require_cuda(xyz, idx)
            _, S, K = idx.shape
        D = 0 if feat is None else feat.shape[1]
        want = 3 + (2 * D if self.mode == 0 else D)
        assert want == self.cin, "feature width %d does not match the first conv (%d)" % (want, self.cin)
        feat, feat_pm = as_cm_or_pm(feat)
        assert xyz.is_contiguous() and (idx is None or idx.is_contiguous())
        out = torch.empty((B, S, self.couts[2]) if out_point_major else (B, self.couts[2], S),
                          dtype=torch.float32, device=xyz.device)
        p = SaParams()
        p.mode, p.B, p.N, p.S, p.K, p.D = self.mode, B, N, S, K, D
        p.c1, p.c2, p.c3 = self.couts
        p.xyz, p.feat, p.idx, p.centre_idx = _p(xyz), _p(feat), _p(idx), _p(centre_idx)
        for i in range(3):
            p.wp[i], p.scale[i], p.shift[i] = _p(self.wp[i]), _p(self.scale[i]), _p(self.shift[i])
        p.out = _p(out)
        p.feat_point_major, p.out_point_major = int(feat_pm), int(bool(out_point_major))
        ragged = cnt is not None and self.fast and self.mode == 1
        if cnt is not None:
            assert cnt.is_contiguous() and cnt.dtype == torch.int32 and cnt.shape == (B, S)
        tiled = ragged or (self.fast and self.mode == 1 and L.load().pcr_sa_krow_uses_tiles(
            self.couts[0], self.couts[1], self.couts[2], K, PRECISIONS[PRECISION]))
        if tiled:
            n_ws = L.load().pcr_sa_tile_ws_ints(B, S, K, self.couts[1], self.couts[2])
            if n_ws > 0:
                tile_ws = torch.empty((n_ws,), dtype=torch.int32, device=xyz.device)
                p.tile_ws = _p(tile_ws)
            if ragged:
                p.cnt = _p(cnt)
                p.row_tab = _p(rows)
        if self.fast:
            p.wa = _p(self.wa)
            p.wa_packed = _p(self.wa_packed)
            p.wa_shift_packed = _p(self.wa_shift_packed)
            p.precision = PRECISIONS[PRECISION]
            n_claim = 0 if (ragged or not SA_CLAIMS) else L.load().pcr_sa_claim_ws_ints(
                self.couts[0], self.couts[1], self.couts[2], K, N, PRECISIONS[PRECISION])
            if n_claim > 0:
                claim_ws = torch.empty((n_claim,), dtype=torch.int32, device=xyz.device)
                p.claim_ws = _p(claim_ws)
            for i in range(2):
                p.wps[i], p.shift_pad[i] = _p(self.wps[i]), _p(self.shift_pad[i])
                p.wps_bf[i] = _p(self.wps_bf[i])
            if D:
                c1_, c2_, c3_ = self.couts
                pqw = (2 if self.mode == 0 else 1) * self.couts[0]
                ws = torch.empty((B, N, pqw), dtype=torch.float32, device=xyz.device)
                p.wpq, p.pq_ws = _p(self.wpq), _p(ws)
                with _prof("sa_tables[D=%d,out=%d,N=%d]" % (D, pqw, N), 2.0 * B * N * D * pqw,
                           4.0 * B * N * (D + pqw), arith="lib"):
                    if PRECISION == "f32":
                        L.run.pcr_dense_pm_f32(feat, self.wpq, ws, B, D, pqw, N, int(feat_pm), L.stream_ptr())
                    elif (SA_XYZ_TABLES and not ragged and not tiled and idx is not None and
                          L.load().pcr_sa_tables_take_xyz(self.mode, D, c1_, c2_, c3_, K, PRECISIONS[PRECISION])):
                        q_rows = min(N, (S + 63) // 64 * 64) if centre_idx is None else N
                        q_rows = q_rows if q_rows % 64 == 0 else N
                        L.run.pcr_dense_pm_xyz_f32(feat, self.wpq_bf, xyz, self.wxyz, ws, B, D, pqw, N, int(feat_pm),
                                                   PRECISIONS[PRECISION], q_rows, c1_ if q_rows < N else pqw,
                                                   L.stream_ptr())
                        p.pq_has_xyz = 1
                    else:
                        L.run.pcr_dense_pm_prec_f32(feat, self.wpq_bf, ws, B, D, pqw, N, int(feat_pm),
                                                    PRECISIONS[PRECISION], L.stream_ptr())
                p.pq_ready = 1
        c1, c2, c3 = self.couts
        flops = 2.0 * B * S * K * (self.cin * c1 + c1 * c2 + c2 * c3)
        nbytes = 4.0 * B * (3 * N + D * N + S * K + c3 * S)
        exec_flops = 2.0 * B * S * K * (c1 * c2 + c2 * c3) if self.fast else flops
        if ragged:
            rows = float(((cnt.clamp(1, K) + 1) // 2 * 2).sum().item()) if PROFILE is not None else 0.0
            exec_flops = 2.0 * rows * (c1 * c2 + c2 * c3)
        name = "sa_ragged" if ragged else "sa_fused"
        with _prof("%s[D=%d,c=%d/%d/%d,N=%d,S=%d,K=%d]" % (name, D, c1, c2, c3, N, S, K), flops, nbytes, exec_flops,
                   arith="lib"):
            L.run.pcr_sa_mlp_f32(ctypes.byref(p), L.stream_ptr())
        return out.transpose(1, 2) if out_point_major else out


def _live_block(live):
    count, period, offset = live
    L.require_cuda(count)
    if count.dtype != torch.int32 or count.numel() < 1 or not count.is_contiguous():
        raise L.PcrError("live: count must be a contiguous int32 device tensor of at least one element")
    if int(period) < 1 or int(offset) < 0:
        raise L.PcrError("live: period must be positive and offset non-negative, got %r, %r" % (period, offset))
    lv = LiveParams()
    lv.count, lv.period, lv.offset = _p(count), int(period), int(offset)
    return lv


class AttnPlan:

    def __init__(self, m, pos_name, device, nhead, q_pos, k_pos, residual, final=None):
        pos = getattr(m, pos_name)
        L.require_default_eps(m.norm1, m.norm2)
        self.device = device
        self.nhead, self.q_pos, self.k_pos, self.residual = nhead, int(q_pos), int(k_pos), int(residual)
        self.d = d = m.q_proj.weight.shape[0]
        self.c1 = m.q_proj.weight.shape[1]
        self.c2 = m.k_proj.weight.shape[1]
        self.cout = m.mlp[2].weight.shape[0]
        f64 = lambda x: x.detach().double().cpu()
        W2, b2 = f64(pos[2].weight), f64(pos[2].bias)
        Wq, Wk, Wv = f64(m.q_proj.weight), f64(m.k_proj.weight), f64(m.v_proj.weight)
        if q_pos:
            wq = torch.cat([Wq, Wq @ W2], dim=1)
            bq = Wq @ b2
        else:
            wq, bq = Wq, torch.zeros(d, dtype=torch.float64)
        kz = (Wk @ W2) if k_pos else torch.zeros(d, d, dtype=torch.float64)
        wkv = torch.cat([torch.cat([Wk, kz], dim=1), torch.cat([Wv, Wv @ W2], dim=1)], dim=0)
        bkv = torch.cat([(Wk @ b2) if k_pos else torch.zeros(d, dtype=torch.float64), Wv @ b2])
        self.t = dict(
            pos0_w=_dev32(pos[0].weight, device), pos0_b=_dev32(pos[0].bias, device),
            wq=pack_weight(wq.float(), device), bq=_dev32(bq.float(), device),
            wkv=pack_weight(wkv.float(), device), bkv=_dev32(bkv.float(), device),
            wmerge=_dev32(m.merge.weight, device),
            wmlp0=pack_weight(m.mlp[0].weight, device), wmlp2=pack_weight(m.mlp[2].weight, device),
            ln1_g=_dev32(m.norm1.weight, device), ln1_b=_dev32(m.norm1.bias, device),
            ln2_g=_dev32(m.norm2.weight, device), ln2_b=_dev32(m.norm2.bias, device))
        if d <= 128:
            if d % 32 == 0 and (d // nhead) % 32 == 0:
                self.t["wmerge_packed"] = pack_weight(m.merge.weight, device)
            if (d == 64 and self.c2 in (64, 128)) or (d == 32 and self.c2 == 32) or d == 128:
                self.t["wkv_bf"] = pack_weight_bf(wkv.float(), device)
            if d == 64 and self.c1 % 16:
                w0 = m.mlp[0].weight.detach().float().cpu()
                pad = torch.zeros(w0.shape[0], 16 * ((self.c1 + 15) // 16) - self.c1)
                self.t["wmlp0_bf_xpad"] = pack_weight_bf(torch.cat([w0[:, :self.c1], pad, w0[:, self.c1:]], dim=1), device)
            self.t.update(wq_bf=pack_weight_bf(wq.float(), device),
                          wmlp0_bf=pack_weight_bf(m.mlp[0].weight, device), wmlp2_bf=pack_weight_bf(m.mlp[2].weight, device))
        if d > 128:
            dh = d // nhead
            if d % 64 or dh % 64 or dh > 256:
                raise L.PcrError("attention with d_model %d, %d heads is not covered (heads of 64..256 channels)" % (d, nhead))
            imgs, biases = [], []
            for g in range(d // 64):
                hd = (64 * g) // dh
                rows = torch.cat([torch.arange(64 * g, 64 * g + 64), torch.arange(d + hd * dh, d + (hd + 1) * dh)])
                imgs.append(pack_weight(wkv[rows].float(), device))
                biases.append(bkv[rows].float())
            self.t["wkv_wide"] = torch.cat(imgs).contiguous()
            self.t["bkv_wide"] = _dev32(torch.cat(biases), device)
            self.t["wmerge_packed"] = pack_weight(m.merge.weight, device)
        self.cfinal = 0
        if final is not None:
            self.t["wfinal"] = pack_weight(final.weight, device)
            if d <= 128:
                self.t["wfinal_bf"] = pack_weight_bf(final.weight, device)
            self.cfinal = final.weight.shape[0]
            bpad = torch.zeros((self.cfinal + 31) // 32 * 32, dtype=torch.float32, device=device)
            bpad[:self.cfinal] = final.bias.detach().to(device).float()
            self.t["bfinal"] = bpad

    def _params(self, B, Lq, Sk, feat_q, xyz_q, feat_k, xyz_k, kv, out, kv_index=None, q_index=None):
        p = AttnParams()
        p.B, p.Lq, p.Sk = B, Lq, Sk
        p.c1, p.c2, p.d, p.cout, p.nhead = self.c1, self.c2, self.d, self.cout, self.nhead
        p.q_pos, p.residual = self.q_pos, self.residual
        p.feat_q, p.xyz_q, p.feat_k, p.xyz_k = _p(feat_q), _p(xyz_q), _p(feat_k), _p(xyz_k)
        p.kv_index, p.q_index = _p(kv_index), _p(q_index)
        for k, v in self.t.items():
            setattr(p, k, _p(v))
        p.cfinal = self.cfinal
        p.kv, p.out = _p(kv), _p(out)
        p.precision = PRECISIONS[PRECISION]
        return p

    def live_ok(self):
        dummy = torch.empty(0)
        p = self._params(1, 32, 32, dummy, None, dummy, None, dummy, dummy)
        p.feat_q = p.feat_k = p.xyz_q = p.xyz_k = p.kv = p.out = 1
        return bool(L.load().pcr_attn_live_ok(ctypes.byref(p)))

    def kv(self, feat_k, xyz_k, live=None, out=None):
        L.require_cuda(feat_k, xyz_k)
        assert feat_k.is_contiguous() and xyz_k.is_contiguous() and feat_k.dtype == torch.float32
        B, c2, Sk = feat_k.shape
        assert c2 == self.c2
        lib = L.load()
        if out is not None:
            L.require_cuda(out)
            assert out.is_contiguous() and out.dtype == torch.float32 and tuple(out.shape) == (B, lib.pcr_attn_kv_floats(self.d))
        kv = out if out is not None else torch.empty((B, lib.pcr_attn_kv_floats(self.d)), dtype=torch.float32,
                                                     device=feat_k.device)
        p = self._params(B, 1, Sk, feat_k, xyz_k, feat_k, xyz_k, kv, kv)
        d = self.d
        ns = lib.pcr_attn_kv_splits(B, Sk, d) if KV_SPLITS is None else KV_SPLITS
        if live is not None and ns > 1:
            raise L.PcrError("a gated kv launch takes whole clouds (kv_splits = %d)" % ns)
        if ns > 1:
            part = torch.empty((B, ns, lib.pcr_attn_kv_floats(d)), dtype=torch.float32, device=feat_k.device)
            p.kv_splits, p.kv_part = ns, _p(part)
        kv_flops = 2.0 * B * Sk * (3 * d + d * c2 + 2 * c2 * d + d * d / self.nhead)
        with _prof("attn_kv[d=%d,c2=%d,Sk=%d]" % (d, c2, Sk), kv_flops, 4.0 * B * (c2 * Sk + 3 * Sk + d * d + d),
                   arith="lib"):
            if live is not None:
                L.run.pcr_attn_kv_live_f32(ctypes.byref(p), ctypes.byref(_live_block(live)), L.stream_ptr())
            else:
                L.run.pcr_attn_kv_f32(ctypes.byref(p), L.stream_ptr())
        kv._pcr_precision = PRECISION
        return kv

    def pool_ok(self, Lq, Sk):
        dummy = torch.empty(0)
        p = self._params(1, Lq, Sk, dummy, None, dummy, None, dummy, dummy)
        p.feat_q = p.feat_k = p.xyz_k = p.kv = p.out = 1
        return bool(L.load().pcr_attn_apply_pool_ok(ctypes.byref(p)))

    def apply(self, feat_q, xyz_q, kv, Sk, kv_index=None, q_index=None, n_out=None, pooled=False, live=None, out=None):
        L.require_cuda(feat_q, kv)
        assert feat_q.is_contiguous() and feat_q.dtype == torch.float32 and (xyz_q is None or xyz_q.is_contiguous())
        Bq, c1, Lq = feat_q.shape
        assert c1 == self.c1
        made = getattr(kv, "_pcr_precision", PRECISION)
        if (made == "f32") != (PRECISION == "f32") and self.d <= 128:
            raise L.PcrError("attention state was built in %r mode and is applied in %r mode: the per-cloud matrix is "
                             "stored in the arithmetic's own layout" % (made, PRECISION))
        B = n_out if n_out is not None else Bq
        shape = (B, 2, self.cout) if pooled else (B, self.cfinal or self.cout, Lq)
        if out is not None:
            L.require_cuda(out)
            assert out.is_contiguous() and out.dtype == torch.float32 and tuple(out.shape) == shape
        if pooled:
            if out is None:
                out = (torch.zeros if live is not None else torch.empty)(shape, dtype=torch.float32, device=feat_q.device)
            p = self._params(B, Lq, Sk, feat_q, xyz_q, feat_q, xyz_q if xyz_q is not None else feat_q, kv, None,
                             kv_index, q_index)
            p.pool_out = _p(out)
        else:
            if out is None:
                out = torch.empty(shape, dtype=torch.float32, device=feat_q.device)
            p = self._params(B, Lq, Sk, feat_q, xyz_q, feat_q, xyz_q if xyz_q is not None else feat_q, kv, out,
                             kv_index, q_index)
        d = self.d
        ap_flops = 2.0 * B * Lq * (c1 * d + d * d / self.nhead + d * d + (c1 + d) * 2 * d + 2 * d * self.cout
                                   + self.cout * self.cfinal + (self.q_pos * (3 * d + d * c1)))
        with _prof("attn_apply[d=%d,c1=%d,out=%d,Lq=%d%s]" % (d, c1, self.cfinal or self.cout, Lq, ",pooled" if pooled else ""),
                   ap_flops, 4.0 * B * (c1 * Lq + d * d + d + (2 if pooled else Lq) * (self.cfinal or self.cout)), arith="lib"):
            if live is not None:
                L.run.pcr_attn_apply_live_f32(ctypes.byref(p), ctypes.byref(_live_block(live)), L.stream_ptr())
            else:
                L.run.pcr_attn_apply_f32(ctypes.byref(p), L.stream_ptr())
        return out

    def run(self, feat_q, xyz_q, feat_k, xyz_k, kv_index=None):
        assert feat_k.shape[0] == feat_q.shape[0]
        kv = self.kv(feat_k, xyz_k)
        return self.apply(feat_q, xyz_q, kv, feat_k.shape[2], kv_index=kv_index)


class HeadPlan:

    def __init__(self, linres, out_linear, device):
        if getattr(linres, "transform", None) is not None:
            raise L.PcrError("pcr_pool_head_f32 covers LinearRes with n_in == n_out only")
        L.require_default_eps(linres.norm1, linres.norm2)
        self.n = linres.linear1.weight.shape[0]
        self.groups = linres.norm1.num_groups
        self.t = dict(w1=_dev32(linres.linear1.weight, device), w2=_dev32(linres.linear2.weight, device),
                      gn1_g=_dev32(linres.norm1.weight, device), gn1_b=_dev32(linres.norm1.bias, device),
                      gn2_g=_dev32(linres.norm2.weight, device), gn2_b=_dev32(linres.norm2.bias, device),
                      w_out=_dev32(out_linear.weight, device), b_out=_dev32(out_linear.bias, device),
                      w1t=_dev32(linres.linear1.weight.detach().t().contiguous(), device),
                      w2t=_dev32(linres.linear2.weight.detach().t().contiguous(), device))

    def run(self, o, want_pooled=False, live=None, dead_value=0.0):
        L.require_cuda(o)
        assert o.is_contiguous() and o.dtype == torch.float32
        twoP, C, Lp = o.shape
        P = twoP // 2
        assert 2 * C == self.n, "pooled width %d != match head width %d" % (2 * C, self.n)
        logits = torch.empty((P,), dtype=torch.float32, device=o.device)
        pooled = torch.empty((P, 2 * C), dtype=torch.float32, device=o.device) if want_pooled else None
        p = HeadParams()
        p.P, p.C, p.L, p.groups = P, C, Lp, self.groups
        p.o = _p(o)
        for k, v in self.t.items():
            setattr(p, k, _p(v))
        p.pooled, p.logits = _p(pooled), _p(logits)
        with _prof("pool_head", 4.0 * P * (2 * C) ** 2, 4.0 * twoP * C * Lp):
            if live is not None:
                L.run.pcr_pool_head_live_f32(ctypes.byref(p), ctypes.byref(_live_block(live)),
                                             ctypes.byref(ctypes.c_float(dead_value)), L.stream_ptr())
            else:
                L.run.pcr_pool_head_f32(ctypes.byref(p), L.stream_ptr())
        return (logits, pooled) if want_pooled else logits


def as_cm_or_pm(x):
    if x is None or x.is_contiguous():
        return x, False
    if x.dim() == 3 and x.transpose(1, 2).is_contiguous():
        return x, True
    return x.contiguous(), False


def dense(x, wp, cout, scale=None, shift=None, act=0):
    L.require_cuda(x)
    assert x.dtype == torch.float32
    x, x_pm = as_cm_or_pm(x)
    B, cin, Ln = x.shape
    y = torch.empty((B, cout, Ln), dtype=torch.float32, device=x.device)
    lib = L.load()
    bf = getattr(wp, "_pcr_bf", None)
    if PRECISION != "f32" and bf is not None and not x_pm and lib.pcr_dense_prec_ok(cin, cout, Ln):
        with _prof("dense[cin=%d,cout=%d,L=%d]" % (cin, cout, Ln), 2.0 * B * Ln * cin * cout, 4.0 * B * Ln * (cin + cout),
                   arith=PRECISION):
            L.run.pcr_dense_prec_f32(x, bf, scale, shift, y, B, cin, cout, Ln, act, PRECISIONS[PRECISION],
                                     L.stream_ptr())
        return y
    if PRECISION != "f32" and bf is not None and x_pm and lib.pcr_dense_xpm_prec_ok(cin, cout, Ln):
        with _prof("dense[cin=%d,cout=%d,L=%d]" % (cin, cout, Ln), 2.0 * B * Ln * cin * cout, 4.0 * B * Ln * (cin + cout),
                   arith="lib"):
            L.run.pcr_dense_xpm_prec_f32(x, bf, scale, shift, y, B, cin, cout, Ln, act, PRECISIONS[PRECISION],
                                         L.stream_ptr())
        return y
    fn = L.run.pcr_dense_xpm_f32 if x_pm else L.run.pcr_dense_f32
    with _prof("dense[cin=%d,cout=%d,L=%d]" % (cin, cout, Ln), 2.0 * B * Ln * cin * cout, 4.0 * B * Ln * (cin + cout),
               arith="f32"):
        fn(x, wp, scale, shift, y, B, cin, cout, Ln, act, L.stream_ptr())
    return y
```

Measured before the change: 67330.

## Fuse next SA level's xyz-aware projection tables into attention apply epilogue

```diff
diff --git a/include/pcr.h b/include/pcr.h
--- a/include/pcr.h
+++ b/include/pcr.h
@@ -327,6 +327,14 @@
 int pcr_attn_kv_live_f32(const pcr_attn_params *p, const pcr_live *live, pcr_stream_t stream);
 int pcr_attn_apply_live_f32(const pcr_attn_params *p, const pcr_live *live, pcr_stream_t stream);
 
+typedef struct pcr_attn_tables {
+  float *out;
+  const float *w_bf, *wxyz;
+  int cout, q_rows, q_off;
+} pcr_attn_tables;
+int pcr_attn_apply_tables_ok(const pcr_attn_params *p, int cout);
+int pcr_attn_apply_tables_f32(const pcr_attn_params *p, const pcr_attn_tables *t, pcr_stream_t stream);
+
 typedef struct pcr_head_params {
   int P, C, L, groups;
   const float *o;
diff --git a/point-cloud-reid_amd/csrc/attn_kernels_impl.h b/point-cloud-reid_amd/csrc/attn_kernels_impl.h
--- a/point-cloud-reid_amd/csrc/attn_kernels_impl.h
+++ b/point-cloud-reid_amd/csrc/attn_kernels_impl.h
@@ -16,6 +16,8 @@
   int wpc;
   const int *live_count;
   int live_period, live_offset;
+  pcr_attn_tables t = {};
+  int t_plain = 0;
 };
 
 struct LiveWalk {
@@ -1004,10 +1006,11 @@
 
 #if PCR_ATTN_PREC != 0
 constexpr int kApsWaves = 8;
-template <bool QPOS, int C1S, int CF, int NOB = 2, int ND = 2, bool POOL = false, bool GATE = false>
+template <bool QPOS, int C1S, int CF, int NOB = 2, int ND = 2, bool POOL = false, bool GATE = false, int TBL = 0>
 __global__ __launch_bounds__(64 * kApsWaves) __attribute__((amdgpu_waves_per_eu(2, 2)))
 void attn_apply_stream64_kernel(AttnArgs a) {
   static_assert(!QPOS || C1S == 2 * ND, "q_pos needs c1 == d");
+  static_assert(!TBL || (QPOS && !CF && !POOL && !GATE && NOB == ND && TBL == 2 * ND), "tables: the self-attention forms");
   static_assert(NOB <= 2 || (NOB == 4 && !CF), "cout = 128 has no trailing conv");
   static_assert(!POOL || (!CF && NOB == 2), "pooled output: cout = 64, no trailing conv");
   constexpr int D = 32 * ND, SD = 2 * ND;
@@ -1020,12 +1023,22 @@
   float *s_c = reinterpret_cast<float *>(s_w2 + ND * NOB * 512);
   f32x4 *s_p0 = reinterpret_cast<f32x4 *>(s_c + 448);
   float *s_ks = reinterpret_cast<float *>(s_p0 + 64);
+  f32x4 *s_wx = reinterpret_cast<f32x4 *>(s_ks + 64 * kApsWaves);
+  bf16x8 *s_wt = reinterpret_cast<bf16x8 *>(s_wx + 64 * TBL);
   const int tid = threadIdx.x, lane = tid & 63, j = lane & 31, h = lane >> 5;
   const int wave = __builtin_amdgcn_readfirstlane(tid >> 6);
   LiveWalk lw{};
   if constexpr (GATE) {
     lw = live_walk(a);
     if ((long)blockIdx.x * kApsWaves >= lw.total * (POOL ? 1 : (p.Lq >> 5))) return;
+  }
+  if constexpr (TBL != 0) {
+    if (tid < 64 * TBL) s_wx[tid] = reinterpret_cast<const f32x4 *>(a.t.wxyz)[tid];
+    if constexpr (ND == 1) {
+      const f32x4 *wt = reinterpret_cast<const f32x4 *>(a.t.w_bf);
+      f32x4 *dt = reinterpret_cast<f32x4 *>(s_wt);
+      for (int e = tid; e < SD * TBL * 256; e += 64 * kApsWaves) dt[e] = wt[e];
+    }
   }
   {
     const f32x4 *wq = reinterpret_cast<const f32x4 *>(p.wq),
@@ -1378,6 +1391,100 @@
         const int ch = 16 * (e >> 3) + bf_kpos(0, e & 7);
         const float v = o[e >> 4][e & 15];
         __builtin_amdgcn_raw_buffer_store_b32(__builtin_bit_cast(unsigned, v), rout, vo, ch * p.Lq * 4, 0);
+      }
+      if constexpr (TBL != 0) {
+#pragma unroll
+        for (int cb = 0; cb < NOB; cb++)
+#pragma unroll
+          for (int G = 0; G < 2; G++) to_ops(o[cb], G, bh[2 * cb + G], bl[2 * cb + G]);
+        float cx[16], cy[16], cz[16];
+        {
+          const float *xb = p.xyz_q + (bq_ * p.Lq + blk * 32 + 4 * h) * 3;
+#pragma unroll
+          for (int r = 0; r < 16; r++) {
+            const float *q = xb + 3 * ((r & 3) + 8 * (r >> 2));
+            cx[r] = q[0];
+            cy[r] = q[1];
+            cz[r] = q[2];
+          }
+        }
+        const __amdgpu_buffer_rsrc_t rwt =
+            __builtin_amdgcn_make_buffer_rsrc(const_cast<float *>(a.t.w_bf), 0, SD * TBL * 256 * 16, 0x00020000);
+        auto wt = [&](int unit) __attribute__((always_inline)) {
+          if constexpr (ND == 1) return s_wt[unit * 64 + lane];
+          else return __builtin_bit_cast(bf16x8, __builtin_amdgcn_raw_buffer_load_b128(rwt, lane * 16, unit * 1024, 0));
+        };
+        const __amdgpu_buffer_rsrc_t rtab = __builtin_amdgcn_make_buffer_rsrc(
+            a.t.out + ((size_t)b * p.Lq + blk * 32) * (64 * TBL), 0, 32 * 64 * TBL * 4, 0x00020000);
+        const int tvo = (4 * h * 64 * TBL + j) * 4;
+        constexpr int CB = 2;
+        auto round = [&](int c0, auto split_tag) __attribute__((always_inline)) {
+          constexpr bool SPLIT = decltype(split_tag)::value;
+          f32x16 ta[CB];
+#pragma unroll
+          for (int cb = 0; cb < CB; cb++)
+#pragma unroll
+            for (int r = 0; r < 16; r++) ta[cb][r] = 0.f;
+          bf16x8 wh[2][CB], wl[2][CB];
+          auto fetch = [&](int s2) __attribute__((always_inline)) {
+#pragma unroll
+            for (int cb = 0; cb < CB; cb++) {
+              wh[s2 & 1][cb] = wt((s2 * 2 * TBL + c0 + cb) * 2);
+              if constexpr (SPLIT) wl[s2 & 1][cb] = wt((s2 * 2 * TBL + c0 + cb) * 2 + 1);
+            }
+          };
+          fetch(0);
+#pragma unroll
+          for (int s2 = 0; s2 < SD; s2++) {
+            if (s2 + 1 < SD) fetch(s2 + 1);
+            __builtin_amdgcn_sched_barrier(0);
+            const int u = s2 & 1;
+            if constexpr (SPLIT) {
+#pragma unroll
+              for (int cb = 0; cb < CB; cb++) ta[cb] = __builtin_amdgcn_mfma_f32_32x32x16_bf16(bl[s2], wh[u][cb], ta[cb], 0, 0, 0);
+#pragma unroll
+              for (int cb = 0; cb < CB; cb++) ta[cb] = __builtin_amdgcn_mfma_f32_32x32x16_bf16(bh[s2], wl[u][cb], ta[cb], 0, 0, 0);
+            }
+#pragma unroll
+            for (int cb = 0; cb < CB; cb++) ta[cb] = __builtin_amdgcn_mfma_f32_32x32x16_bf16(bh[s2], wh[u][cb], ta[cb], 0, 0, 0);
+            __builtin_amdgcn_sched_barrier(0);
+          }
+#pragma unroll
+          for (int cb = 0; cb < CB; cb++) {
+            const f32x4 w = s_wx[32 * (c0 + cb) + j];
+            float acc[16];
+#pragma unroll
+            for (int r = 0; r < 16; r++) {
+              acc[r] = ta[cb][r] + w[3];
+              asm volatile("" : "+v"(acc[r]));
+            }
+#pragma unroll
+            for (int r = 0; r < 16; r++) {
+              acc[r] = __builtin_fmaf(w[2], cz[r], acc[r]);
+              asm volatile("" : "+v"(acc[r]));
+            }
+#pragma unroll
+            for (int r = 0; r < 16; r++) {
+              acc[r] = __builtin_fmaf(w[1], cy[r], acc[r]);
+              asm volatile("" : "+v"(acc[r]));
+            }
+#pragma unroll
+            for (int r = 0; r < 16; r++) {
+              acc[r] = __builtin_fmaf(w[0], cx[r], acc[r]);
+              asm volatile("" : "+v"(acc[r]));
+            }
+#pragma unroll
+            for (int r = 0; r < 16; r++)
+              __builtin_amdgcn_raw_buffer_store_b32(__builtin_bit_cast(unsigned, acc[r]), rtab, tvo,
+                                                    (((r & 3) + 8 * (r >> 2)) * 64 * TBL + 32 * (c0 + cb)) * 4, 0);
+          }
+        };
+        const int ncb = blk * 32 < a.t.q_rows ? 2 * TBL : TBL;
+        if (a.t_plain) {
+          for (int c0 = 0; c0 < ncb; c0 += CB) round(c0, std::false_type{});
+        } else {
+          for (int c0 = 0; c0 < ncb; c0 += CB) round(c0, std::true_type{});
+        }
       }
     } else {
 #pragma unroll
@@ -2115,13 +2222,19 @@
   return p.d == 64 && aps_in && aps_out && (p.Lq & 31) == 0 && (p.nhead == 1 || p.nhead == 2 || p.nhead == 4);
 }
 
-static int attn_apply_launch(const pcr_attn_params *pp, const pcr_live *live, pcr_stream_t stream) {
+static int attn_apply_launch(const pcr_attn_params *pp, const pcr_live *live, pcr_stream_t stream,
+                             const pcr_attn_tables *tbl = nullptr) {
   const pcr_attn_params &p = *pp;
   AttnArgs a;
   a.p = p;
   a.dbg = 0;
   a.wpc = 0;
   if (!attn_set_live(a, live) || (live && !attn_live_shape(p))) return PCR_ERR_INVALID;
+  if (tbl) {
+    if (kAPrec == 0 || live) return PCR_ERR_INVALID;
+    a.t = *tbl;
+    a.t_plain = p.precision == PCR_PREC_BF16 ? 1 : 0;
+  }
   const int tb = p.d <= 32 ? 4 : (p.d <= 64 ? 2 : 1), T = 32 * tb, RP = T + 1;
   const int catP = ceil8(p.c1 + p.d);
   int rowsU = catP > 2 * p.d ? catP : 2 * p.d;
@@ -2137,7 +2250,11 @@
   const int aps_c1s = (p.c1 + 15) >> 4, aps_nd = p.d >> 5;
   const size_t aps_lds = (size_t)((aps_c1s + (p.q_pos ? 2 * aps_nd : 0)) * aps_nd * 128 + (aps_c1s + 2 * aps_nd) * aps_nd * 256 +
                                   aps_nd * (p.cout >> 5) * 512) * 16 +
-                         (size_t)(448 + 256 + 64 * kApsWaves) * sizeof(float);
+                         (size_t)(448 + 256 + 64 * kApsWaves) * sizeof(float) +
+                         (tbl ? (size_t)(4 * p.d + (p.d == 32 ? 1024 : 0)) * 16 : 0);
+  if (tbl && (!p.q_pos || p.cfinal || p.pool_out || p.c1 != p.d || p.cout != p.d || (p.d != 32 && !aps64_shape(p)) ||
+             aps_lds > (size_t)kMaxDynLds))
+    return PCR_ERR_INVALID;
   static const int no_s128 = pcr_tune_int("PCR_ATTN_NO_STREAM128");
   if (p.d == 128 && p.c1 == 128 && p.cout == 128 && !p.cfinal && p.q_pos && p.residual && (p.Lq & 31) == 0 && p.Lq >= 256 &&
       (p.nhead == 1 || p.nhead == 2 || p.nhead == 4) && !no_s128) {
@@ -2152,6 +2269,7 @@
     const long nitem = (long)p.B * (p.Lq >> 5);
     const long nwg = (nitem + kApsWaves - 1) / kApsWaves;
     const dim3 gg((unsigned)(nwg < pcr_cu_count() ? nwg : pcr_cu_count())), bb(64 * kApsWaves);
+    if (tbl) return pcr_launch_lds<attn_apply_stream64_kernel<true, 2, 0, 1, 1, false, false, 2>>(gg, bb, aps_lds, st, a);
     return p.q_pos ? pcr_launch_lds<attn_apply_stream64_kernel<true, 2, 0, 1, 1>>(gg, bb, aps_lds, st, a)
                    : pcr_launch_lds<attn_apply_stream64_kernel<false, 2, 0, 1, 1>>(gg, bb, aps_lds, st, a);
   }
@@ -2169,7 +2287,8 @@
       return attn_launch_g<attn_apply_stream64_kernel<false, 4, 0, 2, 2, true>, attn_apply_stream64_kernel<false, 4, 0, 2, 2, true, true>>(ggp, bb, aps_lds, st, a);
     }
     int rc;
-    if (nob == 4)
+    if (tbl) rc = pcr_launch_lds<attn_apply_stream64_kernel<true, 4, 0, 2, 2, false, false, 4>>(gg, bb, aps_lds, st, a);
+    else if (nob == 4)
       rc = p.q_pos ? pcr_launch_lds<attn_apply_stream64_kernel<true, 4, 0, 4>>(gg, bb, aps_lds, st, a)
                    : pcr_launch_lds<attn_apply_stream64_kernel<false, 4, 0, 4>>(gg, bb, aps_lds, st, a);
     else if (p.c1 < 16) rc = pcr_launch_lds<attn_apply_stream64_kernel<false, 1, 2, 1>>(gg, bb, aps_lds, st, a);
@@ -2186,6 +2305,7 @@
     return rc;
   }
 #endif
+  if (tbl) return PCR_ERR_INVALID;
   const bool wide = 2 * p.d > 128 || p.cout > 128 || p.cfinal > 128;
   if (tb == 4 && !live)
     return wide ? pcr_launch_lds<attn_apply_kernel<4, 2>>(g, blk, lds, st, a) : pcr_launch_lds<attn_apply_kernel<4, 1>>(g, blk, lds, st, a);
@@ -2207,9 +2327,13 @@
 #if PCR_ATTN_PREC == 1
 int pcr_attn_kv_bf3(const pcr_attn_params *pp, const pcr_live *live, pcr_stream_t stream) { return attn_kv_narrow(pp, live, stream); }
 int pcr_attn_apply_bf3(const pcr_attn_params *pp, const pcr_live *live, pcr_stream_t stream) { return attn_apply_launch(pp, live, stream); }
+int pcr_attn_apply_tables_bf3(const pcr_attn_params *pp, const pcr_attn_tables *tb, pcr_stream_t stream) {
+  return attn_apply_launch(pp, nullptr, stream, tb);
+}
 #else
 int pcr_attn_kv_bf3(const pcr_attn_params *pp, const pcr_live *live, pcr_stream_t stream);
 int pcr_attn_apply_bf3(const pcr_attn_params *pp, const pcr_live *live, pcr_stream_t stream);
+int pcr_attn_apply_tables_bf3(const pcr_attn_params *pp, const pcr_attn_tables *tb, pcr_stream_t stream);
 
 static bool attn_bf(const pcr_attn_params &p, pcr_attn_params &q) {
   const int widest = 2 * p.d > p.cout ? (2 * p.d > p.cfinal ? 2 * p.d : p.cfinal) : (p.cout > p.cfinal ? p.cout : p.cfinal);
@@ -2287,4 +2411,32 @@
 PCR_EXPORT int pcr_attn_apply_live_f32(const pcr_attn_params *pp, const pcr_live *live, pcr_stream_t stream) {
   return attn_apply_entry(pp, live, stream);
 }
+
+static bool attn_tables_ok(const pcr_attn_params &p, int cout) {
+  pcr_attn_params q;
+  if ((p.d != 32 && p.d != 64) || !p.q_pos || p.c1 != p.d || p.cout != p.d || p.cfinal || p.pool_out || (p.Lq & 31) ||
+      cout != 4 * p.d || !attn_bf(p, q))
+    return false;
+  return p.d == 32 ? (p.nhead == 1 || p.nhead == 2) : aps64_shape(p);
+}
+
+PCR_EXPORT int pcr_attn_apply_tables_ok(const pcr_attn_params *pp, int cout) {
+  return (pp && !attn_check(*pp) && attn_tables_ok(*pp, cout)) ? 1 : 0;
+}
+
+PCR_EXPORT int pcr_attn_apply_tables_f32(const pcr_attn_params *pp, const pcr_attn_tables *tb, pcr_stream_t stream) {
+  if (!pp || !tb || attn_check(*pp) || !pp->out || !attn_tables_ok(*pp, tb->cout)) return PCR_ERR_INVALID;
+  if (pp->q_index) return PCR_ERR_INVALID;
+  if (!tb->out || !tb->w_bf || !tb->wxyz || ((reinterpret_cast<size_t>(tb->out) | reinterpret_cast<size_t>(tb->w_bf) |
+                                               reinterpret_cast<size_t>(tb->wxyz)) & 15))
+    return PCR_ERR_INVALID;
+  if (tb->q_rows < 0 || tb->q_rows > pp->Lq || (tb->q_rows != pp->Lq && (tb->q_rows & 63)) ||
+      (tb->q_rows != pp->Lq && tb->q_off != tb->cout / 2) || (tb->q_rows == pp->Lq && tb->q_off != tb->cout / 2 && tb->q_off != tb->cout))
+    return PCR_ERR_INVALID;
+  if (pp->B == 0) return PCR_OK;
+  if (pp->B > 65535) return PCR_ERR_INVALID;
+  pcr_attn_params q;
+  attn_bf(*pp, q);
+  return pcr_attn_apply_tables_bf3(&q, tb, stream);
+}
 #endif
diff --git a/point-cloud-reid_amd/mmdet3d/models/backbone_net.py b/point-cloud-reid_amd/mmdet3d/models/backbone_net.py
--- a/point-cloud-reid_amd/mmdet3d/models/backbone_net.py
+++ b/point-cloud-reid_amd/mmdet3d/models/backbone_net.py
@@ -36,6 +36,7 @@
         xyz, features = self._break_up_pc(pointcloud)
         l_xyz, l_features = [xyz], [features]
         shared = None
+        tables = None
         for i, sa in enumerate(self.SA_modules):
             knn_idx = None
             if i == 0 and len(self.SA_modules) > 1 and hasattr(sa, "shares_knn_with") and not _NO_KNN2 and \
@@ -45,8 +46,18 @@
                                                      self.SA_modules[1].nsample)
             elif i == 1 and shared is not None:
                 knn_idx = shared
-            li_xyz, li_features = sa(l_xyz[i], l_features[i], numpoints[i]) if knn_idx is None else \
-                sa(l_xyz[i], l_features[i], numpoints[i], knn_idx=knn_idx)
+            nxt = self.SA_modules[i + 1] if i + 1 < len(self.SA_modules) else None
+            if isinstance(sa, PointNetSetAbstractionEdgeSA) and isinstance(nxt, PointNetSetAbstractionEdgeSA) and \
+                    all(m.sampling == "RANDOM" and m.use_knn for m in (sa, nxt)):
+                li_xyz, li_features, next_tables = sa(l_xyz[i], l_features[i], numpoints[i], knn_idx=knn_idx, tables=tables,
+                                                      next_level=(nxt, numpoints[i + 1]))
+            else:
+                kw = {} if knn_idx is None else {"knn_idx": knn_idx}
+                if tables is not None:
+                    kw["tables"] = tables
+                li_xyz, li_features = sa(l_xyz[i], l_features[i], numpoints[i], **kw)
+                next_tables = None
+            tables = next_tables
             l_xyz.append(li_xyz)
             l_features.append(li_features)
         l_features[0] = xyz.transpose(1, 2).contiguous()
diff --git a/point-cloud-reid_amd/mmdet3d/models/pointnet2_utils.py b/point-cloud-reid_amd/mmdet3d/models/pointnet2_utils.py
--- a/point-cloud-reid_amd/mmdet3d/models/pointnet2_utils.py
+++ b/point-cloud-reid_amd/mmdet3d/models/pointnet2_utils.py
@@ -85,13 +85,13 @@
         self.nhead = nhead
         _attn_holder(self, "pos_mlp", d_model, d_model, d_model, d_model, d_model * 2, d_model)
 
-    def forward(self, feat, xyz, mask=None):
+    def forward(self, feat, xyz, mask=None, next_sa=None):
         assert mask is None, "masks are never passed by the ReID model path"
         plan = self._plan(feat.device, lambda dev: engine.AttnPlan(self, "pos_mlp", dev, self.nhead,
                                                                    q_pos=True, k_pos=True, residual=True))
         feat = feat.contiguous()
         xyz = xyz.contiguous()
-        return plan.run(feat, xyz, feat, xyz)
+        return plan.run(feat, xyz, feat, xyz, next_sa=next_sa)
 
 
 class PointNetSetAbstractionEdgeSA(_Planned):
@@ -120,16 +120,24 @@
                 nxt.sampling == "RANDOM" and nxt.use_knn and numpoints == n and numpoints_next <= numpoints and
                 self.nsample <= nxt.nsample <= min(64, n))
 
-    def forward(self, xyz, points, numpoints, knn_idx=None):
-        plan = self._plan(xyz.device, lambda dev: engine.SaPlan(list(self.mlp_convs), list(self.mlp_bns), dev, mode=0))
+    def sa_plan(self, device):
+        return self._plan(device, lambda dev: engine.SaPlan(list(self.mlp_convs), list(self.mlp_bns), dev, mode=0))
+
+    def forward(self, xyz, points, numpoints, knn_idx=None, tables=None, next_level=None):
+        plan = self.sa_plan(xyz.device)
         xyz = xyz.contiguous()
         points = None if points is None else points.contiguous()
         if self.sampling == "RANDOM" and self.use_knn:
             idx = knn_idx if knn_idx is not None else engine.knn_prefix(xyz, numpoints, self.nsample)
             assert idx.shape == (xyz.shape[0], numpoints, self.nsample)
-            pooled = engine.guarded(lambda: plan.run(xyz, points, idx))
+            pooled = engine.guarded(lambda: plan.run(xyz, points, idx, tables=tables))
             new_xyz = xyz[:, :numpoints].contiguous()
-            return new_xyz, self.self_attention(pooled, new_xyz)
+            if next_level is None:
+                return new_xyz, self.self_attention(pooled, new_xyz)
+            nxt, s_next = next_level
+            feats, next_tables = self.self_attention(pooled, new_xyz, next_sa=(nxt.sa_plan(xyz.device), s_next, nxt.nsample))
+            return new_xyz, feats, next_tables
+        assert tables is None and next_level is None
         centre = (farthest_point_sample(xyz, numpoints) if self.sampling == "FPS"
                   else random_point_sample(xyz, numpoints)).to(torch.int32).contiguous()
         new_xyz = index_points(xyz, centre)
diff --git a/point-cloud-reid_amd/pcr_amd/abi.py b/point-cloud-reid_amd/pcr_amd/abi.py
--- a/point-cloud-reid_amd/pcr_amd/abi.py
+++ b/point-cloud-reid_amd/pcr_amd/abi.py
@@ -49,6 +49,7 @@
 HeadParams = _block("HeadParams", """
     int P C L groups; ptr o w1 w2 gn1_g gn1_b gn2_g gn2_b w_out b_out pooled logits w1t w2t""")
 LiveParams = _block("LiveParams", "ptr count; int period offset")
+AttnTables = _block("AttnTables", "ptr out w_bf wxyz; int cout q_rows q_off")
 
 _TFwd = _block("_TFwd", """
     int B cin1 cin2 cout L; ptr x x2 isc ish; int in_relu; ptr wp bias res; int out_relu; ptr y stats; int pool_K;
@@ -73,7 +74,7 @@
     int precision fwd_precision""")
 
 BLOCKS = {"pcr_assoc_multi": AssocMultiParams, "pcr_assoc_decode": AssocDecodeParams, "pcr_bank": BankParams,"pcr_truth": TruthParams, "pcr_store_tables": StoreTables, "pcr_sa_params": SaParams, "pcr_attn_params": AttnParams, "pcr_head_params": HeadParams,
-          "pcr_live": LiveParams,
+          "pcr_live": LiveParams, "pcr_attn_tables": AttnTables,
           "pcr_tdense_fwd": _TFwd, "pcr_tdense_bwd": _TBwd, "pcr_bn_fwd_fin": _BnFwd, "pcr_bn_bwd_fin": _BnBwd,
           "pcr_reduce_job": _ReduceJob, "pcr_linattn": _LinAttnP, "pcr_attn_tail": _AttnTailP,
           "pcr_attn_head": _AttnHeadP}
@@ -193,6 +194,8 @@
     "pcr_attn_live_ok": "i <AttnParams>",
     "pcr_attn_kv_live_f32": "s <AttnParams><LiveParams>S",
     "pcr_attn_apply_live_f32": "s <AttnParams><LiveParams>S",
+    "pcr_attn_apply_tables_ok": "i <AttnParams>i",
+    "pcr_attn_apply_tables_f32": "s <AttnParams><AttnTables>S",
     "pcr_pool_head_f32": "s <HeadParams>S",
     "pcr_pool_head_live_f32": "s <HeadParams><LiveParams>FS",
     "pcr_pool_both_f32": "s FFiiiS",
diff --git a/point-cloud-reid_amd/pcr_amd/engine.py b/point-cloud-reid_amd/pcr_amd/engine.py
--- a/point-cloud-reid_amd/pcr_amd/engine.py
+++ b/point-cloud-reid_amd/pcr_amd/engine.py
@@ -6,7 +6,7 @@
 
 from . import _lib as L
 from ._lib import _p
-from .abi import AttnParams, HeadParams, LiveParams, SaParams
+from .abi import AttnParams, AttnTables, HeadParams, LiveParams, SaParams
 
 import os as _os
 PRECISIONS = {"f32": 0, "bf16x3": 1, "bf16": 2}
@@ -75,6 +75,9 @@
 SA_CLAIMS = _os.environ.get("PCR_SA_CLAIMS", "1") != "0"
 
 SA_XYZ_TABLES = _os.environ.get("PCR_SA_XYZ_TABLES", "1") != "0"
+
+ATTN_TABLES = _os.environ.get("PCR_ATTN_TABLES", "1") != "0"
+ATTN_TABLES_MIN_LQ = int(_os.environ.get("PCR_ATTN_TABLES_MIN_LQ", "256"))
 
 PROFILE = None
 ARITH_NAMES = {0: "f32", 1: "bf16x3", 2: "bf16"}
@@ -221,7 +224,16 @@
         return bool(self.fast and self.mode == 1 and lib.pcr_ball_query_rows_ok(N, K, min_radius or 0.0) and
                     lib.pcr_sa_uses_row_table(self.couts[0], self.couts[1], self.couts[2], K, PRECISIONS[PRECISION]))
 
-    def run(self, xyz, feat, idx, centre_idx=None, cnt=None, out_point_major=False, rows=None, K=None):
+    def xyz_tables_split(self, N, S, K, prefix=True):
+        c1_, c2_, c3_ = self.couts
+        if not (SA_XYZ_TABLES and self.fast and self.mode == 0 and self.D > 0 and PRECISION != "f32" and
+                L.load().pcr_sa_tables_take_xyz(self.mode, self.D, c1_, c2_, c3_, K, PRECISIONS[PRECISION])):
+            return None
+        q_rows = min(N, (S + 63) // 64 * 64) if prefix else N
+        q_rows = q_rows if q_rows % 64 == 0 else N
+        return 2 * c1_, q_rows, c1_ if q_rows < N else 2 * c1_
+
+    def run(self, xyz, feat, idx, centre_idx=None, cnt=None, out_point_major=False, rows=None, K=None, tables=None):
         B, N, _ = xyz.shape
         if rows is not None:
             S = cnt.shape[1]
@@ -273,25 +285,29 @@
                 p.wps[i], p.shift_pad[i] = _p(self.wps[i]), _p(self.shift_pad[i])
                 p.wps_bf[i] = _p(self.wps_bf[i])
             if D:
-                c1_, c2_, c3_ = self.couts
                 pqw = (2 if self.mode == 0 else 1) * self.couts[0]
-                ws = torch.empty((B, N, pqw), dtype=torch.float32, device=xyz.device)
+                split = None if (ragged or tiled or idx is None) else self.xyz_tables_split(N, S, K, centre_idx is None)
+                if tables is not None:
+                    assert split is not None and centre_idx is None, "tables given to a launch that does not read them"
+                    L.require_cuda(tables)
+                    assert tables.is_contiguous() and tables.dtype == torch.float32 and tuple(tables.shape) == (B, N, pqw)
+                    ws = tables
+                    p.pq_has_xyz = 1
+                else:
+                    ws = torch.empty((B, N, pqw), dtype=torch.float32, device=xyz.device)
                 p.wpq, p.pq_ws = _p(self.wpq), _p(ws)
-                with _prof("sa_tables[D=%d,out=%d,N=%d]" % (D, pqw, N), 2.0 * B * N * D * pqw,
-                           4.0 * B * N * (D + pqw), arith="lib"):
-                    if PRECISION == "f32":
-                        L.run.pcr_dense_pm_f32(feat, self.wpq, ws, B, D, pqw, N, int(feat_pm), L.stream_ptr())
-                    elif (SA_XYZ_TABLES and not ragged and not tiled and idx is not None and
-                          L.load().pcr_sa_tables_take_xyz(self.mode, D, c1_, c2_, c3_, K, PRECISIONS[PRECISION])):
-                        q_rows = min(N, (S + 63) // 64 * 64) if centre_idx is None else N
-                        q_rows = q_rows if q_rows % 64 == 0 else N
-                        L.run.pcr_dense_pm_xyz_f32(feat, self.wpq_bf, xyz, self.wxyz, ws, B, D, pqw, N, int(feat_pm),
-                                                   PRECISIONS[PRECISION], q_rows, c1_ if q_rows < N else pqw,
-                                                   L.stream_ptr())
-                        p.pq_has_xyz = 1
-                    else:
-                        L.run.pcr_dense_pm_prec_f32(feat, self.wpq_bf, ws, B, D, pqw, N, int(feat_pm),
-                                                    PRECISIONS[PRECISION], L.stream_ptr())
+                if tables is None:
+                    with _prof("sa_tables[D=%d,out=%d,N=%d]" % (D, pqw, N), 2.0 * B * N * D * pqw,
+                               4.0 * B * N * (D + pqw), arith="lib"):
+                        if PRECISION == "f32":
+                            L.run.pcr_dense_pm_f32(feat, self.wpq, ws, B, D, pqw, N, int(feat_pm), L.stream_ptr())
+                        elif split is not None:
+                            L.run.pcr_dense_pm_xyz_f32(feat, self.wpq_bf, xyz, self.wxyz, ws, B, D, pqw, N, int(feat_pm),
+                                                       PRECISIONS[PRECISION], split[1], split[2], L.stream_ptr())
+                            p.pq_has_xyz = 1
+                        else:
+                            L.run.pcr_dense_pm_prec_f32(feat, self.wpq_bf, ws, B, D, pqw, N, int(feat_pm),
+                                                        PRECISIONS[PRECISION], L.stream_ptr())
                 p.pq_ready = 1
         c1, c2, c3 = self.couts
         flops = 2.0 * B * S * K * (self.cin * c1 + c1 * c2 + c2 * c3)
@@ -438,7 +454,19 @@
         p.feat_q = p.feat_k = p.xyz_k = p.kv = p.out = 1
         return bool(L.load().pcr_attn_apply_pool_ok(ctypes.byref(p)))
 
-    def apply(self, feat_q, xyz_q, kv, Sk, kv_index=None, q_index=None, n_out=None, pooled=False, live=None, out=None):
+    def _next_tables(self, p, next_sa, Lq):
+        if next_sa is None or not ATTN_TABLES or Lq < ATTN_TABLES_MIN_LQ or _LEVEL != 0:
+            return None
+        sa, S, K = next_sa
+        if sa.D != self.cout:
+            return None
+        split = sa.xyz_tables_split(Lq, S, K)
+        if split is None or not L.load().pcr_attn_apply_tables_ok(ctypes.byref(p), split[0]):
+            return None
+        return split
+
+    def apply(self, feat_q, xyz_q, kv, Sk, kv_index=None, q_index=None, n_out=None, pooled=False, live=None, out=None,
+              next_sa=None):
         L.require_cuda(feat_q, kv)
         assert feat_q.is_contiguous() and feat_q.dtype == torch.float32 and (xyz_q is None or xyz_q.is_contiguous())
         Bq, c1, Lq = feat_q.shape
@@ -466,18 +494,35 @@
         d = self.d
         ap_flops = 2.0 * B * Lq * (c1 * d + d * d / self.nhead + d * d + (c1 + d) * 2 * d + 2 * d * self.cout
                                    + self.cout * self.cfinal + (self.q_pos * (3 * d + d * c1)))
-        with _prof("attn_apply[d=%d,c1=%d,out=%d,Lq=%d%s]" % (d, c1, self.cfinal or self.cout, Lq, ",pooled" if pooled else ""),
-                   ap_flops, 4.0 * B * (c1 * Lq + d * d + d + (2 if pooled else Lq) * (self.cfinal or self.cout)), arith="lib"):
-            if live is not None:
+        split = None
+        if next_sa is not None and not pooled and live is None and q_index is None and n_out is None:
+            split = self._next_tables(p, next_sa, Lq)
+        tables, tb = None, None
+        if split is not None:
+            sa, pqw = next_sa[0], split[0]
+            tables = torch.empty((B, Lq, pqw), dtype=torch.float32, device=feat_q.device)
+            tb = AttnTables()
+            tb.out, tb.w_bf, tb.wxyz = _p(tables), _p(sa.wpq_bf), _p(sa.wxyz)
+            tb.cout, tb.q_rows, tb.q_off = split
+            ap_flops += 2.0 * B * (Lq + split[1]) * d * (pqw // 2)
+        name = "attn_apply[d=%d,c1=%d,out=%d,Lq=%d%s]" % (
+            d, c1, self.cfinal or self.cout, Lq, ",pooled" if pooled else (",tables=%d" % split[0] if split else ""))
+        nbytes = 4.0 * B * (c1 * Lq + d * d + d + (2 if pooled else Lq) * (self.cfinal or self.cout))
+        if split is not None:
+            nbytes += 4.0 * B * (Lq + split[1]) * (split[0] // 2)
+        with _prof(name, ap_flops, nbytes, arith="lib"):
+            if tb is not None:
+                L.run.pcr_attn_apply_tables_f32(ctypes.byref(p), ctypes.byref(tb), L.stream_ptr())
+            elif live is not None:
                 L.run.pcr_attn_apply_live_f32(ctypes.byref(p), ctypes.byref(_live_block(live)), L.stream_ptr())
             else:
                 L.run.pcr_attn_apply_f32(ctypes.byref(p), L.stream_ptr())
-        return out
-
-    def run(self, feat_q, xyz_q, feat_k, xyz_k, kv_index=None):
+        return (out, tables) if next_sa is not None else out
+
+    def run(self, feat_q, xyz_q, feat_k, xyz_k, kv_index=None, next_sa=None):
         assert feat_k.shape[0] == feat_q.shape[0]
         kv = self.kv(feat_k, xyz_k)
-        return self.apply(feat_q, xyz_q, kv, feat_k.shape[2], kv_index=kv_index)
+        return self.apply(feat_q, xyz_q, kv, feat_k.shape[2], kv_index=kv_index, next_sa=next_sa)
 
 
 class HeadPlan:
```

Measured after the change: 67820 (median of 6 runs). No clear change (+0.7%).
